# pmandros/node2vec2rank

Hardware: AMD Instinct MI355X
Metric: nodes ranked/sec + SpMM HBM GB/s, K-layer N-node graph at 1/2/4/8 GPUs (higher is better)
Workload: dtype fp32; 1 GPU; cfg4: 2-layer ER N=1M avg-deg 50, dims {8,16,32,64,128} x {cosine,euclidean}, sequential; nodes=1000000, layers=2, embed_dim=128, columns=10, comparisons=1, parallelism=single GPU

## Files before the change

### include/n2v2r.h

```cpp
#ifndef N2V2R_H
#define N2V2R_H

#include <stddef.h>
#include <stdint.h>

#ifdef __cplusplus
extern "C" {
#endif

typedef enum {
  N2V2R_OK = 0,
  N2V2R_ERR_BAD_ARG = 1,
  N2V2R_ERR_UNSUPPORTED_METRIC = 2,
  N2V2R_ERR_NO_CONVERGENCE = 3,
  N2V2R_ERR_HIP = 4,
  N2V2R_ERR_OUT_OF_MEMORY = 5,
  N2V2R_ERR_NOT_READY = 6,
  N2V2R_ERR_UNSUPPORTED_AGG = 7,
  N2V2R_ERR_INTERNAL = 8,
  N2V2R_ERR_RCCL = 9
} n2v2r_status;

enum { N2V2R_SEQUENTIAL = 0, N2V2R_ONE_VS_BEFORE = 1, N2V2R_ONE_VS_REST = 2 };
enum { N2V2R_COSINE = 0, N2V2R_EUCLIDEAN = 1, N2V2R_CORRELATION = 2 };
enum { N2V2R_SYM_DETECT = -1, N2V2R_SYM_NO = 0, N2V2R_SYM_YES = 1 };
enum { N2V2R_AGG_BORDA = 0, N2V2R_AGG_NONE = -1 };

enum { N2V2R_EIG_FULL_FIRST_PASS = 1, N2V2R_EIG_DENSE_RR = 2,
       N2V2R_EIG_TEST_REDO_CYCLE = 4 ,
       N2V2R_EIG_TEST_BAND_FAIL = 8 ,
       N2V2R_EIG_TEST_STURM_FAIL = 32 ,
       N2V2R_EIG_TIME_SPMM = 16 ,
       N2V2R_EIG_TEST_NO_STAGNATION = 64 ,
       N2V2R_EIG_TEST_FAIL_ALONE = 128 ,
       N2V2R_EIG_TEST_TRI_TIMEOUT = 1024  };

typedef struct n2v2r_handle n2v2r_handle;
typedef struct n2v2r_simgroup n2v2r_simgroup;

typedef struct {
  int block;
  int max_basis;
  int keep;
  int max_restarts;
  double tol;
  uint64_t seed;
  int solver_flags;
} n2v2r_eig_opts;

typedef struct {
  int restarts;
  int block_applications;
  int converged;
  int basis;
  double max_residual;
  double ms_total, ms_spmm, ms_ortho, ms_rr_host;
  int64_t spmm_launches;
  double spmm_algo_bytes;
  int stagnated;
  int rr_fallbacks;
  double gpu_ms_spmm[2];
  int64_t spmm_timed_launches[2];
  double spmm_stage_bytes[2];
  double est_scale;
  int lean_checks;
  int pool_blocks;
  int spmm_form;
  double stag_cap;
  int y_captured;
  int tri_fallbacks;
} n2v2r_eig_stats;

int n2v2r_create(int device, n2v2r_handle** out);
void n2v2r_destroy(n2v2r_handle* h);
int n2v2r_last_error(const n2v2r_handle* h, char* buf, size_t len);
const char* n2v2r_version(void);

#define N2V2R_UNIQUE_ID_BYTES 128
int n2v2r_comm_unique_id(char* out, size_t len);
int n2v2r_create_rccl(int device, int rank, int world, const char* unique_id, n2v2r_handle** out);
int n2v2r_simgroup_create(int world, n2v2r_simgroup** out);
void n2v2r_simgroup_destroy(n2v2r_simgroup* g);
int n2v2r_create_sim(int device, n2v2r_simgroup* g, int rank, n2v2r_handle** out);
int n2v2r_dist_info(const n2v2r_handle* h, int* rank, int* world, int64_t* row0, int64_t* n_local);

int n2v2r_create_multi(const int* devices, int n_gpus, n2v2r_handle** out);
int n2v2r_multi_devices(const n2v2r_handle* h, int* devices, int cap);

int n2v2r_set_num_layers(n2v2r_handle* h, int num_layers, int64_t n);
int n2v2r_set_layer_csr(n2v2r_handle* h, int k, int64_t n, int64_t nnz, const int64_t* indptr,
                        const int32_t* indices, const float* data, int symmetric);
int n2v2r_set_layer_dense(n2v2r_handle* h, int k, int64_t n, const float* A, int symmetric);
enum { N2V2R_CORR_UNSIGNED = 0, N2V2R_CORR_SIGNED = 1, N2V2R_CORR_SIGNED_HYBRID = 2,
       N2V2R_CORR_RAW = 3 };
int n2v2r_set_layer_corr(n2v2r_handle* h, int k, int64_t n, int64_t samples,
                         const double* E , int kind, double power);
int n2v2r_soft_connectivity(n2v2r_handle* h, int64_t n, int64_t samples, const double* E,
                            int kind, const double* powers, int n_powers, double* conn);
enum { N2V2R_COR_PEARSON = 0, N2V2R_COR_SPEARMAN = 1, N2V2R_COR_BICOR = 2 };
int n2v2r_set_layer_corr_method(n2v2r_handle* h, int k, int64_t n, int64_t samples,
                                const double* E , int kind,
                                double power, int method, int64_t* fallback );
int n2v2r_soft_connectivity_method(n2v2r_handle* h, int64_t n, int64_t samples, const double* E,
                                   int kind, const double* powers, int n_powers, int method,
                                   double* conn, int64_t* fallback );
enum { N2V2R_TF_ABSOLUTE = 1, N2V2R_TF_BINARIZE = 2, N2V2R_TF_THRESHOLD = 4 };
typedef struct { int64_t nonzero; int64_t kept; double cut; } n2v2r_transform_stats;
int n2v2r_transform_layer(n2v2r_handle* h, int k, int flags, double threshold,
                          double top_percent_keep, n2v2r_transform_stats* stats );
enum { N2V2R_TOM_UNSIGNED = 0, N2V2R_TOM_SIGNED = 1 };
int n2v2r_tom_layer(n2v2r_handle* h, int k, int type);
int n2v2r_layers_to_csr(n2v2r_handle* h, int64_t* nnz );
int n2v2r_count_layer_nonzeros(n2v2r_handle* h, int64_t* nnz );
int n2v2r_set_layer_csr_rows(n2v2r_handle* h, int k, int64_t n, int64_t row0, int64_t n_rows,
                             int64_t nnz, const int64_t* indptr, const int32_t* indices,
                             const float* data);

int n2v2r_uase(n2v2r_handle* h, int d, const n2v2r_eig_opts* opts, n2v2r_eig_stats* stats);
// ... 32 lines not shown
```

### include/n2v2r_diag.h

```cpp
#ifndef N2V2R_DIAG_H
#define N2V2R_DIAG_H

#include "n2v2r.h"

#ifdef __cplusplus
extern "C" {
#endif

int n2v2r_bench_spmm(n2v2r_handle* h, int k, int transpose, int b, int reps, const float* X,
                     float* Y, double* avg_ms, double* algo_bytes);
int n2v2r_bench_spmm_tiled(n2v2r_handle* h, int k, int transpose, int b, int nb, int reps,
                           const float* X, float* Y, double* avg_ms);

int n2v2r_spmm_col_blocks(const n2v2r_handle* h, int b);

int n2v2r_rr_top(n2v2r_handle* h, int c, const double* H, int p, double* w, float* S);

int n2v2r_pip_pass(n2v2r_handle* h, int64_t n, int nq, const float* Q, float* Za, float* Zb,
                   float tau, int first, int form, uint64_t seed, double* gram, double* R,
                   int* flags, int* any_flag, int* skipped);

typedef struct n2v2r_gram_info {
  int form;
  int rs_form;
  int rs_chunks;
  int split2;
  int tile_nb, tile_wb, tile_rows;
  int rpw1, rpw2;
} n2v2r_gram_info;

int n2v2r_gram_apply(n2v2r_handle* h, int b, const float* X, float* Z, float* W,
                     n2v2r_gram_info* info);

typedef struct n2v2r_ritz_info {
  int fused;
  int launches;
  int lds_bytes;
} n2v2r_ritz_info;

int n2v2r_ritz_step(n2v2r_handle* h, int b, int nq, int keep, int lean, const float* Q,
                    const float* W, const float* S, const double* theta, float* X, float* MX,
                    double* res, n2v2r_ritz_info* info);

typedef struct n2v2r_pass_info {
  int gram_form;
  int gram_flush;
  int64_t nchunks;
  int64_t rows_per_chunk;
  int stage;
  int nwg;
  int apply_kernel;
  int reserved;
  uint64_t fill_seed;
} n2v2r_pass_info;

int n2v2r_block_gram(n2v2r_handle* h, int b, int na, int nb, const float* A, const float* B,
                     double* G, n2v2r_pass_info* info);

int n2v2r_ortho_pass(n2v2r_handle* h, int b, int nq, const float* Q, float* Z, int in_place,
                     int first, int cond, uint64_t seed, double* gram, double* xinv, float* F,
                     int* flags, int* any_flag, n2v2r_pass_info* info);

int n2v2r_rr_band_top(n2v2r_handle* h, int c, int kp, const double* hband, int64_t hband_len,
                      const double* theta_prev, int p, double* w, float* S);

typedef struct n2v2r_rr_info {
  int form_ran;
  int sturm_err;
  int second_solves;
  int reduce_err;
  int tri_coop;
  int msect_points, msect_rounds;
  int reserved;
} n2v2r_rr_info;

int n2v2r_rr_stage(n2v2r_handle* h, int c, int kp, const double* hband, int64_t hband_len,
                   const double* theta_prev, int p, int form, double* w, float* S,
                   double* Y , n2v2r_rr_info* info);

typedef struct n2v2r_embed_info {
  int form;
  int launches;
  int ldu;
  int rpw;
  int64_t colmax_chunks;
  int64_t colmax_rows;
} n2v2r_embed_info;

int n2v2r_embed_step(n2v2r_handle* h, int b, int d, const float* U, const double* theta,
                     n2v2r_embed_info* info);

int n2v2r_h2d_layer_bytes(const n2v2r_handle* h, int64_t* per_rank, int cap);

int n2v2r_get_layer_dense(n2v2r_handle* h, int k, float* A );

int n2v2r_get_layer_csr_nnz(n2v2r_handle* h, int k, int transpose, int64_t* nnz);
int n2v2r_get_layer_csr(n2v2r_handle* h, int k, int transpose, int64_t* indptr, int32_t* indices,
                        float* data);

int n2v2r_bench_sparsify_pass(n2v2r_handle* h, int k, int which, int reps, double* avg_ms,
                              double* bytes);

int n2v2r_bench_transform_pass(n2v2r_handle* h, int k, int which, int flags, double threshold,
// ... 21 lines not shown
```

### node2vec2rank_amd/_lib.py

```python
from __future__ import annotations

import atexit
import ctypes
import os
import threading
import warnings
import weakref

import numpy as np

from .coexpression import KINDS, METHODS, Coexpression, method_name

_HERE = os.path.dirname(os.path.abspath(__file__))
LIB_PATH = os.environ.get("N2V2R_LIB", os.path.join(_HERE, "lib", "libn2v2r_hip.so"))

OK = 0
ERR_BAD_ARG = 1
ERR_UNSUPPORTED_METRIC = 2
ERR_NO_CONVERGENCE = 3
ERR_HIP = 4
ERR_OUT_OF_MEMORY = 5
ERR_NOT_READY = 6
ERR_UNSUPPORTED_AGG = 7
ERR_INTERNAL = 8
ERR_RCCL = 9
AGG_BORDA, AGG_NONE = 0, -1
EIG_TIME_SPMM = 16
EIG_TEST_NO_STAGNATION = 64
EIG_TEST_FAIL_ALONE = 128

STRATEGY = {"sequential": 0, "one_vs_before": 1, "one_vs_rest": 2}
METRIC = {"cosine": 0, "euclidean": 1, "correlation": 2}
SYM_DETECT, SYM_NO, SYM_YES = -1, 0, 1

EXPORTED = [
    "n2v2r_create", "n2v2r_destroy", "n2v2r_last_error", "n2v2r_version",
    "n2v2r_set_num_layers", "n2v2r_set_layer_csr", "n2v2r_uase", "n2v2r_get_embedding",
    "n2v2r_get_left_embedding", "n2v2r_get_singular_values", "n2v2r_set_embedding",
    "n2v2r_rank", "n2v2r_get_distances", "n2v2r_get_borda", "n2v2r_rank_timing",
    "n2v2r_pairwise_distances", "n2v2r_borda_columns", "n2v2r_borda_columns_ex",
    "n2v2r_column_sums",
    "n2v2r_synchronize", "n2v2r_bench_spmm", "n2v2r_bench_spmm_tiled", "n2v2r_spmm_col_blocks",
    "n2v2r_comm_unique_id", "n2v2r_create_rccl", "n2v2r_simgroup_create",
    "n2v2r_simgroup_destroy", "n2v2r_create_sim", "n2v2r_dist_info", "n2v2r_set_layer_csr_rows",
    "n2v2r_rr_top", "n2v2r_rr_band_top", "n2v2r_set_layer_dense", "n2v2r_project",
    "n2v2r_create_multi", "n2v2r_multi_devices", "n2v2r_h2d_layer_bytes",
    "n2v2r_set_layer_corr", "n2v2r_get_layer_dense", "n2v2r_transform_layer",
    "n2v2r_bench_transform_pass", "n2v2r_tom_layer", "n2v2r_bench_tom_tiles", "n2v2r_pip_pass",
    "n2v2r_gram_apply", "n2v2r_ritz_step", "n2v2r_layers_to_csr", "n2v2r_count_layer_nonzeros",
    "n2v2r_get_layer_csr_nnz", "n2v2r_get_layer_csr", "n2v2r_bench_sparsify_pass",
    "n2v2r_block_gram", "n2v2r_ortho_pass", "n2v2r_soft_connectivity",
    "n2v2r_soft_connectivity_chunks", "n2v2r_set_layer_corr_method",
    "n2v2r_soft_connectivity_method", "n2v2r_corr_ranks", "n2v2r_corr_standardise",
    "n2v2r_bench_corr_rows", "n2v2r_rr_stage", "n2v2r_embed_step",
]
UNIQUE_ID_BYTES = 128


class ArpackNoConvergence(RuntimeError):
    """UASE eigensolver did not reach the residual tolerance (scipy raises
    ``ArpackNoConvergence`` in the reference's svds path)."""


class EigOpts(ctypes.Structure):
    _fields_ = [("block", ctypes.c_int), ("max_basis", ctypes.c_int), ("keep", ctypes.c_int),
                ("max_restarts", ctypes.c_int), ("tol", ctypes.c_double),
                ("seed", ctypes.c_uint64), ("solver_flags", ctypes.c_int)]


class EigStats(ctypes.Structure):
    _fields_ = [("restarts", ctypes.c_int), ("block_applications", ctypes.c_int),
                ("converged", ctypes.c_int), ("basis", ctypes.c_int),
                ("max_residual", ctypes.c_double), ("ms_total", ctypes.c_double),
                ("ms_spmm", ctypes.c_double), ("ms_ortho", ctypes.c_double),
                ("ms_rr_host", ctypes.c_double), ("spmm_launches", ctypes.c_int64),
                ("spmm_algo_bytes", ctypes.c_double), ("stagnated", ctypes.c_int),
                ("rr_fallbacks", ctypes.c_int), ("gpu_ms_spmm", ctypes.c_double * 2),
                ("spmm_timed_launches", ctypes.c_int64 * 2),
                ("spmm_stage_bytes", ctypes.c_double * 2), ("est_scale", ctypes.c_double),
                ("lean_checks", ctypes.c_int), ("pool_blocks", ctypes.c_int),
                ("spmm_form", ctypes.c_int), ("stag_cap", ctypes.c_double),
                ("y_captured", ctypes.c_int), ("tri_fallbacks", ctypes.c_int)]

    def as_dict(self):
        out = {}
        for k, _ in self._fields_:
            v = getattr(self, k)
            out[k] = list(v) if isinstance(v, ctypes.Array) else v
        return out


class GramInfo(ctypes.Structure):
    _fields_ = [(k, ctypes.c_int) for k in ("form", "rs_form", "rs_chunks", "split2", "tile_nb",
                                            "tile_wb", "tile_rows", "rpw1", "rpw2")]


class EmbedInfo(ctypes.Structure):
    _fields_ = [("form", ctypes.c_int), ("launches", ctypes.c_int), ("ldu", ctypes.c_int),
                ("rpw", ctypes.c_int), ("colmax_chunks", ctypes.c_int64),
                ("colmax_rows", ctypes.c_int64)]


class RitzInfo(ctypes.Structure):
    _fields_ = [(k, ctypes.c_int) for k in ("fused", "launches", "lds_bytes")]


class PassInfo(ctypes.Structure):
    _fields_ = [("gram_form", ctypes.c_int), ("gram_flush", ctypes.c_int),
                ("nchunks", ctypes.c_int64), ("rows_per_chunk", ctypes.c_int64),
                ("stage", ctypes.c_int), ("nwg", ctypes.c_int), ("apply_kernel", ctypes.c_int),
                ("reserved", ctypes.c_int), ("fill_seed", ctypes.c_uint64)]


class RrInfo(ctypes.Structure):
    _fields_ = [(k, ctypes.c_int) for k in ("form_ran", "sturm_err", "second_solves",
                                            "reduce_err", "tri_coop", "msect_points",
                                            "msect_rounds", "reserved")]


RR_AS_FIT, RR_STURM, RR_BAND_REDUCE, RR_DENSE_FROM_BAND, RR_DENSE = -1, 0, 1, 2, 3

GRAM_STREAM, GRAM_LINES, GRAM_NARROW, GRAM_MFMA = 0, 1, 2, 3


class TransformStats(ctypes.Structure):
    _fields_ = [("nonzero", ctypes.c_int64), ("kept", ctypes.c_int64), ("cut", ctypes.c_double)]


TF_ABSOLUTE, TF_BINARIZE, TF_THRESHOLD = 1, 2, 4
TOM_KINDS = {"unsigned": 0, "signed": 1}


def _warn_zero_mad(what, fallback):
    if int(fallback[0]) > 0:
        warnings.warn(f"{what}: {int(fallback[0])} rows have zero MAD (first: row "
                      f"{int(fallback[1])}); Pearson standardisation used for them",
                      RuntimeWarning, stacklevel=3)


_lib = None
_lock = threading.RLock()

_vp = ctypes.c_void_p
_i = ctypes.c_int
_i64 = ctypes.c_int64


def _p(dtype):
    return np.ctypeslib.ndpointer(dtype=dtype, flags="C_CONTIGUOUS")


def load(path: str | None = None):
    global _lib
    with _lock:
        if _lib is not None:
            return _lib
        p = path or LIB_PATH
        if not os.path.exists(p):
            raise RuntimeError(
                f"n2v2r HIP library not found at {p}; build it with "
                "`python -m node2vec2rank_amd.build` (there is no CPU fallback)")
        lib = ctypes.CDLL(p)
        atexit.register(_teardown)
        sig = {
            "n2v2r_create": (_i, [_i, ctypes.POINTER(_vp)]),
            "n2v2r_destroy": (None, [_vp]),
            "n2v2r_last_error": (_i, [_vp, ctypes.c_char_p, ctypes.c_size_t]),
            "n2v2r_version": (ctypes.c_char_p, []),
            "n2v2r_set_num_layers": (_i, [_vp, _i, _i64]),
            "n2v2r_set_layer_csr": (_i, [_vp, _i, _i64, _i64, _p(np.int64), _p(np.int32),
                                         _p(np.float32), _i]),
            "n2v2r_uase": (_i, [_vp, _i, ctypes.POINTER(EigOpts), ctypes.POINTER(EigStats)]),
            "n2v2r_get_embedding": (_i, [_vp, _p(np.float32)]),
            "n2v2r_get_left_embedding": (_i, [_vp, _p(np.float32)]),
            "n2v2r_get_singular_values": (_i, [_vp, _p(np.float64)]),
            "n2v2r_set_embedding": (_i, [_vp, _i, _i64, _i, _p(np.float32)]),
            "n2v2r_rank": (_i, [_vp, _i, _p(np.int32), _i, _p(np.int32), _i, _i,
                                ctypes.POINTER(_i), ctypes.POINTER(_i)]),
            "n2v2r_get_distances": (_i, [_vp, _i, _p(np.float64)]),
            "n2v2r_get_borda": (_i, [_vp, _i, _p(np.int64)]),
            "n2v2r_rank_timing": (_i, [_vp, ctypes.POINTER(ctypes.c_double),
                                       ctypes.POINTER(ctypes.c_double)]),
            "n2v2r_pairwise_distances": (_i, [_vp, _p(np.float64), _p(np.float64), _i64, _i, _i,
                                              _p(np.float64)]),
            "n2v2r_borda_columns": (_i, [_vp, _p(np.float64), _i64, _i, _p(np.int64)]),
            "n2v2r_borda_columns_ex": (_i, [_vp, _p(np.float64), _i64, _i, _vp, _i, _vp,
                                            _p(np.int64), _p(np.int32)]),
            "n2v2r_column_sums": (_i, [_vp, _i, _p(np.float32)]),
            "n2v2r_synchronize": (_i, [_vp]),
            "n2v2r_bench_spmm": (_i, [_vp, _i, _i, _i, _i, _p(np.float32), _vp,
                                      ctypes.POINTER(ctypes.c_double),
                                      ctypes.POINTER(ctypes.c_double)]),
            "n2v2r_bench_spmm_tiled": (_i, [_vp, _i, _i, _i, _i, _i, _p(np.float32), _vp,
                                            ctypes.POINTER(ctypes.c_double)]),
            "n2v2r_spmm_col_blocks": (_i, [_vp, _i]),
            "n2v2r_rr_top": (_i, [_vp, _i, _p(np.float64), _i, _p(np.float64), _p(np.float32)]),
            "n2v2r_pip_pass": (_i, [_vp, _i64, _i, _p(np.float32), _p(np.float32), _vp,
                                    ctypes.c_float, _i, _i, ctypes.c_uint64, _p(np.float64), _vp,
                                    _p(np.int32), _p(np.int32), _p(np.int32)]),
            "n2v2r_gram_apply": (_i, [_vp, _i, _p(np.float32), _vp, _p(np.float32),
                                      ctypes.POINTER(GramInfo)]),
            "n2v2r_embed_step": (_i, [_vp, _i, _i, _vp, _vp, ctypes.POINTER(EmbedInfo)]),
            "n2v2r_ritz_step": (_i, [_vp, _i, _i, _i, _i, _vp, _vp, _vp, _vp, _vp, _vp, _vp,
                                     ctypes.POINTER(RitzInfo)]),
            "n2v2r_block_gram": (_i, [_vp, _i, _i, _i, _vp, _vp, _vp, ctypes.POINTER(PassInfo)]),
            "n2v2r_ortho_pass": (_i, [_vp, _i, _i, _vp, _vp, _i, _i, _i, ctypes.c_uint64, _vp,
                                      _vp, _vp, _vp, _vp, ctypes.POINTER(PassInfo)]),
            "n2v2r_rr_band_top": (_i, [_vp, _i, _i, _p(np.float64), ctypes.c_int64, _vp, _i,
                                       _p(np.float64), _p(np.float32)]),
            "n2v2r_rr_stage": (_i, [_vp, _i, _i, _vp, ctypes.c_int64, _vp, _i, _i, _vp, _vp, _vp,
                                    ctypes.POINTER(RrInfo)]),
            "n2v2r_set_layer_dense": (_i, [_vp, _i, _i64, _p(np.float32), _i]),
            "n2v2r_project": (_i, [_vp, _i64, _i64, _p(np.float64), _i, _p(np.float64)]),
            "n2v2r_comm_unique_id": (_i, [ctypes.c_char_p, ctypes.c_size_t]),
            "n2v2r_create_rccl": (_i, [_i, _i, _i, ctypes.c_char_p, ctypes.POINTER(_vp)]),
            "n2v2r_simgroup_create": (_i, [_i, ctypes.POINTER(_vp)]),
            "n2v2r_simgroup_destroy": (None, [_vp]),
            "n2v2r_create_sim": (_i, [_i, _vp, _i, ctypes.POINTER(_vp)]),
            "n2v2r_dist_info": (_i, [_vp, ctypes.POINTER(_i), ctypes.POINTER(_i),
                                     ctypes.POINTER(_i64), ctypes.POINTER(_i64)]),
            "n2v2r_set_layer_csr_rows": (_i, [_vp, _i, _i64, _i64, _i64, _i64, _p(np.int64),
                                              _p(np.int32), _p(np.float32)]),
            "n2v2r_create_multi": (_i, [_p(np.int32), _i, ctypes.POINTER(_vp)]),
            "n2v2r_multi_devices": (_i, [_vp, _vp, _i]),
            "n2v2r_h2d_layer_bytes": (_i, [_vp, _vp, _i]),
            "n2v2r_set_layer_corr": (_i, [_vp, _i, _i64, _i64, _p(np.float64), _i,
                                          ctypes.c_double]),
            "n2v2r_get_layer_dense": (_i, [_vp, _i, _p(np.float32)]),
            "n2v2r_transform_layer": (_i, [_vp, _i, _i, ctypes.c_double, ctypes.c_double,
                                           ctypes.POINTER(TransformStats)]),
            "n2v2r_bench_transform_pass": (_i, [_vp, _i, _i, _i, ctypes.c_double, _i,
                                                ctypes.POINTER(ctypes.c_double),
                                                ctypes.POINTER(ctypes.c_double)]),
            "n2v2r_tom_layer": (_i, [_vp, _i, _i]),
            "n2v2r_bench_tom_tiles": (_i, [_vp, _i, _i, _i, _p(np.float64),
                                           ctypes.POINTER(ctypes.c_double)]),
            "n2v2r_layers_to_csr": (_i, [_vp, _vp]),
            "n2v2r_count_layer_nonzeros": (_i, [_vp, _p(np.int64)]),
            "n2v2r_get_layer_csr_nnz": (_i, [_vp, _i, _i, ctypes.POINTER(_i64)]),
            "n2v2r_get_layer_csr": (_i, [_vp, _i, _i, _p(np.int64), _p(np.int32),
                                         _p(np.float32)]),
            "n2v2r_bench_sparsify_pass": (_i, [_vp, _i, _i, _i, ctypes.POINTER(ctypes.c_double),
                                               ctypes.POINTER(ctypes.c_double)]),
            "n2v2r_soft_connectivity": (_i, [_vp, _i64, _i64, _p(np.float64), _i, _p(np.float64),
                                             _i, _p(np.float64)]),
            "n2v2r_soft_connectivity_chunks": (_i, [_vp, _i64, _i64, _p(np.float64), _i,
                                                    _p(np.float64), _i, _i, _p(np.float64),
                                                    ctypes.POINTER(_i),
                                                    ctypes.POINTER(ctypes.c_double)]),
            "n2v2r_set_layer_corr_method": (_i, [_vp, _i, _i64, _i64, _p(np.float64), _i,
                                                 ctypes.c_double, _i, _vp]),
            "n2v2r_soft_connectivity_method": (_i, [_vp, _i64, _i64, _p(np.float64), _i,
                                                    _p(np.float64), _i, _i, _p(np.float64),
                                                    _vp]),
            "n2v2r_corr_ranks": (_i, [_vp, _i64, _i64, _p(np.float64), _p(np.float64)]),
            "n2v2r_corr_standardise": (_i, [_vp, _i64, _i64, _p(np.float64), _i, _p(np.float64),
                                            ctypes.POINTER(_i64)]),
            "n2v2r_bench_corr_rows": (_i, [_vp, _i64, _i64, _p(np.float64), _i, _i,
                                           _p(np.float64)]),
        }
        for name, (res, args) in sig.items():
            f = getattr(lib, name)
            f.restype = res
            f.argtypes = args
        _lib = lib
        return lib


def comm_unique_id() -> bytes:
    lib = load()
    buf = ctypes.create_string_buffer(UNIQUE_ID_BYTES)
    st = lib.n2v2r_comm_unique_id(buf, UNIQUE_ID_BYTES)
    if st != OK:
        raise RuntimeError(f"n2v2r_comm_unique_id failed with status {st}")
    return buf.raw


class SimGroup:

    def __init__(self, world: int):
        self.lib = load()
        g = _vp()
        st = self.lib.n2v2r_simgroup_create(int(world), ctypes.byref(g))
        if st != OK:
            raise RuntimeError(f"n2v2r_simgroup_create failed with status {st}")
# ... 499 lines not shown
            e = np.ascontiguousarray(np.asarray(values), dtype=np.float64)
        except (TypeError, ValueError) as err:
            raise ValueError(f"expression must be a real n x samples array: {err}") from None
        if e.ndim != 2:
            raise ValueError(f"expression must be 2-D (n x samples), got {e.ndim}-D")
        return e

    def corr_ranks(self, E):
        e = self._rows_arg(E)
        out = np.empty_like(e)
        self._check(self.lib.n2v2r_corr_ranks(self.h, e.shape[0], e.shape[1], e, out),
                    "corr_ranks")
        return out

    def corr_standardise(self, E, method: str = "pearson", return_bad_row: bool = False):
        e = self._rows_arg(E)
        out = np.empty_like(e)
        bad = _i64()
        self._check(self.lib.n2v2r_corr_standardise(self.h, e.shape[0], e.shape[1], e,
                                                    METHODS[method_name(method)], out,
                                                    ctypes.byref(bad)), "corr_standardise")
        return (out, int(bad.value)) if return_bad_row else out

    def bench_corr_rows(self, E, method: str = "pearson", reps: int = 10):
        e = self._rows_arg(E)
        ms = np.empty(int(reps), dtype=np.float64)
        self._check(self.lib.n2v2r_bench_corr_rows(self.h, e.shape[0], e.shape[1], e,
                                                   METHODS[method_name(method)], int(reps), ms),
                    "bench_corr_rows")
        return ms

    def soft_connectivity_chunks(self, E, kind: str = "unsigned", powers=(6.0,), chunks: int = 0):
        e, kid, pw = self._soft_args(E, kind, powers)
        out = np.empty((pw.size, e.shape[0]), dtype=np.float64)
        used, ms = _i(), ctypes.c_double()
        self._check(self.lib.n2v2r_soft_connectivity_chunks(
            self.h, e.shape[0], e.shape[1], e, kid, pw, int(pw.size), int(chunks), out,
            ctypes.byref(used), ctypes.byref(ms)), "soft_connectivity_chunks")
        return out, used.value, ms.value

    def rr_top(self, H, p: int):
        H = np.ascontiguousarray(H, dtype=np.float64)
        c = H.shape[0]
        w = np.empty(p, dtype=np.float64)
        S = np.empty((c, p), dtype=np.float32)
        self._check(self.lib.n2v2r_rr_top(self.h, c, H, int(p), w, S), "rr_top")
        return w, S

    def pip_pass(self, Q, Za, Zb=None, tau: float = 0.0, first: int = 0, form: int = 0,
                 seed: int = 1):
        Q = np.ascontiguousarray(Q, dtype=np.float32)
        nq, n = Q.shape[0], Q.shape[1]
        za = np.array(Za, dtype=np.float32, order="C")
        zb = None if Zb is None else np.array(Zb, dtype=np.float32, order="C")
        if Q.shape != (nq, n, 8) or za.shape != (n, 8) or (zb is not None and zb.shape != (n, 8)):
            raise ValueError("pip_pass: Q is (nq, n, 8), Za and Zb are (n, 8)")
        nz = 1 if zb is None else 2
        gram = np.empty((nq + 1, 8, 8) if zb is None else (2, nq + 2, 8, 8), dtype=np.float64)
        R = np.empty((8, 8), dtype=np.float64) if zb is None else None
        flags = np.empty(8, dtype=np.int32)
        any_flag = np.empty(1, dtype=np.int32)
        skipped = np.empty(nq + nz, dtype=np.int32)
        self._check(self.lib.n2v2r_pip_pass(
            self.h, n, nq, Q, za, None if zb is None else zb.ctypes.data_as(ctypes.c_void_p),
            float(tau), int(first), int(form), int(seed), gram,
            None if R is None else R.ctypes.data_as(ctypes.c_void_p), flags, any_flag, skipped),
            "pip_pass")
        return {"Za": za, "Zb": zb, "gram": gram, "R": R, "flags": flags,
                "any_flag": int(any_flag[0]), "skipped": skipped}

    def gram_apply(self, X, want_z: bool = True):
        X = np.ascontiguousarray(X, dtype=np.float32)
        if X.ndim != 2 or X.shape[0] != self.n:
            raise ValueError(f"gram_apply: X must be ({self.n}, b), got {X.shape}")
        b, nl = X.shape[1], self._n_local()
        W = np.empty((nl, b), dtype=np.float32)
        Z = np.empty((self.num_layers, nl, b), dtype=np.float32) if want_z else None
        info = GramInfo()
        self._check(self.lib.n2v2r_gram_apply(
            self.h, int(b), X, Z.ctypes.data_as(ctypes.c_void_p) if want_z else None, W,
            ctypes.byref(info)), "gram_apply")
        return W, Z, {k: getattr(info, k) for k, _ in GramInfo._fields_}

    def embed_step(self, U, theta, b: int = 8):
        if U is None or theta is None:
            raise ValueError("embed_step: U and theta are required")
        U = np.ascontiguousarray(U, dtype=np.float32)
        theta = np.ascontiguousarray(theta, dtype=np.float64)
        if U.ndim != 2 or U.shape[0] != self.n or theta.shape != (U.shape[1],):
            raise ValueError(f"embed_step: U must be ({self.n}, d) and theta (d,), got "
                             f"{U.shape} and {theta.shape}")
        info = EmbedInfo()
        self._check(self.lib.n2v2r_embed_step(
            self.h, int(b), int(U.shape[1]), U.ctypes.data_as(ctypes.c_void_p),
            theta.ctypes.data_as(ctypes.c_void_p), ctypes.byref(info)), "embed_step")
        self.d = int(U.shape[1])
        return {k: getattr(info, k) for k, _ in EmbedInfo._fields_}

    def ritz_step(self, Q, W, S, theta, lean: bool = False):
        Q = np.ascontiguousarray(Q, dtype=np.float32)
        S = np.ascontiguousarray(S, dtype=np.float32)
        theta = np.ascontiguousarray(theta, dtype=np.float64)
        W = None if W is None else np.ascontiguousarray(W, dtype=np.float32)
        nl = self._n_local()
        if Q.ndim != 3 or Q.shape[1] != nl or (W is not None and W.shape != Q.shape):
            raise ValueError(f"ritz_step: Q and W must be (nq, {nl}, b), got {Q.shape}")
        nq, b = Q.shape[0], Q.shape[2]
        if S.ndim != 2 or S.shape[0] != nq * b or theta.shape != (S.shape[1],):
            raise ValueError("ritz_step: S must be (nq b, keep) and theta (keep,)")
        keep = S.shape[1]
        pb = max(1, keep // max(b, 1))
        X = np.empty((pb, nl, b), dtype=np.float32)
        MX = None if lean else np.empty((pb, nl, b), dtype=np.float32)
        res = None if lean else np.empty(keep, dtype=np.float64)
        info = RitzInfo()

        def ptr(a):
            return None if a is None else a.ctypes.data_as(ctypes.c_void_p)

        self._check(self.lib.n2v2r_ritz_step(
            self.h, int(b), int(nq), int(keep), int(bool(lean)), ptr(Q), ptr(W), ptr(S),
            ptr(theta), ptr(X), ptr(MX), ptr(res), ctypes.byref(info)), "ritz_step")
        return X, MX, res, {k: getattr(info, k) for k, _ in RitzInfo._fields_}

    def block_gram(self, A, B):
        A = np.ascontiguousarray(A, dtype=np.float32)
        B = np.ascontiguousarray(B, dtype=np.float32)
        nl = self._n_local()
        if A.ndim != 3 or B.ndim != 3 or A.shape[1:] != B.shape[1:] or A.shape[1] != nl:
            raise ValueError(f"block_gram: A and B must be (blocks, {nl}, b), got {A.shape}, "
                             f"{B.shape}")
        na, nb, b = A.shape[0], B.shape[0], A.shape[2]
        G = np.empty((na * b, nb * b), dtype=np.float64)
        info = PassInfo()
        vp = lambda a: a.ctypes.data_as(ctypes.c_void_p)
        self._check(self.lib.n2v2r_block_gram(self.h, int(b), int(na), int(nb), vp(A), vp(B),
                                              vp(G), ctypes.byref(info)), "block_gram")
        return G, {k: getattr(info, k) for k, _ in PassInfo._fields_}

    def ortho_pass(self, Q, Z, in_place: bool = True, first: int = 0, cond: int = -1,
                   seed: int = 1):
        z = np.array(Z, dtype=np.float32, order="C")
        nl = self._n_local()
        if z.ndim != 2 or z.shape[0] != nl:
            raise ValueError(f"ortho_pass: Z must be ({nl}, b), got {z.shape}")
        b = z.shape[1]
        Q = np.ascontiguousarray(Q, dtype=np.float32).reshape(-1, nl, b)
        nq = Q.shape[0]
        gram = np.empty(((nq + 1) * b, b), dtype=np.float64)
        xinv = None if b == 8 else np.empty((b, b), dtype=np.float64)
        F = None if b == 8 else np.empty(((nq + 1) * b, b), dtype=np.float32)
        flags = np.empty(b, dtype=np.int32)
        any_flag = np.empty(1, dtype=np.int32)
        info = PassInfo()
        vp = lambda a: None if a is None or a.size == 0 else a.ctypes.data_as(ctypes.c_void_p)
        self._check(self.lib.n2v2r_ortho_pass(
            self.h, int(b), int(nq), vp(Q), vp(z), int(bool(in_place)), int(first), int(cond),
            int(seed), vp(gram), vp(xinv), vp(F), vp(flags), vp(any_flag), ctypes.byref(info)),
            "ortho_pass")
        return {"Z": z, "gram": gram, "xinv": xinv, "F": F, "flags": flags,
                "any_flag": int(any_flag[0]),
                "info": {k: getattr(info, k) for k, _ in PassInfo._fields_}}

    def rr_band_top(self, hband, c: int, kp: int, theta_prev, p: int):
        hband = np.ascontiguousarray(hband, dtype=np.float64).ravel()
        tp = None
# ... 106 lines not shown
```

### node2vec2rank_amd/build.py

```python
from __future__ import annotations

import os
import subprocess
import sys

HERE = os.path.dirname(os.path.abspath(__file__))
CSRC = os.path.join(HERE, "csrc")
OUT_DIR = os.path.join(HERE, "lib")
_TAG = os.environ.get("N2V2R_BUILD_TAG", "")
LIB = os.path.join(OUT_DIR, f"libn2v2r_hip_{_TAG}.so" if _TAG else "libn2v2r_hip.so")
OBJ_DIR = os.path.join(OUT_DIR, f"obj_{_TAG}" if _TAG else "obj")

HIP_SOURCES = ["spmm.hip", "dense.hip", "gemm.hip", "corr.hip", "soft_threshold.hip", "tom.hip", "transform.hip", "sparsify.hip", "rank.hip",
               "rr.hip", "rr_band.hip", "rr_sturm.hip", "ingest.hip", "engine.cpp", "layers.cpp",
               "comm.cpp", "gram_op.cpp", "solver.cpp", "ranking.cpp", "multi.cpp"]
HOST_SOURCES: list = []
HEADERS = ["common.h", "corr_tile.h", "pip_pass.h", "spmm_args.h", "engine.h", "gram_op.h", os.path.join("..", "..", "include", "n2v2r.h"),
           os.path.join("..", "..", "include", "n2v2r_diag.h")]
ARCH = os.environ.get("N2V2R_OFFLOAD_ARCH", "gfx950")
_EXTRA = os.environ.get("N2V2R_EXTRA_HIP_FLAGS", "").split() if _TAG else []


def _hipcc():
    for c in (os.environ.get("HIPCC"), "/opt/rocm/bin/hipcc", "hipcc"):
        if c and (os.path.isabs(c) and os.path.exists(c) or not os.path.isabs(c)):
            return c
    raise RuntimeError("hipcc not found")


def _newer(target, deps):
    if not os.path.exists(target):
        return True
    t = os.path.getmtime(target)
    return any(os.path.getmtime(d) > t for d in deps if os.path.exists(d))


def build(force: bool = False, verbose: bool = False) -> str:
    os.makedirs(OBJ_DIR, exist_ok=True)
    hipcc = _hipcc()
    headers = [os.path.join(CSRC, h) for h in HEADERS]
    objs, cmds = [], []
    for src in HIP_SOURCES + HOST_SOURCES:
        path = os.path.join(CSRC, src)
        obj = os.path.join(OBJ_DIR, src + ".o")
        objs.append(obj)
        if not force and not _newer(obj, [path, __file__] + headers):
            continue
        if src in HIP_SOURCES:
            lang = ["-x", "hip"]
            cmd = [hipcc, *lang, f"--offload-arch={ARCH}", "-O3", "-std=c++17", "-fPIC",
                   "-munsafe-fp-atomics", *_EXTRA, "-c", path, "-o", obj]
        else:
            cmd = ["g++", "-O3", "-march=x86-64-v3", "-std=c++17", "-fPIC", "-c", path, "-o", obj]
        cmds.append(cmd)
    from concurrent.futures import ThreadPoolExecutor
    jobs = max(1, min(8, len(cmds), os.cpu_count() or 1))

    def _run(cmd):
        if verbose:
            print(" ".join(cmd), flush=True)
        subprocess.run(cmd, check=True)

    with ThreadPoolExecutor(jobs) as ex:
        list(ex.map(_run, cmds))
    if force or _newer(LIB, objs):
        tmp = LIB + ".tmp"
        cmd = [hipcc, f"--offload-arch={ARCH}", "-shared", "-fPIC", *objs, "-o", tmp,
               "-L/opt/rocm/lib", "-lrccl", "-Wl,-rpath,/opt/rocm/lib"]
        if verbose:
            print(" ".join(cmd), flush=True)
        subprocess.run(cmd, check=True)
        os.replace(tmp, LIB)
    return LIB


if __name__ == "__main__":
    print(build(force="--force" in sys.argv, verbose=True))
```

### node2vec2rank_amd/csrc/engine.h

```cpp
#pragma once

#include <hip/hip_runtime.h>
#include <rccl/rccl.h>

#include <algorithm>
#include <chrono>
#include <cmath>
#include <condition_variable>
#include <cstdarg>
#include <cstdlib>
#include <cstdio>
#include <cstring>
#include <memory>
#include <mutex>
#include <numeric>
#include <string>
#include <thread>
#include <exception>
#include <system_error>
#include <vector>

#include "../../include/n2v2r.h"
#include "../../include/n2v2r_diag.h"
#include "common.h"

#include "pip_pass.h"
#include "spmm_args.h"
#define DIST_MAX_COLS 256
struct DistPlan {
  int n_cols;
  int col_dim[DIST_MAX_COLS];
  int col_metric[DIST_MAX_COLS];
  int col_out[DIST_MAX_COLS];
  int dmax;
};
extern "C" {
hipError_t n2v2r_launch_spmm(const SpmmArgs& args, int B, hipStream_t stream);
int n2v2r_spmm_rpw(const SpmmArgs& args, int B);
hipError_t n2v2r_launch_row_sums(const CsrDev& A, float* out, hipStream_t stream);
hipError_t n2v2r_launch_spmm_tile(const SpmmTileArgs& a, hipStream_t stream);
hipError_t n2v2r_launch_chunk_major_keys(uint64_t* keys, int64_t nnz, int64_t npad, int W,
                                         int64_t rc, hipStream_t stream);
int n2v2r_spmm_tile_rows(int64_t n, int ncu, int wpc, int wbits);
hipError_t n2v2r_launch_cb_count(const CsrDev& A, int64_t cw, int nb, int32_t* cnt,
                                 hipStream_t stream);
hipError_t n2v2r_launch_cb_rowptrs(const int32_t* cnt, int64_t n, int nb, int64_t nnz,
                                   int64_t* tsum, size_t tsum_elems, int64_t* rp, int32_t* wo,
                                   int wbits, hipStream_t stream);
int64_t n2v2r_cb_scan_tiles(int64_t n, int nb);
hipError_t n2v2r_launch_cb_fill(const CsrDev& A, int64_t cw, int nb, const int64_t* rp,
                                int32_t* idx, float* dat, int cbits, int wbits,
                                hipStream_t stream);
hipError_t n2v2r_launch_ritz_nn(const BlockList& A0, const BlockList& A1, const float* G, int ldg,
                                int cb, const OutBlockList& O0, const OutBlockList& O1, int64_t n,
                                int grid, hipStream_t stream);
size_t n2v2r_ritz_nn_lds_bytes(int a_blocks, int cb);
hipError_t n2v2r_launch_ts_nn(const BlockList& A, const float* G, int ldg, int cb,
                              const OutBlockList& O, const BlockList& C, float alpha, float beta,
                              int64_t n, hipStream_t stream);
hipError_t n2v2r_launch_rr_band(const double* hband, int c, int kp, double* theta, double* AB,
                                double* Varr, double* taua, double* d, double* e, double* refl,
                                double* Y, float* S, int ldS, int p, int* err,
                                hipStream_t stream);
int n2v2r_rr_band_jm(int c);
hipError_t n2v2r_launch_ts_tn2(const BlockList& A, const float* Za, const float* Zb, int64_t n,
                               double* partial, size_t partial_elems, double* out,
                               hipStream_t stream);
hipError_t n2v2r_launch_rmul8(const double* r2, double* r1, hipStream_t stream);
hipError_t n2v2r_launch_pair_fixup(double* g2, int nblk_all, int nq_old, double* ra,
                                   hipStream_t stream);
constexpr size_t N2V2R_PAIR_PLAN_WORDS = 208 + (size_t)(N2V2R_BAND_MAXC / 8) * 129;
hipError_t n2v2r_launch_pip_pair(const BlockList& Q, float* Za, float* Zb, double* g2, int64_t n,
                                 int* flags, int* any_flag, int* sticky, uint64_t seed_a,
                                 uint64_t seed_b, int64_t row0, float skip_tol, int* skipped,
                                 int* plan, size_t plan_bytes, hipStream_t stream);
hipError_t n2v2r_launch_fill_normal(float* blk, int w, int64_t n, uint64_t seed, const int* flags,
                                    const int* cond, uint64_t ctr0, hipStream_t stream);
hipError_t n2v2r_launch_resid(const BlockList& X, const BlockList& MX, const double* theta,
                              int64_t n, double* partial, size_t partial_elems, double* out,
                              hipStream_t stream);
hipError_t n2v2r_launch_scale_cols(float* blk, int w, int64_t n, const float* s,
                                   hipStream_t stream);
hipError_t n2v2r_colmax_plan(int64_t n, int d, size_t key_elems, int64_t* nchunks,
                             int64_t* rows_per_chunk);
hipError_t n2v2r_launch_colmax_keys(const float* U, int64_t ldu, int64_t n, int d, int64_t row0,
                                    unsigned long long* keys, size_t key_elems,
                                    unsigned long long* best, hipStream_t stream);
hipError_t n2v2r_launch_colmax_sign(const unsigned long long* best, int ncols_padded,
                                    const float* U, int64_t ldu, int d, int64_t row0, int64_t n,
                                    float* sign, hipStream_t stream);
hipError_t n2v2r_launch_distances(const float* Y, int K, int64_t n, int64_t ldy, int64_t lrows,
                                  int strategy, int layer_i, const DistPlan& plan, double* out,
                                  int64_t ldo, hipStream_t stream);
hipError_t n2v2r_launch_pairwise(const double* a, const double* b, int64_t n, int dim, int metric,
                                 double* out, hipStream_t stream);
hipError_t n2v2r_launch_borda_init(const double* vals, int64_t n, int nseg, uint64_t* keys,
                                   int32_t* idx, unsigned long long* seg_or,
                                   unsigned long long* seg_and, hipStream_t stream);
int n2v2r_radix_tiles(int64_t n);
size_t n2v2r_radix_hist_elems(int64_t n, int nseg);
hipError_t n2v2r_launch_radix_pass(const uint64_t* kin, const int32_t* pin, uint64_t* kout,
                                   int32_t* pout, int64_t n, int nseg, int shift, uint32_t* hist,
                                   hipStream_t stream);
hipError_t n2v2r_launch_borda_finish(const int32_t* sorted_idx, int64_t n, int nseg, int ncols,
                                     int32_t* pos, int64_t* borda, hipStream_t stream);
hipError_t n2v2r_launch_tie_flags(const uint64_t* sorted_keys, int64_t n, int nseg, int32_t* tied,
// ... 70 lines not shown
                                 hipStream_t stream);
size_t n2v2r_rr_sturm_scratch(int c, int p);
void n2v2r_rr_sturm_msect(int p, int* points, int* rounds);
hipError_t n2v2r_launch_rr_band_expand(const double* hband, int c, int kp, const double* theta,
                                       double* H, hipStream_t stream);
hipError_t n2v2r_launch_csr_scan(const int64_t* ip, const int32_t* ix, const float* dv,
                                 int64_t n_rows, int64_t n_cols, uint64_t* keys, int32_t* idx,
                                 unsigned* flags, hipStream_t stream);
hipError_t n2v2r_launch_csr_from_sorted(const uint64_t* keys, const int32_t* idx, const float* dv,
                                        int64_t nnz, int64_t n_cols, int64_t* tp, int32_t* tx,
                                        float* td, hipStream_t stream);
hipError_t n2v2r_launch_csr_compare(const int64_t* ap, const int32_t* ax, const float* av,
                                    const int64_t* bp, const int32_t* bx, const float* bv,
                                    int64_t n_rows, int64_t nnz, unsigned* flag,
                                    hipStream_t stream);
hipError_t n2v2r_launch_csr_rebase(const int64_t* ip, int64_t r0, int64_t nr, int64_t* out,
                                   hipStream_t stream);
}

inline bool rr_sturm_enabled() {
  const char* e = std::getenv("N2V2R_RR");
  return !(e && e[0] == 'b');
}

enum class RrForm {
  Sturm = 0,
  BandReduce = 1,
  DenseFromBand = 2,
  Dense = 3
};
inline bool banded(RrForm f) { return f == RrForm::Sturm || f == RrForm::BandReduce; }

constexpr int kReduceMaxc = 640;
inline bool rr_reduce_fits(int kp, int c) { return kp + 8 <= 192 && c <= kReduceMaxc; }
inline RrForm rr_after_sturm(int kp, int c) {
  return rr_reduce_fits(kp, c) ? RrForm::BandReduce : RrForm::DenseFromBand;
}

inline bool lean_enabled() {
  const char* e = std::getenv("N2V2R_LEAN_W");
  return !(e && e[0] == '0');
}


namespace n2v2r_int {

struct HipFail {
  hipError_t e;
  std::string where;
};
struct StatusFail {
  int code;
  std::string msg;
};

#define HIPCHK(expr)                                                  \
  do {                                                                \
    hipError_t _e = (expr);                                           \
    if (_e != hipSuccess) throw HipFail{_e, #expr};                   \
  } while (0)

inline double now_ms() {
  using namespace std::chrono;
  return duration<double, std::milli>(steady_clock::now().time_since_epoch()).count();
}

inline bool env_flag(const char* name) {
  const char* e = std::getenv(name);
  return e && *e && *e != '0';
}
inline bool debug_poison() {
  static const bool v = env_flag("N2V2R_POISON");
  return v;
}
inline bool debug_finite() {
  static const bool v = env_flag("N2V2R_DEBUG_FINITE");
  return v;
}
inline bool debug_ortho() {
  static const bool v = env_flag("N2V2R_DEBUG_ORTHO");
  return v;
}

struct DevBuf {
  void* p = nullptr;
  size_t bytes = 0;
  DevBuf() = default;
  DevBuf(const DevBuf&) = delete;
  DevBuf& operator=(const DevBuf&) = delete;
  ~DevBuf() { release(); }
  void release() {
    if (p) (void)hipFree(p);
    p = nullptr;
    bytes = 0;
  }
  void ensure(size_t b, hipStream_t st = nullptr) {
    if (bytes >= b && p) return;
    release();
    if (b == 0) b = 16;
    hipError_t e = hipMalloc(&p, b);
    if (e != hipSuccess) {
      p = nullptr;
      throw StatusFail{N2V2R_ERR_OUT_OF_MEMORY,
                       "hipMalloc of " + std::to_string(b) + " bytes failed"};
    }
    const int fill = debug_poison() ? 0xFF : 0;
    if (st) {
      e = hipMemsetAsync(p, fill, b, st);
    } else {
      e = hipMemset(p, fill, b);
      if (e == hipSuccess) e = hipDeviceSynchronize();
    }
    if (e != hipSuccess) throw HipFail{e, "hipMemset"};
    bytes = b;
  }
  void ensure_raw(size_t b) {
    if (bytes >= b && p) return;
    if (b == 0) b = 16;
    if (debug_poison()) return ensure(b);
    release();
    if (hipMalloc(&p, b) != hipSuccess) {
      p = nullptr;
      throw StatusFail{N2V2R_ERR_OUT_OF_MEMORY,
                       "hipMalloc of " + std::to_string(b) + " bytes failed"};
    }
    bytes = b;
  }
  void swap(DevBuf& o) {
    std::swap(p, o.p);
    std::swap(bytes, o.bytes);
  }
  template <class T>
  T* as() const {
    return static_cast<T*>(p);
  }
};

struct LayerDev {
  DevBuf indptr, indices, data;
  DevBuf t_indptr, t_indices, t_data;
  int64_t nnz = 0, t_nnz = 0;
  int64_t n_rows = 0;
  bool unit = false, t_unit = false;
  bool symmetric = true;
  bool loaded = false;
  bool dense = false;
  DevBuf dA, dAT;
  int64_t lda = 0;
  const float* dense_a() const { return dA.as<float>(); }
  const float* dense_at() const { return symmetric ? dA.as<float>() : dAT.as<float>(); }
  CsrDev csr() const {
    return CsrDev{indptr.as<int64_t>(), indices.as<int32_t>(), data.as<float>(), n_rows, nnz,
                  unit ? 1 : 0};
  }
  CsrDev csr_t() const {
    if (symmetric) return csr();
    return CsrDev{t_indptr.as<int64_t>(), t_indices.as<int32_t>(), t_data.as<float>(), n_rows,
                  t_nnz, t_unit ? 1 : 0};
  }
  struct ColBlocks {
    DevBuf wo, idx, dat;
    CsrBlk blk[CB_MAX];
    int nb = 0;
    int wbits = 0;
    int cbits = 0;
    int64_t ncols = 0;
    bool built = false;
    bool usable = false;
  };
  ColBlocks cb, cb_t;
  DevBuf c_indptr, c_indices, c_data;
  int64_t c_nnz = 0, c_rows = 0;
  int64_t c_rc = 0;
  bool c_built = false;
  CsrDev csr_c() const {
    return CsrDev{c_indptr.as<int64_t>(), c_indices.as<int32_t>(), c_data.as<float>(), c_rows,
                  c_nnz, (symmetric ? unit : t_unit) ? 1 : 0};
  }
  void drop_col_blocks() {
    for (ColBlocks* c : {&cb, &cb_t}) {
      c->wo.release();
      c->idx.release();
      c->dat.release();
      c->built = false;
    }
    c_indptr.release();
    c_indices.release();
    c_data.release();
    c_built = false;
  }
};

void build_col_blocks(const CsrDev& A, int64_t ncols, LayerDev::ColBlocks& out, hipStream_t st,
                      int nb, int wbits);
bool ensure_col_blocks(LayerDev& L, int64_t ncols, hipStream_t st, int nb, int wbits);
int tile_wbits(const std::vector<std::unique_ptr<LayerDev>>& layers, int nb);
void ensure_colcsr(LayerDev& L, int64_t ncols, int64_t rows_out, hipStream_t st, int64_t npad = 0,
                   int W = 1, int64_t rc = 0);

struct Comm {
  int rank = 0, world = 1;
  virtual ~Comm() = default;
  virtual void allgather(const void* send, void* recv, size_t bytes, hipStream_t st) = 0;
  virtual void allreduce_sum_f64(double* buf, size_t count, hipStream_t st) = 0;
  virtual void allreduce_max_u64(unsigned long long* buf, size_t count, hipStream_t st) = 0;
  virtual void allreduce_sum_u64(unsigned long long* buf, size_t count, hipStream_t st) = 0;
  virtual void allreduce_sum_f32(float* buf, size_t count, hipStream_t st) = 0;
  virtual void reduce_scatter_sum_f32(const float* send, float* recv, size_t count,
                                      hipStream_t st) = 0;
  virtual const char* kind() const = 0;
  virtual bool shares_device() const { return false; }
  virtual void abort() {}
};

struct NcclFail {
  ncclResult_t r;
  std::string where;
};
#define NCCLCHK(expr)                                   \
  do {                                                  \
    ncclResult_t _r = (expr);                           \
    if (_r != ncclSuccess) throw NcclFail{_r, #expr};   \
  } while (0)

std::unique_ptr<Comm> make_rccl_comm(ncclComm_t c, int rank, int world);
}

struct n2v2r_simgroup {
  int world = 1;
  std::mutex m;
  std::condition_variable cv;
  int arrived = 0;
  uint64_t generation = 0;
  bool aborted = false;
  std::vector<const void*> ptrs;
  std::vector<std::vector<unsigned char>> host;
  std::vector<int> dev;
  void barrier() {
    std::unique_lock<std::mutex> lk(m);
    const uint64_t gen = generation;
    if (aborted) throw n2v2r_int::StatusFail{N2V2R_ERR_INTERNAL, "thread group aborted"};
    if (++arrived == world) {
      arrived = 0;
      ++generation;
      cv.notify_all();
    } else {
      cv.wait(lk, [&] { return generation != gen || aborted; });
      if (generation == gen)
        throw n2v2r_int::StatusFail{N2V2R_ERR_INTERNAL, "thread group aborted"};
    }
  }
  void abort() {
    std::lock_guard<std::mutex> lk(m);
    aborted = true;
    cv.notify_all();
  }
};

namespace n2v2r_int {
std::unique_ptr<Comm> make_thread_comm(n2v2r_simgroup* g, int rank, int device);

struct EigWorkspace {
  std::vector<std::unique_ptr<DevBuf>> pool;
  size_t block_bytes = 0;
  std::vector<std::unique_ptr<DevBuf>> zk;
  DevBuf zg;
  DevBuf rinv, flg, anyflag, gsmall, csmall;
  DevBuf rback;
  DevBuf tri, refl, ytri, tscr;
  DevBuf trcoop;
  DevBuf btf;
  DevBuf hband, band, varr, taua, rrerr;
  DevBuf fcoef;
  DevBuf dbgflag;
  DevBuf tflag;
  DevBuf s2part;
  DevBuf g2, pair_ra;
  DevBuf pair_plan;
  DevBuf sturm;
  DevBuf rres;
  DevBuf skipc;
  DevBuf tblk;
};
}

using n2v2r_int::Comm;
using n2v2r_int::DevBuf;
using n2v2r_int::LayerDev;
using n2v2r_int::EigWorkspace;
using n2v2r_int::HipFail;
using n2v2r_int::StatusFail;

struct n2v2r_handle {
  int device = 0;
  hipStream_t stream = nullptr;
  hipStream_t side = nullptr;
  hipEvent_t cb_ev[2 * SPMM_MAX_LAYERS] = {};
  void* pin = nullptr;
  size_t pin_bytes = 0;
  void ensure_pin(size_t bytes) {
    if (pin_bytes >= bytes) return;
    if (pin) (void)hipHostFree(pin);
    pin = nullptr;
    pin_bytes = 0;
    if (hipHostMalloc(&pin, bytes, hipHostMallocDefault) != hipSuccess) {
      (void)hipGetLastError();
      throw std::bad_alloc();
    }
    pin_bytes = bytes;
  }
  std::string err;
  int K = 0;
  int64_t n = 0;
  std::unique_ptr<Comm> comm;
  int rank = 0, world = 1;
  int64_t row0 = 0, nloc = 0, npad = 0;
  int64_t h2d_layer_bytes = 0;
  std::vector<std::unique_ptr<LayerDev>> layers;

  int d = 0;
  int ldy = 0;
  DevBuf Y;
  DevBuf U;
  std::vector<double> sigma;
  bool have_embedding = false;

  int ncmp = 0, ncols = 0;
  DevBuf D;
  DevBuf Dloc;
  DevBuf Dgat;
  DevBuf borda;
  bool have_borda = false;
  std::vector<hipEvent_t> tev;
  double ms_dist = 0, ms_borda = 0;

  DevBuf partial;
  size_t partial_elems = 0;
  DevBuf theta;
  DevBuf resid;
  DevBuf colscale;
  DevBuf keys, best;
  DevBuf gath;
  EigWorkspace ews;
  DevBuf dense_work;
  size_t dense_work_elems = 0;
  bool dense_layers() const { return !layers.empty() && layers[0]->dense; }
  void dense_apply(const float* Aloc, int64_t lda, const float* X, int ldx, int b, float* Y,
                   int64_t ldy, float beta, const float* colscale, const float* Bt = nullptr) {
    const size_t need = (size_t)std::max<int64_t>(nloc, 1) * b * 16;
    if (dense_work_elems < need) {
      dense_work.ensure(sizeof(float) * need);
      dense_work_elems = need;
    }
    const char* tn = std::getenv("N2V2R_DENSE_TN");
    if (Bt && nloc == n && !(tn && tn[0] == '0')) {
      const hipError_t e = n2v2r_launch_dense_tn(Bt, lda, nloc, n, X, ldx, b, Y, ldy, beta,
                                                 colscale, dense_work.as<float>(),
                                                 dense_work_elems, stream);
      if (e == hipSuccess) return;
      if (e != hipErrorNotSupported) throw HipFail{e, "n2v2r_launch_dense_tn"};
    }
    HIPCHK(n2v2r_launch_dense_gemm(Aloc, lda, nloc, n, X, ldx, b, Y, ldy, beta, colscale,
                                   dense_work.as<float>(), dense_work_elems, stream));
  }
  DevBuf rs_keys[2], rs_idx[2], rs_pos, rs_hist, rs_or, rs_and;
  DevBuf ing_keys[2], ing_pay[2], ing_hist, ing_flag;
  DevBuf tf_scr;
  DevBuf tom_out;
  DevBuf ypanel;


  void set_err(const char* fmt, ...) {
    char buf[1024];
    va_list ap;
    va_start(ap, fmt);
    vsnprintf(buf, sizeof(buf), fmt, ap);
    va_end(ap);
    err = buf;
  }

  void set_partition(int64_t n_global) {
    n = n_global;
    if (world <= 1) {
      row0 = 0;
      nloc = npad = n;
      return;
    }
    npad = (n + world - 1) / world;
    row0 = std::min<int64_t>(n, (int64_t)rank * npad);
    nloc = std::max<int64_t>(0, std::min<int64_t>(n, row0 + npad) - row0);
  }

  void gather_panel(const float* local, float* global, int w) {
    if (!comm) {
      if (local != global)
        HIPCHK(hipMemcpyAsync(global, local, sizeof(float) * npad * w, hipMemcpyDeviceToDevice,
                              stream));
      return;
    }
    comm->allgather(local, global, sizeof(float) * npad * w, stream);
  }
  hipStream_t cstream = nullptr;
  hipEvent_t cev[2 * SPMM_MAX_LAYERS] = {};
  void gather_panel_async(const float* local, float* global, int w, int slot) {
    if (!cstream) {
      HIPCHK(hipStreamCreateWithFlags(&cstream, hipStreamNonBlocking));
      for (hipEvent_t& e : cev) HIPCHK(hipEventCreateWithFlags(&e, hipEventDisableTiming));
    }
    HIPCHK(hipEventRecord(cev[2 * slot], stream));
    HIPCHK(hipStreamWaitEvent(cstream, cev[2 * slot], 0));
    comm->allgather(local, global, sizeof(float) * npad * w, cstream);
    HIPCHK(hipEventRecord(cev[2 * slot + 1], cstream));
  }
  void gather_wait(int slot) { HIPCHK(hipStreamWaitEvent(stream, cev[2 * slot + 1], 0)); }
  hipEvent_t rev[SPMM_MAX_LAYERS + 1] = {};
  int rs_pending = 0;
  void reduce_scatter_async(const float* send, float* recv, size_t count) {
    if (!cstream) {
      HIPCHK(hipStreamCreateWithFlags(&cstream, hipStreamNonBlocking));
      for (hipEvent_t& e : cev) HIPCHK(hipEventCreateWithFlags(&e, hipEventDisableTiming));
    }
    if (!rev[0])
      for (hipEvent_t& e : rev) HIPCHK(hipEventCreateWithFlags(&e, hipEventDisableTiming));
    HIPCHK(hipEventRecord(rev[rs_pending], stream));
    HIPCHK(hipStreamWaitEvent(cstream, rev[rs_pending], 0));
    comm->reduce_scatter_sum_f32(send, recv, count, cstream);
    ++rs_pending;
  }
  void rs_wait_all() {
    if (!rs_pending) return;
    HIPCHK(hipEventRecord(rev[SPMM_MAX_LAYERS], cstream));
    HIPCHK(hipStreamWaitEvent(stream, rev[SPMM_MAX_LAYERS], 0));
    rs_pending = 0;
  }
  void allreduce_f64(double* buf, size_t count) {
    if (comm) comm->allreduce_sum_f64(buf, count, stream);
  }

  std::vector<n2v2r_handle*> ranks;
  std::unique_ptr<n2v2r_simgroup> own_group;
  struct n2v2r_int_rank_pool* pool = nullptr;
  bool broken = false;
  bool multi() const { return !ranks.empty(); }
};

namespace n2v2r_int {

template <class F>
int guarded(n2v2r_handle* h, F&& f) {
// ... 92 lines not shown
```

### node2vec2rank_amd/csrc/gram_op.cpp

```cpp
#include "gram_op.h"

using namespace n2v2r_int;

namespace n2v2r_int {

bool layers_ready(n2v2r_handle* h) {
  if (h->K < 1) {
    h->err = "no layers set";
    return false;
  }
  for (auto& L : h->layers)
    if (!L->loaded) {
      h->err = "a layer was not loaded";
      return false;
    }
  return true;
}

bool col_blocks_wanted(const n2v2r_handle* h, int b) {
  if (b != 8 || h->dense_layers() || h->layers.empty()) return false;
  const char* e = std::getenv("N2V2R_SPMM_CB");
  if (e && e[0] == '1') return true;
  if (e && e[0] == '0') return false;
  const double panel = 4.0 * b * (double)h->n;
  return panel > 8.0e6;
}

bool gather_overlap() {
  const char* e = std::getenv("N2V2R_GATHER_OVERLAP");
  return !(e && e[0] == '0');
}

bool split2_wanted(const n2v2r_handle* h, int b) {
  const char* e = std::getenv("N2V2R_SPMM_SPLIT");
  const int force = e ? (e[0] == '0' ? 0 : 1) : -1;
  if (b != 8 || h->comm || h->dense_layers() || h->K < 2 || h->K > 8) return false;
  if (force >= 0) return force == 1;
  return (double)h->K * (double)h->n * 32.0 > 4.0 * 1024 * 1024;
}

int tile_nb_auto(int64_t nglob) {
  int nb = 4;
  while (nb < 64 && (double)nglob * 32.0 / nb > 2.0 * 1024 * 1024) nb *= 2;
  return nb;
}

int tile_rows_for(const n2v2r_handle* h, int wbits) {
  int ncu = 0;
  HIPCHK(hipDeviceGetAttribute(&ncu, hipDeviceAttributeMultiprocessorCount, h->device));
  return n2v2r_spmm_tile_rows(h->nloc, ncu, 2, wbits);
}

SpmmTileArgs spmm_tile_args(const CsrBlk* table, int nb, int wbits, int tile_rows, int64_t n,
                            int k0, int nk, int sum, int64_t ldy) {
  SpmmTileArgs a{};
  a.blk = table + (size_t)k0 * nb;
  a.ldx = 8;
  a.ldy = ldy;
  a.n = n;
  a.K = nk;
  a.nb = nb;
  a.sum = sum;
  a.tile_rows = tile_rows;
  a.wbits = wbits;
  return a;
}


void GramOp::setup(int b_, bool time_stages) {
  b = b_;
  time_spmm = time_stages;
  tkind.clear();
  tbytes.clear();
  const size_t bb = sizeof(float) * npad * b;
  while ((int)h->ews.zk.size() < K) h->ews.zk.emplace_back(new DevBuf());
  for (int k = 0; k < K; ++k) h->ews.zk[k]->ensure(bb);
  if (h->comm) {
    h->gath.ensure(sizeof(float) * h->world * npad * b);
    h->ews.zg.ensure(sizeof(float) * (size_t)K * h->world * npad * b);
  }
  setup_tiled();
  setup_stage2_form();
}

void GramOp::setup_tiled() {
  const int64_t nglob = h->n;
  col_blocks = col_blocks_wanted(h, b);
  if (!col_blocks) return;
  const int nb_auto = tile_nb_auto(nglob);
  const char* tn_ = std::getenv("N2V2R_SPMM_TILE_NB");
  tile_nb = tn_ ? std::atoi(tn_) : nb_auto;
  if (tile_nb != 4 && tile_nb != 8 && tile_nb != 16 && tile_nb != 32 && tile_nb != 64 &&
      tile_nb != 128)
    tile_nb = nb_auto;
  tile_wb = tile_wbits(h->layers, tile_nb);
  for (auto& Lp : h->layers)
    col_blocks = ensure_col_blocks(*Lp, nglob, st, tile_nb, tile_wb) && col_blocks;
  if (!col_blocks) return;
  tile_rows = tile_rows_for(h, tile_wb);
  const int nb = tile_nb;
  std::vector<CsrBlk> hb((size_t)2 * K * nb);
  for (int k = 0; k < K; ++k) {
    const LayerDev& L = *h->layers[k];
    for (int j = 0; j < nb; ++j) {
      hb[(size_t)k * nb + j] = (L.symmetric ? L.cb : L.cb_t).blk[j];
      hb[(size_t)(K + k) * nb + j] = L.cb.blk[j];
    }
  }
  h->ews.tblk.ensure(sizeof(CsrBlk) * hb.size());
  HIPCHK(hipMemcpyAsync(h->ews.tblk.p, hb.data(), sizeof(CsrBlk) * hb.size(),
                        hipMemcpyHostToDevice, st));
  HIPCHK(hipStreamSynchronize(st));
}

void GramOp::setup_stage2_form() {
  rs_form = false;
  if (h->comm && !h->dense_layers()) {
    const char* e = std::getenv("N2V2R_DIST_STAGE2");
    rs_form = e && std::strcmp(e, "rs") == 0 ? true
              : e && std::strcmp(e, "gather") == 0 ? false
              : h->world > 1;
    if (rs_form) {
      const char* ce = std::getenv("N2V2R_RS_CHUNKS");
      rs_chunks = std::max(1, std::min(SPMM_MAX_LAYERS, ce ? std::atoi(ce) : 4));
      rs_rc = (npad + rs_chunks - 1) / rs_chunks;
      rs_chunks = (int)((npad + rs_rc - 1) / rs_rc);
      if (rs_chunks <= 1) rs_rc = 0;
      for (auto& Lp : h->layers)
        ensure_colcsr(*Lp, h->n, (int64_t)h->world * npad, st, npad, h->world, rs_rc);
    }
  }
  split2 = split2_wanted(h, b) && !col_blocks;
  pending = nullptr;
  if (split2) h->ews.s2part.ensure(sizeof(float) * (size_t)K * npad * 8);
}

void GramOp::poison_scratch() {
  for (auto& d : h->ews.zk) HIPCHK(hipMemsetAsync(d->p, 0xFF, d->bytes, st));
}


int GramOp::tbeg() {
  if (!time_spmm) return -1;
  const size_t i = tkind.size();
  while (h->tev.size() < 2 * (i + 1)) {
    hipEvent_t e;
    HIPCHK(hipEventCreate(&e));
    h->tev.push_back(e);
  }
  HIPCHK(hipEventRecord(h->tev[2 * i], st));
  tkind.push_back(-1);
  tbytes.push_back(0.0);
  return (int)i;
}
void GramOp::tend(int i, int kind, double bytes) {
  if (i < 0) return;
  HIPCHK(hipEventRecord(h->tev[2 * (size_t)i + 1], st));
  tkind[i] = kind;
  tbytes[i] = bytes;
}
void GramOp::tsum(n2v2r_eig_stats* out) {
  if (!time_spmm || !out) return;
  HIPCHK(hipStreamSynchronize(st));
  for (size_t i = 0; i < tkind.size(); ++i) {
    if (tkind[i] < 0) continue;
    float ms = 0.f;
    HIPCHK(hipEventElapsedTime(&ms, h->tev[2 * i], h->tev[2 * i + 1]));
    out->gpu_ms_spmm[tkind[i]] += ms;
    out->spmm_timed_launches[tkind[i]] += 1;
    out->spmm_stage_bytes[tkind[i]] += tbytes[i];
  }
}
double GramOp::layer_bytes(int k, bool transposed) const {
  const LayerDev& L = *h->layers[k];
  const bool t = transposed && !L.symmetric;
  return spmm_algo_bytes(t ? L.t_nnz : L.nnz, t ? L.t_unit : L.unit, n,
                         (int64_t)h->world * npad, b);
}
double GramOp::stage_bytes(bool transposed) const {
  double s = 0.0;
  for (int k = 0; k < K; ++k) s += layer_bytes(k, transposed);
  return s;
}


void GramOp::materialize() {
  if (!pending) return;
  const float* parts[SPMM_MAX_LAYERS];
  const int np = pending_parts(parts);
  HIPCHK(n2v2r_launch_zsum(parts, np, pending, n, st));
  pending = nullptr;
}

void GramOp::stage1(const float* xg, int layer) {
  const int k0 = layer < 0 ? 0 : layer, nk = layer < 0 ? K : 1;
  const double bytes = layer < 0 ? stage_bytes(true) : layer_bytes(layer, true);
  int te;
  if (col_blocks) {
    SpmmTileArgs a = tile_args(false, k0, nk, 0, 8);
    for (int i = 0; i < nk; ++i) {
      a.X[i] = xg;
      a.Y[i] = zk(k0 + i);
    }
    te = tbeg();
    HIPCHK(n2v2r_launch_spmm_tile(a, st));
  } else {
    SpmmArgs a{};
    a.K = nk;
    a.ldx = a.ldy = b;
    a.split = split2 ? 1 : 0;
    for (int i = 0; i < nk; ++i) {
      a.A[i] = h->layers[k0 + i]->csr_t();
      a.X[i] = xg;
      a.Y[i] = zk(k0 + i);
    }
    a.rpw = rpw1 = n2v2r_spmm_rpw(a, b);
    te = tbeg();
    HIPCHK(n2v2r_launch_spmm(a, b, st));
  }
  tend(te, 0, bytes);
}

void GramOp::stage1_gathered(const float* xg) {
  if (h->comm && K > 1 && gather_overlap() && st == h->stream) {
    for (int k = 0; k < K; ++k) {
      stage1(xg, k);
      h->gather_panel_async(zk(k), gathered_z(k), b, k);
    }
    for (int k = 0; k < K; ++k) h->gather_wait(k);
    return;
  }
  stage1(xg);
  if (h->comm)
    for (int k = 0; k < K; ++k) h->gather_panel(zk(k), gathered_z(k), b);
}

void GramOp::stage2_flat(float* Wout) {
  SpmmArgs s{};
  s.K = K;
  s.sum = 1;
  s.ldx = s.ldy = b;
  for (int k = 0; k < K; ++k) {
    s.A[k] = h->layers[k]->csr();
    s.X[k] = stage2_in(k);
  }
  s.Y[0] = Wout;
  if (split2) {
    materialize();
    s.sum = 0;
    s.split = 1;
    for (int k = 0; k < K; ++k) s.Y[k] = s2part(k);
    pending = Wout;
  }
  s.rpw = rpw2 = n2v2r_spmm_rpw(s, b);
  const double bytes = stage_bytes(false);
  const int te = tbeg();
  HIPCHK(n2v2r_launch_spmm(s, b, st));
  tend(te, 1, bytes);
  for (int k = 0; k < K; ++k) {
    const LayerDev& L = *h->layers[k];
    algo_bytes += spmm_algo_bytes(L.nnz, L.unit, n, n, b) +
                  spmm_algo_bytes(L.symmetric ? L.nnz : L.t_nnz,
                                  L.symmetric ? L.unit : L.t_unit, n, n, b);
  }
  launches += 2;
}

void GramOp::stage2_tiled(float* Wout) {
  SpmmTileArgs s = tile_args(true, 0, K, 1, 8);
  for (int k = 0; k < K; ++k) s.X[k] = stage2_in(k);
  s.Y[0] = Wout;
  const double b0 = stage_bytes(true), b1 = stage_bytes(false);
  const int te = tbeg();
  HIPCHK(n2v2r_launch_spmm_tile(s, st));
  tend(te, 1, b1);
  algo_bytes += b0 + b1;
  launches += 2;
}

void GramOp::stage2_rs(float* Wout) {
  const int64_t ng = (int64_t)h->world * npad;
  float* P = h->ews.zg.as<float>();
  const double b0 = stage_bytes(true);
  double b1 = 0.0;
  SpmmArgs s2{};
  s2.K = K;
  s2.sum = 1;
  s2.ldx = s2.ldy = b;
  for (int k = 0; k < K; ++k) {
    const LayerDev& L = *h->layers[k];
    s2.A[k] = L.csr_c();
    s2.X[k] = zk(k);
    b1 += spmm_algo_bytes(L.c_nnz, s2.A[k].unit != 0, ng, npad, b);
  }
  s2.Y[0] = P;
  s2.rpw = rpw2 = n2v2r_spmm_rpw(s2, b);
  const int te = tbeg();
  if (rs_chunks <= 1) {
    HIPCHK(n2v2r_launch_spmm(s2, b, st));
    tend(te, 1, b1);
    h->comm->reduce_scatter_sum_f32(P, Wout, (size_t)npad * b, st);
  } else {
    const int W = h->world;
    for (int c = 0; c < rs_chunks; ++c) {
      const int64_t r0 = (int64_t)c * rs_rc;
      const int64_t rows_c = std::min<int64_t>(rs_rc, npad - r0);
      if (rows_c <= 0) break;
      SpmmArgs sc = s2;
      for (int k = 0; k < K; ++k) {
        sc.A[k].indptr = s2.A[k].indptr + (size_t)r0 * W;
        sc.A[k].n_rows = (int64_t)W * rows_c;
      }
      float* pc = P + (size_t)r0 * W * b;
      sc.Y[0] = pc;
      HIPCHK(n2v2r_launch_spmm(sc, b, st));
      h->reduce_scatter_async(pc, Wout + (size_t)r0 * b, (size_t)rows_c * b);
    }
    tend(te, 1, b1);
    h->rs_wait_all();
  }
  algo_bytes += b0 + b1;
  launches += 2;
}

void GramOp::apply_M_dense(const float* xg, float* Wout) {
  const int64_t ng = (int64_t)h->world * npad;
  const double gb = 4.0 * (double)n * (double)h->n + 4.0 * (double)(ng + n) * b;
  for (int k = 0; k < K; ++k) {
    const LayerDev& L = *h->layers[k];
    const int te = tbeg();
    h->dense_apply(L.dense_at(), L.lda, xg, b, b, zk(k), b, 0.f, nullptr,
                   h->comm ? nullptr : L.dense_a());
    tend(te, 0, gb);
  }
  for (int k = 0; k < K; ++k) {
    const LayerDev& L = *h->layers[k];
    if (h->comm) h->gather_panel(zk(k), gathered_z(k), b);
    const int te = tbeg();
    h->dense_apply(L.dense_a(), L.lda, stage2_in(k), b, b, Wout, b, k == 0 ? 0.f : 1.f, nullptr,
                   h->comm ? nullptr : L.dense_at());
    tend(te, 1, gb);
    algo_bytes += 2.0 * gb;
  }
  launches += 2 * K;
}

void GramOp::apply(const float* X, float* Wout) {
  const double t0 = now_ms();
  lds_poison(st);
  const float* xg = X;
  if (h->comm) {
    float* xgb = h->gath.as<float>();
    h->gather_panel(X, xgb, b);
    xg = xgb;
  }
  if (h->dense_layers()) {
    apply_M_dense(xg, Wout);
  } else if (rs_form) {
    stage1(xg);
    stage2_rs(Wout);
  } else {
    stage1_gathered(xg);
    if (col_blocks)
      stage2_tiled(Wout);
    else
      stage2_flat(Wout);
  }
  t_spmm += now_ms() - t0;
}

}

extern "C" {

int n2v2r_gram_apply(n2v2r_handle* h, int b, const float* X, float* Z, float* W,
                     n2v2r_gram_info* info) {
  return guarded(h, [&]() -> int {
    if (h->multi() || (b != 8 && b != 16 && b != 32 && b != 64) || !X || !W) return N2V2R_ERR_BAD_ARG;
    if (!layers_ready(h)) return N2V2R_ERR_BAD_ARG;
    GramOp op(h);
    op.setup(b);
    hipStream_t st = op.st;
    DevBuf xb, wb;
    xb.ensure(sizeof(float) * op.npad * b, st);
    wb.ensure(sizeof(float) * op.npad * b, st);
    float* x = xb.as<float>();
    float* w = wb.as<float>();
    const size_t rows = sizeof(float) * (size_t)op.n * b;
    HIPCHK(hipMemsetAsync(w, 0xFF, rows, st));
    for (int k = 0; k < op.K; ++k) HIPCHK(hipMemsetAsync(op.zk(k), 0xFF, rows, st));
    if (op.split2)
      for (int k = 0; k < op.K; ++k) HIPCHK(hipMemsetAsync(op.s2part(k), 0xFF, rows, st));
    if (h->comm) {
      HIPCHK(hipMemsetAsync(h->gath.p, 0xFF, h->gath.bytes, st));
      HIPCHK(hipMemsetAsync(h->ews.zg.p, 0xFF, h->ews.zg.bytes, st));
    }
    HIPCHK(hipMemcpyAsync(x, X + (size_t)h->row0 * b, rows, hipMemcpyHostToDevice, st));
    HIPCHK(hipStreamSynchronize(st));
    op.apply(x, w);
    op.materialize();
    HIPCHK(hipMemcpyAsync(W, w, rows, hipMemcpyDeviceToHost, st));
    if (Z)
      for (int k = 0; k < op.K; ++k)
        HIPCHK(hipMemcpyAsync(Z + (size_t)k * op.n * b, op.zk(k), rows, hipMemcpyDeviceToHost,
                              st));
    HIPCHK(hipStreamSynchronize(st));
    if (info) {
      info->form = op.spmm_form();
      info->rs_form = op.rs_form ? 1 : 0;
      info->rs_chunks = op.rs_form ? op.rs_chunks : 0;
      info->split2 = op.split2 ? 1 : 0;
      info->tile_nb = op.col_blocks ? op.tile_nb : 0;
      info->tile_wb = op.col_blocks ? op.tile_wb : 0;
      info->tile_rows = op.col_blocks ? op.tile_rows : 0;
      info->rpw1 = op.rpw1;
      info->rpw2 = op.rpw2;
    }
    return N2V2R_OK;
  });
}

}
```

### node2vec2rank_amd/csrc/gram_op.h

```cpp
#pragma once

#include "engine.h"

namespace n2v2r_int {

bool layers_ready(n2v2r_handle* h);

inline void lds_poison(hipStream_t st) {
  if (debug_poison()) HIPCHK(n2v2r_launch_lds_poison(st));
}

bool col_blocks_wanted(const n2v2r_handle* h, int b);
bool gather_overlap();
bool split2_wanted(const n2v2r_handle* h, int b);

int tile_nb_auto(int64_t nglob);
int tile_rows_for(const n2v2r_handle* h, int wbits);
SpmmTileArgs spmm_tile_args(const CsrBlk* table, int nb, int wbits, int tile_rows, int64_t n,
                            int k0, int nk, int sum, int64_t ldy);

struct GramOp {
  n2v2r_handle* h;
  hipStream_t st;
  int64_t n;
  int64_t npad;
  int K;
  int b = 0;
  bool col_blocks = false;
  int tile_rows = 0, tile_nb = CB_NB, tile_wb = CB_WIN_BITS_MIN;
  bool rs_form = false;
  int rs_chunks = 1;
  int64_t rs_rc = 0;
  bool split2 = false;
  float* pending = nullptr;
  int rpw1 = 0, rpw2 = 0;
  double t_spmm = 0;
  int64_t launches = 0;
  double algo_bytes = 0;
  bool time_spmm = false;
  std::vector<int> tkind;
  std::vector<double> tbytes;

  explicit GramOp(n2v2r_handle* h_)
      : h(h_), st(h_->stream), n(h_->nloc), npad(h_->npad), K(h_->K) {}

  void setup(int b_, bool time_stages = false);
  void apply(const float* X, float* Wout);

  float* zk(int k) const { return h->ews.zk[k]->as<float>(); }
  float* s2part(int k) const { return h->ews.s2part.as<float>() + (size_t)k * npad * 8; }
  void materialize();
  int pending_parts(const float* parts[SPMM_MAX_LAYERS]) const {
    for (int k = 0; k < K; ++k) parts[k] = s2part(k);
    return K;
  }
  void stored() { pending = nullptr; }
  SpmmTileArgs tile_args(bool stage2, int k0, int nk, int sum, int64_t ldy) const {
    return spmm_tile_args(h->ews.tblk.as<CsrBlk>() + (size_t)(stage2 ? K : 0) * tile_nb, tile_nb,
                          tile_wb, tile_rows, n, k0, nk, sum, ldy);
  }
  int spmm_form() const { return h->dense_layers() ? 4 : col_blocks ? 5 : split2 ? 1 : 0; }
  void tsum(n2v2r_eig_stats* out);
  void poison_scratch();

 private:
  int tbeg();
  void tend(int i, int kind, double bytes);
  double layer_bytes(int k, bool transposed) const;
  double stage_bytes(bool transposed) const;
  float* gathered_z(int k) const {
    return h->ews.zg.as<float>() + (size_t)k * h->world * npad * b;
  }
  const float* stage2_in(int k) const { return h->comm ? gathered_z(k) : zk(k); }
  void setup_tiled();
  void setup_stage2_form();
  void stage1(const float* xg, int layer = -1);
  void stage1_gathered(const float* xg);
  void stage2_flat(float* Wout);
  void stage2_tiled(float* Wout);
  void stage2_rs(float* Wout);
  void apply_M_dense(const float* xg, float* Wout);
};

}
```

### node2vec2rank_amd/csrc/layers.cpp

```cpp
#include "engine.h"

using namespace n2v2r_int;

namespace n2v2r_int {
void build_col_blocks(const CsrDev& A, int64_t ncols, LayerDev::ColBlocks& out, hipStream_t st,
                      int nb, int wbits) {
  const int64_t n = A.n_rows;
  const int64_t cw = (ncols + nb - 1) / nb;
  int cbits = 1;
  while (((int64_t)1 << cbits) < cw) ++cbits;
  out.ncols = ncols;
  out.nb = nb;
  out.wbits = wbits;
  out.cbits = cbits + wbits <= 31 ? cbits : 0;
  out.built = true;
  out.usable = false;
  if (n <= 0 || out.cbits == 0) return;
  DevBuf cnt, rp64, tsum;
  cnt.ensure(sizeof(int32_t) * nb * n, st);
  HIPCHK(n2v2r_launch_cb_count(A, cw, nb, cnt.as<int32_t>(), st));
  const int64_t ntiles = n2v2r_cb_scan_tiles(n, nb);
  tsum.ensure(sizeof(int64_t) * ntiles, st);
  rp64.ensure(sizeof(int64_t) * nb * (n + 1), st);
  const int64_t nw1 = ((n + ((int64_t)1 << wbits) - 1) >> wbits) + 1;
  out.wo.ensure(sizeof(int32_t) * nb * nw1, st);
  HIPCHK(n2v2r_launch_cb_rowptrs(cnt.as<int32_t>(), n, nb, A.nnz, tsum.as<int64_t>(),
                                 (size_t)ntiles, rp64.as<int64_t>(), out.wo.as<int32_t>(), wbits,
                                 st));
  std::vector<int64_t> ends(2 * (size_t)nb);
  for (int j = 0; j < nb; ++j) {
    HIPCHK(hipMemcpyAsync(&ends[2 * j], rp64.as<int64_t>() + (size_t)j * (n + 1),
                          sizeof(int64_t), hipMemcpyDeviceToHost, st));
    HIPCHK(hipMemcpyAsync(&ends[2 * j + 1], rp64.as<int64_t>() + (size_t)j * (n + 1) + n,
                          sizeof(int64_t), hipMemcpyDeviceToHost, st));
  }
  HIPCHK(hipStreamSynchronize(st));
  if (ends[2 * (nb - 1) + 1] != A.nnz || ends[0] != 0)
    throw StatusFail{N2V2R_ERR_INTERNAL, "column-block split lost entries"};
  for (int j = 0; j < nb; ++j)
    if (ends[2 * j + 1] - ends[2 * j] > (int64_t)INT32_MAX) return;
  out.idx.ensure(sizeof(int32_t) * std::max<int64_t>(A.nnz, 1), st);
  if (!A.unit) out.dat.ensure(sizeof(float) * std::max<int64_t>(A.nnz, 1), st);
  HIPCHK(n2v2r_launch_cb_fill(A, cw, nb, rp64.as<int64_t>(), out.idx.as<int32_t>(),
                              A.unit ? nullptr : out.dat.as<float>(), out.cbits, wbits, st));
  HIPCHK(hipStreamSynchronize(st));
  for (int j = 0; j < nb; ++j)
    out.blk[j] = CsrBlk{out.wo.as<int32_t>() + (size_t)j * nw1, out.idx.as<int32_t>(),
                        A.unit ? nullptr : out.dat.as<float>(), ends[2 * j], n,
                        ends[2 * j + 1] - ends[2 * j], A.unit, out.cbits, (int64_t)j * cw};
  out.usable = true;
}

bool ensure_col_blocks(LayerDev& L, int64_t ncols, hipStream_t st, int nb, int wbits) {
  auto stale = [&](const LayerDev::ColBlocks& c) {
    return !c.built || c.ncols != ncols || c.nb != nb || c.wbits != wbits;
  };
  if (stale(L.cb)) build_col_blocks(L.csr(), ncols, L.cb, st, nb, wbits);
  if (!L.symmetric && stale(L.cb_t)) build_col_blocks(L.csr_t(), ncols, L.cb_t, st, nb, wbits);
  return L.cb.usable && L.cb.cbits && (L.symmetric || (L.cb_t.usable && L.cb_t.cbits));
}

int tile_wbits(const std::vector<std::unique_ptr<LayerDev>>& layers, int nb) {
  (void)layers;
  (void)nb;
  if (const char* e = std::getenv("N2V2R_SPMM_WBITS")) {
    const int v = std::atoi(e);
    if (v >= CB_WIN_BITS_MIN && v <= CB_WIN_BITS_MAX) return v;
  }
  return 6;
}

void ensure_colcsr(LayerDev& L, int64_t ncols, int64_t rows_out, hipStream_t st, int64_t npad,
                   int W, int64_t rc) {
  if (rc <= 0 || rc >= npad) rc = 0;
  if (L.c_built && L.c_rows == rows_out && L.c_rc == rc) return;
  const CsrDev s = L.csr_t();
  const int64_t nnz = s.nnz;
  if (nnz > (int64_t)INT32_MAX)
    throw StatusFail{N2V2R_ERR_BAD_ARG, "a rank's layer block over 2^31 - 1 entries"};
  L.c_indptr.ensure(sizeof(int64_t) * (rows_out + 1));
  L.c_indices.ensure(sizeof(int32_t) * std::max<int64_t>(nnz, 1));
  if (!s.unit) L.c_data.ensure(sizeof(float) * std::max<int64_t>(nnz, 1));
  if (nnz == 0) {
    HIPCHK(n2v2r_launch_csr_from_sorted(nullptr, nullptr, nullptr, 0, rows_out,
                                        L.c_indptr.as<int64_t>(), nullptr, nullptr, st));
  } else {
    DevBuf keys[2], pay[2], hist, flag;
    for (int i = 0; i < 2; ++i) {
      keys[i].ensure(sizeof(uint64_t) * nnz);
      pay[i].ensure(sizeof(int32_t) * nnz);
    }
    flag.ensure(sizeof(unsigned) * 4, st);
    HIPCHK(hipMemsetAsync(flag.p, 0, sizeof(unsigned) * 4, st));
    HIPCHK(n2v2r_launch_csr_scan(s.indptr, s.indices, s.unit ? nullptr : s.data, s.n_rows,
                                 ncols, keys[0].as<uint64_t>(), pay[0].as<int32_t>(),
                                 flag.as<unsigned>(), st));
    if (rc > 0)
      HIPCHK(n2v2r_launch_chunk_major_keys(keys[0].as<uint64_t>(), nnz, npad, W, rc, st));
    hist.ensure(sizeof(uint32_t) * n2v2r_radix_hist_elems(nnz, 1));
    int bits = 1;
    const int64_t span = rc > 0 ? rows_out : ncols;
    while (bits < 31 && ((int64_t)1 << bits) < span) ++bits;
    int cur = 0;
    for (int sh = 32; sh < 32 + bits; sh += 8) {
      HIPCHK(n2v2r_launch_radix_pass(keys[cur].as<uint64_t>(), pay[cur].as<int32_t>(),
                                     keys[cur ^ 1].as<uint64_t>(), pay[cur ^ 1].as<int32_t>(),
                                     nnz, 1, sh, hist.as<uint32_t>(), st));
      cur ^= 1;
    }
    HIPCHK(n2v2r_launch_csr_from_sorted(keys[cur].as<uint64_t>(), pay[cur].as<int32_t>(), s.data,
                                        nnz, rows_out, L.c_indptr.as<int64_t>(),
                                        L.c_indices.as<int32_t>(),
                                        s.unit ? nullptr : L.c_data.as<float>(), st));
    HIPCHK(hipStreamSynchronize(st));
  }
  L.c_nnz = nnz;
  L.c_rows = rows_out;
  L.c_rc = rc;
  L.c_built = true;
}

int host_threads() {
  return (int)std::min<unsigned>(16u, std::max(1u, std::thread::hardware_concurrency()));
}

// ... 181 lines not shown
    HIPCHK(hipMemsetAsync(flag + 2, 0xFF, sizeof(unsigned), st));
    HIPCHK(n2v2r_launch_corr_bicor(e, n, s, z, flag, st));
  } else if (method == N2V2R_COR_SPEARMAN) {
    ranks.ensure_raw(sizeof(double) * n * s);
    HIPCHK(n2v2r_launch_corr_ranks(e, n, s, ranks.as<double>(), st));
    HIPCHK(n2v2r_launch_corr_standardise(ranks.as<double>(), n, s, z, flag, st));
  } else {
    HIPCHK(n2v2r_launch_corr_standardise(e, n, s, z, flag, st));
  }
  unsigned w[3] = {0, 0, 0};
  HIPCHK(hipMemcpyAsync(w, flag, sizeof(unsigned) * (method == N2V2R_COR_BICOR ? 3 : 1),
                        hipMemcpyDeviceToHost, st));
  HIPCHK(hipStreamSynchronize(st));
  out.bad = w[0];
  if (method == N2V2R_COR_BICOR && w[1] > 0) {
    out.fallback[0] = (int64_t)w[1];
    out.fallback[1] = (int64_t)w[2];
  }
  return out;
}
}

extern "C" {

int n2v2r_set_num_layers(n2v2r_handle* h, int num_layers, int64_t n) {
  if (h && h->multi()) return multi_set_num_layers(h, num_layers, n);
  return guarded(h, [&]() -> int {
    if (num_layers < 1 || n < 1 || n > (int64_t)INT32_MAX) {
      h->set_err("bad layer count %d or node count %lld", num_layers, (long long)n);
      return N2V2R_ERR_BAD_ARG;
    }
    if (num_layers > SPMM_MAX_LAYERS) {
      h->set_err("at most %d layers are supported", SPMM_MAX_LAYERS);
      return N2V2R_ERR_BAD_ARG;
    }
    h->K = num_layers;
    h->set_partition(n);
    h->layers.clear();
    for (int k = 0; k < num_layers; ++k) h->layers.emplace_back(new LayerDev());
    h->have_embedding = false;
    h->ncmp = h->ncols = 0;
    return N2V2R_OK;
  });
}

int n2v2r_set_layer_csr(n2v2r_handle* h, int k, int64_t n, int64_t nnz, const int64_t* indptr,
                        const int32_t* indices, const float* data, int symmetric) {
  if (h && h->multi()) return multi_set_layer_csr(h, k, n, nnz, indptr, indices, data, symmetric);
  return guarded(h, [&]() -> int {
    if (k < 0 || k >= h->K || n != h->n || nnz < 0 || !indptr || (nnz > 0 && (!indices || !data))) {
      h->set_err("bad CSR arguments for layer %d", k);
      return N2V2R_ERR_BAD_ARG;
    }
    if (indptr[0] != 0 || indptr[n] != nnz) {
      h->set_err("layer %d: indptr must start at 0 and end at nnz", k);
      return N2V2R_ERR_BAD_ARG;
    }
    if (symmetric != N2V2R_SYM_YES && nnz > (int64_t)INT32_MAX) {
      h->set_err("layer %d: more than 2^31 - 1 entries need symmetric = N2V2R_SYM_YES (the GPU "
                 "transpose / symmetry test sorts int32 entry indices)", k);
      return N2V2R_ERR_BAD_ARG;
    }
    for (int64_t r = 0; r < n; ++r)
      if (indptr[r + 1] < indptr[r]) {
        h->set_err("layer %d: indptr not monotone", k);
        return N2V2R_ERR_BAD_ARG;
      }
    for (int j = 0; j < h->K; ++j)
      if (j != k && h->layers[j]->loaded && h->layers[j]->dense) {
        h->err = "layers must be all CSR or all dense";
        return N2V2R_ERR_BAD_ARG;
      }
    LayerDev& L = *h->layers[k];
    L.dense = false;
    L.loaded = false;
    L.drop_col_blocks();
    L.n_rows = h->nloc;
    const hipStream_t st = h->stream;
    const bool whole = !h->comm;
    DevBuf gip, gix, gdv;
    DevBuf& dip = whole ? L.indptr : gip;
    DevBuf& dix = whole ? L.indices : gix;
    DevBuf& ddv = whole ? L.data : gdv;
    dip.ensure(sizeof(int64_t) * (n + 1));
    dix.ensure(sizeof(int32_t) * std::max<int64_t>(nnz, 1));
    ddv.ensure(sizeof(float) * std::max<int64_t>(nnz, 1));
    HIPCHK(hipMemcpyAsync(dip.p, indptr, sizeof(int64_t) * (n + 1), hipMemcpyHostToDevice, st));
    const bool ones = nnz > 0 && host_all_ones(nnz, data);
    if (nnz) {
      HIPCHK(hipMemcpyAsync(dix.p, indices, sizeof(int32_t) * nnz, hipMemcpyHostToDevice, st));
      if (ones)
        HIPCHK(hipMemsetD32Async((hipDeviceptr_t)ddv.p, 0x3F800000, (size_t)nnz, st));
      else
        HIPCHK(hipMemcpyAsync(ddv.p, data, sizeof(float) * nnz, hipMemcpyHostToDevice, st));
    }
    h->h2d_layer_bytes += 8 * (n + 1) + (ones ? 4 : 8) * nnz;
    const bool need_t = symmetric != N2V2R_SYM_YES;
    DevBuf* keys = h->ing_keys;
    DevBuf* pay = h->ing_pay;
    DevBuf& hist = h->ing_hist;
    DevBuf& flag = h->ing_flag;
    flag.ensure_raw(sizeof(unsigned) * 4);
    HIPCHK(hipMemsetAsync(flag.p, 0, sizeof(unsigned) * 4, st));
    if (need_t && nnz) {
      keys[0].ensure_raw(sizeof(uint64_t) * nnz);
      pay[0].ensure_raw(sizeof(int32_t) * nnz);
    }
    HIPCHK(n2v2r_launch_csr_scan(dip.as<int64_t>(), dix.as<int32_t>(), ddv.as<float>(), n, n,
                                 need_t && nnz ? keys[0].as<uint64_t>() : nullptr,
                                 need_t && nnz ? pay[0].as<int32_t>() : nullptr,
                                 flag.as<unsigned>(), st));
    unsigned fl = 0;
    HIPCHK(hipMemcpyAsync(&fl, flag.p, sizeof(unsigned), hipMemcpyDeviceToHost, st));
    HIPCHK(hipStreamSynchronize(st));
    if (fl & 1u) {
      h->set_err("layer %d: column index out of range", k);
      return N2V2R_ERR_BAD_ARG;
    }
    const bool unit = !(fl & 2u);
    const bool sorted = !(fl & 4u);
    auto transpose = [&](const int64_t* ip_, const int32_t* ix_, const float* dv_, bool have_keys,
                         DevBuf& tp, DevBuf& tx, DevBuf& td) {
      tp.ensure(sizeof(int64_t) * (n + 1));
      tx.ensure(sizeof(int32_t) * std::max<int64_t>(nnz, 1));
      if (!unit) td.ensure(sizeof(float) * std::max<int64_t>(nnz, 1));
      if (nnz == 0) {
        HIPCHK(n2v2r_launch_csr_from_sorted(nullptr, nullptr, nullptr, 0, n, tp.as<int64_t>(),
                                            nullptr, nullptr, st));
        return;
      }
      keys[0].ensure_raw(sizeof(uint64_t) * nnz);
      pay[0].ensure_raw(sizeof(int32_t) * nnz);
      keys[1].ensure_raw(sizeof(uint64_t) * nnz);
      pay[1].ensure_raw(sizeof(int32_t) * nnz);
      if (!have_keys)
        HIPCHK(n2v2r_launch_csr_scan(ip_, ix_, dv_, n, n, keys[0].as<uint64_t>(),
                                     pay[0].as<int32_t>(), flag.as<unsigned>() + 1, st));
      hist.ensure_raw(sizeof(uint32_t) * n2v2r_radix_hist_elems(nnz, 1));
      int bits = 1;
      while (bits < 31 && ((int64_t)1 << bits) < n) ++bits;
      int cur = 0;
      for (int sh = 32; sh < 32 + bits; sh += 8) {
        HIPCHK(n2v2r_launch_radix_pass(keys[cur].as<uint64_t>(), pay[cur].as<int32_t>(),
                                       keys[cur ^ 1].as<uint64_t>(), pay[cur ^ 1].as<int32_t>(),
                                       nnz, 1, sh, hist.as<uint32_t>(), st));
        cur ^= 1;
      }
      HIPCHK(n2v2r_launch_csr_from_sorted(keys[cur].as<uint64_t>(), pay[cur].as<int32_t>(), dv_,
                                          nnz, n, tp.as<int64_t>(), tx.as<int32_t>(),
                                          unit ? nullptr : td.as<float>(), st));
    };
    bool sym = symmetric == N2V2R_SYM_YES;
    DevBuf gtp, gtx, gtd;
    DevBuf& tp = whole ? L.t_indptr : gtp;
    DevBuf& tx = whole ? L.t_indices : gtx;
    DevBuf& td = whole ? L.t_data : gtd;
    if (need_t) {
      transpose(dip.as<int64_t>(), dix.as<int32_t>(), ddv.as<float>(), true, tp, tx, td);
      if (symmetric == N2V2R_SYM_DETECT) {
        const float* tv = unit ? ddv.as<float>() : td.as<float>();
        HIPCHK(hipMemsetAsync(flag.as<unsigned>() + 2, 0, sizeof(unsigned), st));
        if (sorted) {
          HIPCHK(n2v2r_launch_csr_compare(dip.as<int64_t>(), dix.as<int32_t>(), ddv.as<float>(),
                                          tp.as<int64_t>(), tx.as<int32_t>(), tv, n, nnz,
                                          flag.as<unsigned>() + 2, st));
        } else {
          DevBuf sp_, sx, sv;
          transpose(tp.as<int64_t>(), tx.as<int32_t>(), tv, false, sp_, sx, sv);
          HIPCHK(n2v2r_launch_csr_compare(sp_.as<int64_t>(), sx.as<int32_t>(),
                                          unit ? ddv.as<float>() : sv.as<float>(),
                                          tp.as<int64_t>(), tx.as<int32_t>(), tv, n, nnz,
                                          flag.as<unsigned>() + 2, st));
          HIPCHK(hipStreamSynchronize(st));
        }
        unsigned mism = 0;
        HIPCHK(hipMemcpyAsync(&mism, flag.as<unsigned>() + 2, sizeof(unsigned),
                              hipMemcpyDeviceToHost, st));
        HIPCHK(hipStreamSynchronize(st));
        sym = mism == 0;
      }
    }
    HIPCHK(hipStreamSynchronize(st));
    keys[0].release();
    keys[1].release();
    pay[0].release();
    pay[1].release();
    auto slice = [&](DevBuf& sip, DevBuf& six, DevBuf& sdv, bool copy_values, DevBuf& oip,
                     DevBuf& oix, DevBuf& odv, int64_t& onnz) {
      int64_t p0 = 0, p1 = 0;
      HIPCHK(hipMemcpyAsync(&p0, sip.as<int64_t>() + h->row0, sizeof(int64_t),
                            hipMemcpyDeviceToHost, st));
      HIPCHK(hipMemcpyAsync(&p1, sip.as<int64_t>() + h->row0 + h->nloc, sizeof(int64_t),
                            hipMemcpyDeviceToHost, st));
      HIPCHK(hipStreamSynchronize(st));
      onnz = p1 - p0;
      oip.ensure(sizeof(int64_t) * (h->nloc + 1));
      oix.ensure(sizeof(int32_t) * std::max<int64_t>(onnz, 1));
      odv.ensure(sizeof(float) * std::max<int64_t>(onnz, 1));
      HIPCHK(n2v2r_launch_csr_rebase(sip.as<int64_t>(), h->row0, h->nloc, oip.as<int64_t>(), st));
      if (onnz) {
        HIPCHK(hipMemcpyAsync(oix.p, six.as<int32_t>() + p0, sizeof(int32_t) * onnz,
                              hipMemcpyDeviceToDevice, st));
        if (copy_values)
          HIPCHK(hipMemcpyAsync(odv.p, sdv.as<float>() + p0, sizeof(float) * onnz,
                                hipMemcpyDeviceToDevice, st));
      }
      HIPCHK(hipStreamSynchronize(st));
    };
    if (whole) {
      L.nnz = nnz;
      L.t_nnz = nnz;
      if (sym) {
        L.t_indptr.release();
        L.t_indices.release();
        L.t_data.release();
      }
    } else {
      slice(gip, gix, gdv, true, L.indptr, L.indices, L.data, L.nnz);
      if (!sym) slice(gtp, gtx, gtd, !unit, L.t_indptr, L.t_indices, L.t_data, L.t_nnz);
    }
    L.unit = unit;
    L.t_unit = unit;
    L.symmetric = sym;
    L.loaded = true;
    h->have_embedding = false;
    return N2V2R_OK;
  });
}

int n2v2r_set_layer_dense(n2v2r_handle* h, int k, int64_t n, const float* A, int symmetric) {
  if (h && h->multi()) return multi_set_layer_dense(h, k, n, A, symmetric);
  return guarded(h, [&]() -> int {
    if (k < 0 || k >= h->K || n != h->n || !A) {
      h->set_err("bad dense arguments for layer %d", k);
      return N2V2R_ERR_BAD_ARG;
    }
    for (int j = 0; j < h->K; ++j)
      if (j != k && h->layers[j]->loaded && !h->layers[j]->dense) {
        h->err = "layers must be all CSR or all dense";
        return N2V2R_ERR_BAD_ARG;
      }
    LayerDev& L = *h->layers[k];
    L.dense = true;
    L.n_rows = h->nloc;
    L.lda = (n + 63) / 64 * 64;
    const int64_t nl = std::max<int64_t>(h->nloc, 1);
    L.dA.ensure(sizeof(float) * nl * L.lda);
    HIPCHK(hipMemcpy2D(L.dA.p, sizeof(float) * L.lda, A + h->row0 * n, sizeof(float) * n,
                       sizeof(float) * n, h->nloc, hipMemcpyHostToDevice));
    bool sym = symmetric == N2V2R_SYM_YES;
    if (!sym) {
      DevBuf full;
      const float* src = L.dA.as<float>();
      if (h->comm) {
        full.ensure(sizeof(float) * n * L.lda);
        HIPCHK(hipMemcpy2D(full.p, sizeof(float) * L.lda, A, sizeof(float) * n,
                           sizeof(float) * n, n, hipMemcpyHostToDevice));
        src = full.as<float>();
      }
      L.dAT.ensure(sizeof(float) * nl * L.lda);
      HIPCHK(n2v2r_launch_transpose(src + h->row0, L.lda, n, h->nloc, L.dAT.as<float>(), L.lda,
                                    h->stream));
      if (symmetric == N2V2R_SYM_DETECT) {
        DevBuf cnt;
        cnt.ensure(sizeof(unsigned long long));
        HIPCHK(n2v2r_launch_mismatch(L.dA.as<float>(), L.dAT.as<float>(), L.lda, h->nloc, n,
                                     cnt.as<unsigned long long>(), h->stream));
        unsigned long long mism = 0;
        HIPCHK(hipMemcpyAsync(&mism, cnt.p, sizeof(mism), hipMemcpyDeviceToHost, h->stream));
        HIPCHK(hipStreamSynchronize(h->stream));
        sym = mism == 0;
      }
      HIPCHK(hipStreamSynchronize(h->stream));
      if (sym) L.dAT.release();
    }
    L.symmetric = sym;
    L.loaded = true;
    h->have_embedding = false;
    return N2V2R_OK;
  });
}

int n2v2r_set_layer_corr(n2v2r_handle* h, int k, int64_t n, int64_t samples, const double* E,
                         int kind, double power) {
  return n2v2r_set_layer_corr_method(h, k, n, samples, E, kind, power, N2V2R_COR_PEARSON, nullptr);
}

int n2v2r_set_layer_corr_method(n2v2r_handle* h, int k, int64_t n, int64_t samples,
                                const double* E, int kind, double power, int method,
                                int64_t* fallback) {
  if (h && h->multi())
    return multi_set_layer_corr(h, k, n, samples, E, kind, power, method, fallback);
  return guarded(h, [&]() -> int {
    if (k < 0 || k >= h->K || n != h->n || n < 1 || !E) {
      h->set_err("bad co-expression arguments for layer %d", k);
      return N2V2R_ERR_BAD_ARG;
    }
    LayerDev& L = *h->layers[k];
    L.loaded = false;
// ... 317 lines not shown
    return nullptr;
  }
  return h->layers[k].get();
}
}

extern "C" {

int n2v2r_layers_to_csr(n2v2r_handle* h, int64_t* nnz) {
  if (h && h->multi()) return multi_layers_to_csr(h, nnz);
  return guarded(h, [&]() -> int {
    if (const int st = sparsify_refusal(h, "layers_to_csr")) return st;
    const int K = h->K;
    hipStream_t st = h->stream;
    DevBuf red;
    if (h->comm) red.ensure_raw(sizeof(unsigned long long) * (K + 1));
    std::vector<CsrBuild> a(K), t(K);
    int fail = N2V2R_OK;
    std::string why;
    try {
      DevBuf cnt;
      for (int k = 0; k < K; ++k) {
        const LayerDev& L = *h->layers[k];
        sparsify_count(h, L.dA.as<float>(), L.lda, cnt, a[k]);
        if (!L.symmetric) sparsify_count(h, L.dAT.as<float>(), L.lda, cnt, t[k]);
      }
      for (int k = 0; k < K; ++k)
        for (CsrBuild* b : {&a[k], &t[k]}) {
          if (b == &t[k] && h->layers[k]->symmetric) continue;
          b->ix.ensure_raw(sizeof(int32_t) * std::max<int64_t>(b->nnz, 1));
          b->dv.ensure_raw(sizeof(float) * std::max<int64_t>(b->nnz, 1));
        }
      for (int k = 0; k < K; ++k) {
        const LayerDev& L = *h->layers[k];
        for (CsrBuild* b : {&a[k], &t[k]}) {
          const bool tr = b == &t[k];
          if (tr && L.symmetric) continue;
          if (b->unit && b->nnz)
            HIPCHK(hipMemsetD32Async((hipDeviceptr_t)b->dv.p, 0x3F800000, (size_t)b->nnz, st));
          HIPCHK(n2v2r_launch_dense_row_compact((tr ? L.dAT : L.dA).as<float>(), h->nloc, L.lda,
                                                h->n, b->ip.as<int64_t>(), b->ix.as<int32_t>(),
                                                b->unit ? nullptr : b->dv.as<float>(), st));
        }
      }
      HIPCHK(hipStreamSynchronize(st));
    } catch (const StatusFail& sf) {
      fail = sf.code;
      why = sf.msg;
      (void)hipGetLastError();
    } catch (const HipFail& hf) {
      fail = N2V2R_ERR_HIP;
      why = std::string("HIP error (") + hipGetErrorString(hf.e) + ") at " + hf.where;
      (void)hipGetLastError();
    }
    std::vector<unsigned long long> tot(K + 1);
    for (int k = 0; k < K; ++k) tot[k] = fail ? 0ull : (unsigned long long)a[k].nnz;
    tot[K] = (unsigned long long)fail;
    if (h->comm) {
      unsigned long long* r = red.as<unsigned long long>();
      HIPCHK(hipMemcpyAsync(r, tot.data(), sizeof(unsigned long long) * (K + 1),
                            hipMemcpyHostToDevice, st));
      h->comm->allreduce_sum_u64(r, K, st);
      h->comm->allreduce_max_u64(r + K, 1, st);
      HIPCHK(hipMemcpyAsync(tot.data(), r, sizeof(unsigned long long) * (K + 1),
                            hipMemcpyDeviceToHost, st));
      HIPCHK(hipStreamSynchronize(st));
    }
    if (tot[K] != N2V2R_OK) {
      if (fail)
        h->err = "layers_to_csr: " + why;
      else
        h->set_err("layers_to_csr: another rank failed (status %d); nothing was converted",
                   (int)tot[K]);
      return fail ? fail : (int)tot[K];
    }
    for (int k = 0; k < K; ++k) {
      LayerDev& L = *h->layers[k];
      L.drop_col_blocks();
      L.indptr.swap(a[k].ip);
      L.indices.swap(a[k].ix);
      L.data.swap(a[k].dv);
      L.nnz = a[k].nnz;
      L.unit = a[k].unit;
      if (L.symmetric) {
        L.t_indptr.release();
        L.t_indices.release();
        L.t_data.release();
        L.t_nnz = L.nnz;
        L.t_unit = L.unit;
      } else {
        L.t_indptr.swap(t[k].ip);
        L.t_indices.swap(t[k].ix);
        L.t_data.swap(t[k].dv);
        L.t_nnz = t[k].nnz;
        L.t_unit = t[k].unit;
      }
      L.n_rows = h->nloc;
      L.dense = false;
      L.dA.release();
      L.dAT.release();
      if (nnz) nnz[k] = (int64_t)tot[k];
    }
    h->tom_out.release();
    h->dense_work.release();
    h->dense_work_elems = 0;
    h->have_embedding = false;
    return N2V2R_OK;
  });
}

int n2v2r_count_layer_nonzeros(n2v2r_handle* h, int64_t* nnz) {
  if (h && h->multi()) return multi_count_layer_nonzeros(h, nnz);
  return guarded(h, [&]() -> int {
    if (!nnz) {
      h->err = "count_layer_nonzeros: null output buffer";
      return N2V2R_ERR_BAD_ARG;
    }
    if (const int st = sparsify_refusal(h, "count_layer_nonzeros")) return st;
    const int K = h->K;
    hipStream_t st = h->stream;
    std::vector<unsigned long long> tot(K);
    DevBuf cnt;
    for (int k = 0; k < K; ++k) {
      CsrBuild b;
      sparsify_count(h, h->layers[k]->dA.as<float>(), h->layers[k]->lda, cnt, b);
      tot[k] = (unsigned long long)b.nnz;
    }
    if (h->comm) {
      DevBuf red;
      red.ensure_raw(sizeof(unsigned long long) * K);
      unsigned long long* r = red.as<unsigned long long>();
      HIPCHK(hipMemcpyAsync(r, tot.data(), sizeof(unsigned long long) * K, hipMemcpyHostToDevice,
                            st));
      h->comm->allreduce_sum_u64(r, K, st);
      HIPCHK(hipMemcpyAsync(tot.data(), r, sizeof(unsigned long long) * K, hipMemcpyDeviceToHost,
                            st));
      HIPCHK(hipStreamSynchronize(st));
    }
    for (int k = 0; k < K; ++k) nnz[k] = (int64_t)tot[k];
    return N2V2R_OK;
  });
}

int n2v2r_get_layer_csr_nnz(n2v2r_handle* h, int k, int transpose, int64_t* nnz) {
  if (h && h->multi()) return multi_get_layer_csr_nnz(h, k, transpose, nnz);
  return guarded(h, [&]() -> int {
    const LayerDev* L = nnz ? csr_layer_for_read(h, k, transpose) : nullptr;
    if (!L) {
      if (!nnz) h->err = "get_layer_csr_nnz: null output";
      return N2V2R_ERR_BAD_ARG;
    }
    *nnz = transpose ? L->t_nnz : L->nnz;
    return N2V2R_OK;
  });
}

int n2v2r_get_layer_csr(n2v2r_handle* h, int k, int transpose, int64_t* indptr, int32_t* indices,
                        float* data) {
  if (h && h->multi()) return multi_get_layer_csr(h, k, transpose, indptr, indices, data);
  return guarded(h, [&]() -> int {
    const LayerDev* L = indptr ? csr_layer_for_read(h, k, transpose) : nullptr;
    if (!L) {
      if (!indptr) h->err = "get_layer_csr: null output buffer";
      return N2V2R_ERR_BAD_ARG;
    }
    const CsrDev c = transpose ? L->csr_t() : L->csr();
    if (c.nnz > 0 && (!indices || !data)) {
      h->err = "get_layer_csr: null output buffer";
      return N2V2R_ERR_BAD_ARG;
    }
    HIPCHK(hipStreamSynchronize(h->stream));
    HIPCHK(hipMemcpy(indptr, c.indptr, sizeof(int64_t) * (c.n_rows + 1), hipMemcpyDeviceToHost));
    if (c.nnz > 0) {
      HIPCHK(hipMemcpy(indices, c.indices, sizeof(int32_t) * c.nnz, hipMemcpyDeviceToHost));
      if (c.unit)
        std::fill(data, data + c.nnz, 1.0f);
// ... 476 lines not shown
```

### node2vec2rank_amd/csrc/solver.cpp

```cpp
#include "gram_op.h"

#include <optional>

using namespace n2v2r_int;

namespace n2v2r_int {
constexpr int kAutoMaxc = 640;

struct BasisPlan {
  int b, keep, maxc;
};
BasisPlan plan_basis(int d, int64_t nglob, int block_opt, int keep_opt, int max_basis_opt,
                     bool dense_rr, bool dense_layers) {
  int b = block_opt ? block_opt : (dense_layers ? 32 : 8);
  if (b != 8 && b != 16 && b != 32 && b != 64)
    throw StatusFail{N2V2R_ERR_BAD_ARG, "block must be 8, 16, 32 or 64"};
  int keep = 0, maxc = 0;
  const bool dense_rule = dense_layers && !block_opt;
  const bool big_graph = !dense_rule && nglob >= ((int64_t)1 << 22) && d <= 160;
  for (;; b /= 2) {
    keep = keep_opt ? keep_opt : (dense_rule ? d + b : std::max(d + 16, (d * 21) / 16));
    keep = ((keep + b - 1) / b) * b;
    if (!keep_opt && !dense_rule && b == 8 && keep > 184 && std::max(d + 16, (d * 5) / 4) <= 184)
      keep = 184;
// ... 26 lines not shown
}

struct ReadBack {
  enum Flag { kRefilled = 1, kRrErr = 2, kSecondSolves = 3, kTriErr = 4 };
  static constexpr int nrr = 64, nsl = 8;
  int wres = 0, wth = 0, wflag = 0, wrr = 0, wsl = 0, words = 0;
  void lay_out(int keep) {
    wth = wres + 2 * keep;
    wflag = wth + 2 * keep;
    wrr = wflag + 8;
    wsl = wrr + 2 * nrr;
    words = wsl + nsl * keep;
  }
  size_t bytes(int upto_word) const { return sizeof(int32_t) * (size_t)upto_word; }
  template <class T>
  T* at(void* pin, int word) const {
    return reinterpret_cast<T*>(static_cast<int32_t*>(pin) + word);
  }
};

bool pair_apply_launches(const BlockList& all, double* g2, int64_t n, const PipPass& pa,
                         const PipPass& pz, int* plan, size_t plan_bytes, hipStream_t st) {
  const int nq_old = all.count - 2;
  float* za = const_cast<float*>(all.blk[nq_old]);
  float* zb = const_cast<float*>(all.blk[nq_old + 1]);
  BlockList q = all;
  q.count = nq_old;
  if (plan) {
    const hipError_t pe = n2v2r_launch_pip_pair(q, za, zb, g2, n, pa.flags, pa.any_flag, pa.sticky,
                                                pa.seed, pz.seed, pa.row0, pa.skip_tol, pa.skipped,
                                                plan, plan_bytes, st);
    if (pe == hipSuccess) return true;
    if (pe != hipErrorNotSupported) throw HipFail{pe, "n2v2r_launch_pip_pair"};
  }
  HIPCHK(n2v2r_launch_pip_fused(q, za, za, g2, nq_old * 8, n, pa, st));
  HIPCHK(n2v2r_launch_pair_fixup(g2, nq_old + 2, nq_old, pa.rsave, st));
  q.count = nq_old + 1;
  HIPCHK(n2v2r_launch_pip_fused(q, zb, zb, g2 + (size_t)(nq_old + 2) * 64, (nq_old + 1) * 8, n, pz,
                                st));
  return false;
}

struct Eig {
  n2v2r_handle* h;
  hipStream_t st;
  int64_t n;
  int64_t npad;
  int64_t row0;
  int K;
  GramOp op;
  int b = 0;
  int nb_max = 0;
  int pb = 0;
  int d = 0;
  uint64_t seed = 0;
  std::vector<float*> freelist;
  std::vector<float*> Q, W;
  n2v2r_eig_stats* stats = nullptr;
  double t_ortho = 0;
  uint64_t fill_counter = 0;
  int kry0 = 0;
  bool full_first = false;
  bool band_rr = false;
  bool band_reduce = false;
  bool y_captured = false;
  bool ritz_done = false;
  int ritz_launches = 0;
  int stats_rr_fallbacks = 0;
  int* tri_err = nullptr;
  bool tri_single = false;
  int tri_fallbacks = 0;
  bool lean_off = false;
  float reorth_tol = 0.f;
  bool defer = false;
  bool pair_apply = false;
  float* deferred = nullptr;
  struct LeanRetry {};
  explicit Eig(n2v2r_handle* h_)
      : h(h_), st(h_->stream), n(h_->nloc), npad(h_->npad), row0(h_->row0), K(h_->K), op(h_) {}

  int flags = 0;
  bool flag(int f) const { return (flags & f) != 0; }
  int keep = 0, c_max = 0;
  double tol = 0, stag_cap = 0;
  int max_restarts = 0;
  bool sturm = false;
  bool lean = false;
  bool lazy = true;
  ReadBack rb;
  int cycle = 0, apps = 0, conv = 0, stagnated = 0, lean_checks = 0;
  double maxres = 0, t_start = 0, t_rr = 0;
  double est_scale = 1.0;
  double last_true = 1e300;
  bool rr_armed = false;
  bool tri_test_armed = false;
  std::vector<float*> X, MX;
  float* E_lean = nullptr;
  std::vector<double> wh, res2, hist_res;

  double* part_p = nullptr;
  size_t part_n = 0;
  double* gsm_p = nullptr;
  int* flg_p = nullptr;
  int* any_p = nullptr;

  int dbg_cycle = 0, dbg_apps = 0;
  void dbg(const void* p, int64_t count, bool f64, const char* what) {
    if (!debug_finite() || !p || count <= 0) return;
    int* flag = h->ews.dbgflag.as<int>();
    HIPCHK(hipMemsetAsync(flag, 0, sizeof(int), st));
    HIPCHK(n2v2r_launch_nonfinite(p, count, f64 ? 1 : 0, flag, st));
    int bad = 0;
    HIPCHK(hipMemcpyAsync(&bad, flag, sizeof(int), hipMemcpyDeviceToHost, st));
    HIPCHK(hipStreamSynchronize(st));
    if (bad) {
      const std::string msg = std::string("non-finite values first seen in ") + what +
                              " (cycle " + std::to_string(dbg_cycle) + ", block application " +
                              std::to_string(dbg_apps) + ", b " + std::to_string(b) + ")";
      fprintf(stderr, "[n2v2r] %s\n", msg.c_str());
      throw StatusFail{N2V2R_ERR_INTERNAL, msg};
    }
  }
  void dbg_ortho(float* z, const std::vector<float*>& basis, const char* what,
                 const int* flags = nullptr) {
    if (!debug_ortho()) return;
    std::vector<float*> all(basis);
    all.push_back(z);
    const int nq = (int)all.size();
    DevBuf g;
    g.ensure(sizeof(double) * (size_t)nq * b * b);
    tn(blocks(all, 0, nq), one(z), g.as<double>(), nullptr);
    std::vector<double> hg((size_t)nq * b * b);
    HIPCHK(hipMemcpyAsync(hg.data(), g.p, sizeof(double) * hg.size(), hipMemcpyDeviceToHost, st));
    HIPCHK(hipStreamSynchronize(st));
    double off = 0.0, self = 0.0, nrm = 0.0;
    for (int r = 0; r < nq * b; ++r)
      for (int j = 0; j < b; ++j) {
        const double v = hg[(size_t)r * b + j];
        if (r >= (nq - 1) * b) {
          const int i = r - (nq - 1) * b;
          self = std::max(self, std::fabs(v - (i == j ? 1.0 : 0.0)));
          if (i == j) nrm = std::max(nrm, v);
        } else {
          off = std::max(off, std::fabs(v));
        }
      }
    int fl[8] = {};
    if (flags) {
      HIPCHK(hipMemcpyAsync(fl, flags, sizeof(fl), hipMemcpyDeviceToHost, st));
      HIPCHK(hipStreamSynchronize(st));
    }
    if (off > 1e-3 || self > 1e-3)
      fprintf(stderr, "[n2v2r] %s: cycle %d, application %d, basis %d blocks: |Q^T z| %.3e, "
              "|z^T z - I| %.3e, max z_j^T z_j %.3e%s flags %d%d%d%d%d%d%d%d\n", what,
              dbg_cycle, dbg_apps, nq - 1, off, self, nrm, deferred == z ? " (deferred)" : "",
              fl[0], fl[1], fl[2], fl[3], fl[4], fl[5], fl[6], fl[7]);
  }

  void poison_scratch() {
    if (!debug_poison()) return;
    EigWorkspace& w = h->ews;
    for (DevBuf* d : {&w.rinv, &w.flg, &w.anyflag, &w.gsmall, &w.csmall, &w.tri, &w.refl,
                      &w.ytri, &w.tscr, &w.hband, &w.band, &w.varr, &w.taua, &w.rrerr, &w.fcoef,
                      &h->partial, &h->theta, &h->resid})
      if (d->p) HIPCHK(hipMemsetAsync(d->p, 0xFF, d->bytes, st));
    for (auto& d : w.pool) HIPCHK(hipMemsetAsync(d->p, 0xFF, d->bytes, st));
    op.poison_scratch();
  }

  float* take() {
    if (freelist.empty()) {
      h->ews.pool.emplace_back(new DevBuf());
      h->ews.pool.back()->ensure(sizeof(float) * npad * b, st);
      return h->ews.pool.back()->as<float>();
    }
    float* p = freelist.back();
    freelist.pop_back();
    return p;
  }
  void give(float* p) {
    if (p) freelist.push_back(p);
  }

  BlockList blocks(const std::vector<float*>& v, int from, int count) const {
    BlockList L{};
    L.count = count;
    L.width = b;
    for (int i = 0; i < count; ++i) L.blk[i] = v[from + i];
    return L;
  }
  BlockList one(const float* p) const {
    BlockList L{};
    L.count = 1;
    L.width = b;
    L.blk[0] = p;
    return L;
  }
  OutBlockList out_one(float* p) const {
    OutBlockList L{};
    L.count = 1;
    L.width = b;
    L.blk[0] = p;
    return L;
  }

  void tn(const BlockList& A, const BlockList& B, double* out, const int* cond) {
    HIPCHK(n2v2r_launch_ts_tn(A, B, n, part_p, part_n, out, cond, st));
    if (h->comm)
      h->allreduce_f64(out, (size_t)A.count * A.width * B.count * B.width);
  }


  uint64_t last_fill_seed = 0;
  uint64_t next_fill_seed() { return last_fill_seed = seed ^ (0xABCDull + ++fill_counter); }

  PipPass pass_in_slot(int s) const {
    PipPass p;
    p.flags = flg_p + 64 * s;
    p.any_flag = any_p + s;
    p.row0 = row0;
    return p;
  }
  const std::vector<float*>& first_blocks(const std::vector<float*>& basis,
                                          const std::vector<float*>* local) const {
    return local && !full_first && local->size() < basis.size() ? *local : basis;
  }
  PipPass first_pass(const std::vector<float*>& first, const std::vector<float*>* local,
                     double* save, int* sticky, double* rsave) const {
    const int nsave = (save && local) ? (int)local->size() : 0;
    PipPass p = pass_in_slot(0);
    p.first = 1;
    p.save = nsave ? save : nullptr;
    p.save_row0 = ((int)first.size() - nsave) * b;
    p.save_rows = nsave * b;
    p.sticky = sticky;
    p.rsave = rsave;
    return p;
  }
  PipPass selective_pass(int* sticky, double* rsave = nullptr) const {
    PipPass p = pass_in_slot(1);
    p.skip_tol = reorth_tol;
    p.skipped = reorth_tol != 0.f ? h->ews.skipc.as<int>() : nullptr;
    p.sticky = sticky;
    p.rsave = rsave;
    return p;
  }
  PipPass third_pass() const {
    PipPass p = pass_in_slot(2);
    p.cond = any_p + 1;
    return p;
  }

  void pip_pass(float* Z, const std::vector<float*>& basis, PipPass p,
                const float* Zin = nullptr) {
    p.seed = next_fill_seed();
    const float* zin = Zin ? Zin : Z;
    const int nq = (int)basis.size();
    std::vector<float*> qz(basis);
    qz.push_back(const_cast<float*>(zin));
    const BlockList L = blocks(qz, 0, nq + 1);
    bool done = false;
    if (op.pending && zin == op.pending && !p.cond && !h->comm) {
      const float* parts[SPMM_MAX_LAYERS];
      const int np = op.pending_parts(parts);
// ... 58 lines not shown
    const auto it = std::find(basis.begin(), basis.end(), deferred);
    if (it == basis.end()) throw StatusFail{N2V2R_ERR_INTERNAL, "deferred block left the basis"};
    const std::vector<float*> pre(basis.begin(), it);
    const double t0 = now_ms();
    if (!pre.empty()) pip_pass(deferred, pre, selective_pass(any_p + 3));
    t_ortho += now_ms() - t0;
    deferred = nullptr;
  }

  bool pair_pass(float* zb, const std::vector<float*>& basis) {
    if (!deferred || basis.empty() || basis.back() != deferred) return false;
    const int nq_old = (int)basis.size() - 1;
    if (nq_old + 2 > N2V2R_MAX_BLOCKS || (nq_old + 1) * 8 > N2V2R_BAND_MAXC) return false;
    std::vector<float*> all(basis);
    all.push_back(zb);
    if (h->ews.g2.bytes < sizeof(double) * 2 * (size_t)(nq_old + 2) * 64) return false;
    double* g2 = h->ews.g2.as<double>();
    const double t0 = now_ms();
    lds_poison(st);
    const BlockList L = blocks(all, 0, nq_old + 2);
    const hipError_t e = n2v2r_launch_ts_tn2(L, deferred, zb, n, part_p, part_n, g2, st);
    if (e == hipErrorNotSupported) return false;
    if (e != hipSuccess) throw HipFail{e, "n2v2r_launch_ts_tn2"};
    if (h->comm) h->allreduce_f64(g2, 2 * (size_t)(nq_old + 2) * 64);
    PipPass pa = selective_pass(any_p + 3, h->ews.pair_ra.as<double>()),
            pz = selective_pass(any_p + 3);
    pa.seed = next_fill_seed();
    pz.seed = next_fill_seed();
    pair_apply_launches(L, g2, n, pa, pz, pair_apply ? h->ews.pair_plan.as<int>() : nullptr,
                        h->ews.pair_plan.bytes, st);
    t_ortho += now_ms() - t0;
    deferred = nullptr;
    return true;
  }

  std::vector<float*> local_of(const std::vector<float*>& basis) const {
    const int last = (int)basis.size() - 1;
    const int lo = last <= kry0 ? 0 : last - 1;
    return std::vector<float*>(basis.begin() + lo, basis.end());
  }

  size_t band_off(int j) const {
    if (j == kry0) return 0;
    return (size_t)(kry0 * b + b) * b + (size_t)(j - kry0 - 1) * 2 * b * b;
  }

  void expand_one(const float* w_from, const std::vector<float*>& basis, std::vector<float*>& qs,
                  std::vector<float*>& ws, bool save_band = false, bool lazy = false) {
    float* z = take();
    const std::vector<float*> loc = local_of(basis);
    double* save = (save_band && band_rr)
                       ? h->ews.hband.as<double>() + band_off((int)basis.size() - 1)
                       : nullptr;
    if (defer && lazy && !full_first) {
      const double t0 = now_ms();
      lds_poison(st);
      const std::vector<float*>& first = first_blocks(basis, &loc);
      pip_pass(z, first, first_pass(first, &loc, save, any_p + 3, nullptr), w_from);
      t_ortho += now_ms() - t0;
      if (deferred && pair_pass(z, basis)) {
      } else if (deferred) {
        flush_deferred(basis);
        const double t1 = now_ms();
        pip_pass(z, basis, selective_pass(any_p + 3));
        t_ortho += now_ms() - t1;
      } else {
        deferred = z;
      }
    } else {
      orthonormalize(z, basis, w_from, &loc, save, lazy);
    }
    dbg(z, n * b, false, "orthonormalised Krylov block");
    dbg_ortho(z, basis, "Krylov block before its SpMM");
    float* w = take();
    op.apply(z, w);
    if (debug_finite()) op.materialize();
    dbg(w, n * b, false, "SpMM image M q");
    ++dbg_apps;
    qs.push_back(z);
    ws.push_back(w);
  }


  void reuse_pool() {
    const size_t bb = sizeof(float) * npad * b;
    if (h->ews.block_bytes != bb) {
      h->ews.pool.clear();
      h->ews.block_bytes = bb;
    }
    freelist.clear();
    for (auto& blk : h->ews.pool) freelist.push_back(blk->as<float>());
  }

  void size_scratch() {
    h->partial_elems = std::max<size_t>(4096ull * 1024ull, (size_t)c_max * c_max * 8);
    h->partial_elems = std::max<size_t>(h->partial_elems,
                                        (size_t)((n + 8191) / 8192 + 24) * 2 * (c_max + 2 * b) * b);
    h->partial.ensure(sizeof(double) * h->partial_elems);
    h->ews.gsmall.ensure(sizeof(double) * (size_t)c_max * c_max);
    h->ews.csmall.ensure(sizeof(float) * (size_t)c_max * c_max);
    h->ews.tri.ensure(sizeof(double) * 3 * (size_t)c_max);
    h->ews.refl.ensure(sizeof(double) * std::max<size_t>((size_t)c_max * c_max,
                                                        (size_t)c_max * (c_max / 8 + 2) * 9));
    h->ews.ytri.ensure(sizeof(double) * (size_t)c_max * keep);
    h->ews.tscr.ensure(sizeof(double) * 6 * (size_t)((keep + 63) / 64 * 64) * c_max);
    h->ews.trcoop.ensure(n2v2r_rr_tridiag_scratch_bytes(c_max));
    h->ews.btf.ensure(n2v2r_rr_bt_scratch_bytes(c_max));
    h->ews.rinv.ensure(sizeof(double) * 64 * 64);
    h->ews.fcoef.ensure(sizeof(float) * (size_t)(c_max + 64) * 64);
    h->ews.flg.ensure(sizeof(int) * 256);
    h->ews.anyflag.ensure(sizeof(int) * 4);
    h->theta.ensure(sizeof(double) * c_max);
    h->resid.ensure(sizeof(double) * c_max);
    band_reduce = rr_reduce_fits(keep, c_max);
    band_rr = b == 8 && !flag(N2V2R_EIG_DENSE_RR) && c_max <= N2V2R_BAND_MAXC &&
              (band_reduce || rr_sturm_enabled());
    if (band_rr) {
      h->ews.hband.ensure(sizeof(double) * ((size_t)(keep + b) * b + (size_t)nb_max * 2 * b * b));
      h->ews.band.ensure(sizeof(double) * (size_t)c_max * (b + 1));
      h->ews.varr.ensure(sizeof(double) * (size_t)(keep + b) * (keep + b));
      h->ews.taua.ensure(sizeof(double) * (size_t)(keep + b));
      h->ews.rrerr.ensure(sizeof(int) * 4);
      h->ews.sturm.ensure(sizeof(double) * n2v2r_rr_sturm_scratch(c_max, keep));
    }
    sturm = band_rr && rr_sturm_enabled();
    part_p = h->partial.as<double>();
    part_n = h->partial_elems;
    gsm_p = h->ews.gsmall.as<double>();
    flg_p = h->ews.flg.as<int>();
    any_p = h->ews.anyflag.as<int>();
    lean = b == 8 && band_rr && sturm && !lean_off && lean_enabled();
    h->ews.skipc.ensure(sizeof(int) * (4 + N2V2R_BAND_MAXC / 8));
    HIPCHK(hipMemsetAsync(h->ews.skipc.p, 0, sizeof(int) * (4 + N2V2R_BAND_MAXC / 8), st));
    if (lean) h->ews.rres.ensure(sizeof(double) * 128);
    rb.lay_out(keep);
    h->ews.dbgflag.ensure(sizeof(int) * 4);
    h->ews.tflag.ensure(sizeof(double) * 2);
    wh.assign(keep, 0.0);
    res2.assign(keep, 0.0);
  }

  void set_plan(int b_, int keep_, int nblk) {
    b = b_;
    keep = keep_;
    pb = keep / b;
    nb_max = nblk;
    c_max = nblk * b;
    reuse_pool();
    size_scratch();
  }

  void read_reorth_switches() {
    const char* rt = std::getenv("N2V2R_REORTH_TOL");
    reorth_tol = rt ? (float)std::atof(rt) : (float)std::min(0.1 * tol, 1e-6);
    const char* e = std::getenv("N2V2R_REORTH_DEFER");
    defer = !(e && e[0] == '0') && lean;
    deferred = nullptr;
    const char* pa = std::getenv("N2V2R_PAIR_APPLY");
    pair_apply = pa && std::strcmp(pa, "fused") == 0   ? true
                 : pa && std::strcmp(pa, "split") == 0 ? false
                                                       : n >= (int64_t)1 << 19;
    if (defer) {
      h->ews.g2.ensure(sizeof(double) * 2 * (size_t)(nb_max + 2) * 64, st);
      static const double eye[64] = {1, 0, 0, 0, 0, 0, 0, 0, 0, 1, 0, 0, 0, 0, 0, 0,
                                     0, 0, 1, 0, 0, 0, 0, 0, 0, 0, 0, 1, 0, 0, 0, 0,
                                     0, 0, 0, 0, 1, 0, 0, 0, 0, 0, 0, 0, 0, 1, 0, 0,
                                     0, 0, 0, 0, 0, 0, 1, 0, 0, 0, 0, 0, 0, 0, 0, 1};
      h->ews.pair_ra.ensure(sizeof(double) * 64, st);
      h->ews.pair_plan.ensure(sizeof(int) * N2V2R_PAIR_PLAN_WORDS, st);
      HIPCHK(hipMemcpyAsync(h->ews.pair_ra.p, eye, sizeof(eye), hipMemcpyHostToDevice, st));
      HIPCHK(hipStreamSynchronize(st));
    }
  }


  static bool trace() {
    static const bool v = [] {
      const char* e = std::getenv("N2V2R_TRACE");
      return e && *e && *e != '0';
    }();
    return v;
  }

  double launch_rr(RrForm form, int nq) {
    const int c = nq * b;
    double* trid = h->ews.tri.as<double>();
    op.materialize();
    const double tr0 = now_ms();
    lds_poison(st);
    if (banded(form)) {
      const std::vector<float*> loc = local_of(Q);
      tn(blocks(loc, 0, (int)loc.size()), one(W.back()),
         h->ews.hband.as<double>() + band_off(nq - 1), nullptr);
      if (!rr_armed) HIPCHK(hipMemsetAsync(h->ews.rrerr.as<int>(), 0, 4 * sizeof(int), st));
      rr_armed = true;
      lds_poison(st);
      if (form == RrForm::Sturm) {
        HIPCHK(n2v2r_launch_rr_sturm(h->ews.hband.as<double>(), c, kry0 * b,
                                     h->theta.as<double>(), h->ews.sturm.as<double>(),
                                     h->ews.sturm.bytes / sizeof(double),
                                     h->ews.ytri.as<double>(), h->ews.csmall.as<float>(), keep,
                                     keep, h->ews.rrerr.as<int>(), st));
      } else {
        HIPCHK(n2v2r_launch_rr_band(h->ews.hband.as<double>(), c, kry0 * b, h->theta.as<double>(),
                                    h->ews.band.as<double>(), h->ews.varr.as<double>(),
                                    h->ews.taua.as<double>(), trid, trid + c_max,
                                    h->ews.refl.as<double>(), h->ews.ytri.as<double>(),
                                    h->ews.csmall.as<float>(), keep, keep,
                                    h->ews.rrerr.as<int>(), st));
      }
    } else {
      if (form == RrForm::DenseFromBand) {
        HIPCHK(n2v2r_launch_rr_band_expand(h->ews.hband.as<double>(), c, kry0 * b,
                                           h->ews.sturm.as<double>() + 4,
                                           h->ews.gsmall.as<double>(), st));
      } else {
        tn(blocks(Q, 0, nq), blocks(W, 0, nq), h->ews.gsmall.as<double>(), nullptr);
      }
      dbg(h->ews.gsmall.p, (int64_t)c * c, true, "projected matrix H = Q^T W");
      lds_poison(st);
// ... 141 lines not shown
    if (!banded(form)) {
      bool timed_out = pflag[ReadBack::kTriErr] != 0;
      if (tri_test_armed && tri_err && !tri_single) {
        timed_out = true;
        tri_test_armed = false;
      }
      if (h->comm) {
        double* fl = h->ews.tflag.as<double>();
        const double mine = timed_out ? 1.0 : 0.0;
        HIPCHK(hipMemcpyAsync(fl, &mine, sizeof(double), hipMemcpyHostToDevice, st));
        h->allreduce_f64(fl, 1);
        double any_to = 0.0;
        HIPCHK(hipMemcpyAsync(&any_to, fl, sizeof(double), hipMemcpyDeviceToHost, st));
        HIPCHK(hipStreamSynchronize(st));
        timed_out = any_to > 0.0;
      }
      if (!timed_out) return std::nullopt;
      fprintf(stderr, "[n2v2r] multi-workgroup tridiagonalisation timed out at cycle %d (c %d); "
                      "one-workgroup kernel from here on\n", cycle, c);
      tri_single = true;
      ++tri_fallbacks;
      return form;
    }
    const bool failed = pflag[ReadBack::kRrErr] != 0 || flag(N2V2R_EIG_TEST_BAND_FAIL) ||
                        (flag(N2V2R_EIG_TEST_STURM_FAIL) && form == RrForm::Sturm);
    if (form == RrForm::Sturm) {
      if (trace())
        fprintf(stderr, "[n2v2r] cycle %d: %d of %d Ritz vectors took a second solve\n", cycle,
                pflag[ReadBack::kSecondSolves], keep);
      if (!failed) return std::nullopt;
      if (trace()) fprintf(stderr, "[n2v2r] Sturm Rayleigh-Ritz failed, reducing fallback\n");
      ++stats_rr_fallbacks;
      const RrForm next = rr_after_sturm(keep, c_max);
      if (next == RrForm::DenseFromBand) return next;
      if (kry0 > 0)
        HIPCHK(hipMemcpyAsync(h->theta.as<double>(), h->ews.sturm.as<double>() + 4,
                              sizeof(double) * kry0 * b, hipMemcpyDeviceToDevice, st));
      return RrForm::BandReduce;
    }
    if (!failed) return std::nullopt;
    if (lean) throw LeanRetry{};
    if (trace()) fprintf(stderr, "[n2v2r] banded Rayleigh-Ritz failed, dense fallback\n");
    return RrForm::Dense;
  }

  int nonfinite_pair() const {
    for (int j = 0; j < keep; ++j)
      if (!std::isfinite(wh[j]) || (j < d && !std::isfinite(res2[j]))) return j;
    return -1;
  }

  void drop_cycle(int q_start) {
    const int nq = (int)Q.size();
    give(E_lean);
    for (int q = 0; q < pb; ++q) {
      give(X[q]);
      give(MX[q]);
    }
    for (int q = q_start; q < nq; ++q) {
      give(Q[q]);
      give(W[q]);
    }
    apps -= nq - q_start;
    Q.resize(q_start);
    W.resize(q_start);
  }

  bool residuals_flat() {
    hist_res.push_back(maxres);
    const size_t W8 = 8;
    if (hist_res.size() < 2 * W8) return false;
    const double recent = *std::min_element(hist_res.end() - W8, hist_res.end());
    const double before = *std::min_element(hist_res.begin(), hist_res.end() - W8);
    return !flag(N2V2R_EIG_TEST_NO_STAGNATION) && recent > 0.9 * before && recent <= 100.0 * tol;
  }

  bool lean_final_check(double th1, int ldu) {
    ++lean_checks;
    const int qd = (d + b - 1) / b;
    std::vector<float*> MV(qd);
    const char* ycv = std::getenv("N2V2R_YCAP");
    const bool cap = op.col_blocks && !h->comm && b == 8 && qd * b == ldu &&
                     !(ycv && ycv[0] == '0');
    if (cap) h->Y.ensure(sizeof(float) * (size_t)K * npad * ldu, st);
    for (int q = 0; q < qd; ++q) {
      MV[q] = take();
      op.apply(X[q], MV[q]);
      op.materialize();
      if (cap)
        for (int k = 0; k < K; ++k)
          HIPCHK(hipMemcpy2DAsync(h->Y.as<float>() + (size_t)k * npad * ldu + (size_t)q * b,
                                  sizeof(float) * ldu, op.zk(k),
                                  sizeof(float) * b, sizeof(float) * b, n,
                                  hipMemcpyDeviceToDevice, st));
    }
    y_captured = cap;
    double* pres = rb.at<double>(h->pin, rb.wres);
    HIPCHK(n2v2r_launch_resid(blocks(X, 0, qd), blocks(MV, 0, qd), h->theta.as<double>(), n,
                              h->partial.as<double>(), h->partial_elems,
                              h->resid.as<double>(), st));
    h->allreduce_f64(h->resid.as<double>(), (size_t)qd * b);
    HIPCHK(hipMemcpyAsync(pres, h->resid.as<double>(), sizeof(double) * qd * b,
                          hipMemcpyDeviceToHost, st));
    HIPCHK(hipStreamSynchronize(st));
    for (float* p : MV) give(p);
    double worst = 0.0, est_max = 0.0;
    int tconv = 0;
    for (int j = 0; j < d; ++j) {
      const double r = std::sqrt(std::max(pres[j], 0.0)) / th1;
      const double e = std::sqrt(std::max(res2[j], 0.0)) / th1;
      worst = std::max(worst, r);
      est_max = std::max(est_max, e);
      if (r <= tol) ++tconv;
    }
    const double ratio = est_max > 0.0 ? worst / est_max : 0.0;
    if (trace())
      fprintf(stderr, "[n2v2r] cycle %d: true max_res %.3e converged %d/%d (estimate %.3e)\n",
              cycle, worst, tconv, d, maxres);
    maxres = worst;
    conv = tconv;
    stagnated = 0;
    bool done = true;
    if (conv < d && cycle + 1 < max_restarts) {
      const bool flat = lean_checks >= 2 && worst > 0.9 * last_true;
      if (!flag(N2V2R_EIG_TEST_NO_STAGNATION) && (flat || lean_checks >= 4) &&
          worst <= 100.0 * tol) {
        stagnated = 1;
      } else {
        done = false;
        if (ratio > 0.0) est_scale = std::min(1e3, std::max(1.0, est_scale * 1.25 * ratio));
        hist_res.clear();
      }
    }
    last_true = worst;
    return done;
  }

  void restart() {
    std::vector<float*> E, EW;
    if (lean) {
      E.push_back(E_lean);
      EW.push_back(take());
      op.apply(E_lean, EW[0]);
    } else {
      expand_one(W.back(), Q, E, EW);
    }
    ++apps;
    for (float* p : Q) give(p);
    for (float* p : W) give(p);
    Q.assign(X.begin(), X.end());
    W.assign(MX.begin(), MX.end());
    Q.insert(Q.end(), E.begin(), E.end());
    W.insert(W.end(), EW.begin(), EW.end());
    kry0 = pb;
  }

  void fill_stats() {
    if (!stats) return;
    stats->restarts = cycle + 1;
    stats->block_applications = apps;
    stats->converged = conv;
    stats->basis = c_max;
    stats->max_residual = maxres;
    stats->ms_total = now_ms() - t_start;
    stats->ms_spmm = op.t_spmm;
    stats->ms_ortho = t_ortho;
    stats->ms_rr_host = t_rr;
    stats->spmm_launches = op.launches;
    stats->spmm_algo_bytes = op.algo_bytes;
    stats->stagnated = stagnated;
    stats->rr_fallbacks = stats_rr_fallbacks;
    stats->est_scale = est_scale;
    stats->lean_checks = lean_checks;
    stats->pool_blocks = (int)h->ews.pool.size();
    stats->spmm_form = op.spmm_form();
    stats->stag_cap = stag_cap;
    stats->y_captured = y_captured ? 1 : 0;
    stats->tri_fallbacks = tri_fallbacks;
    op.tsum(stats);
  }

  int run(int d_, const n2v2r_eig_opts& o, std::vector<double>& theta_out, float* Uout,
          int ldu) {
    d = d_;
    seed = o.seed ? o.seed : 0x5EEDull;
    flags = o.solver_flags;
    full_first = flag(N2V2R_EIG_FULL_FIRST_PASS);
    tri_test_armed = flag(N2V2R_EIG_TEST_TRI_TIMEOUT);
    kry0 = 0;
    tol = o.tol > 0 ? o.tol : 1e-6;
    max_restarts = o.max_restarts > 0 ? o.max_restarts : 2000;
    const BasisPlan plan = plan_basis(d, h->n, o.block, o.keep, o.max_basis,
                                      flag(N2V2R_EIG_DENSE_RR), h->dense_layers());
    b = plan.b;
    keep = plan.keep;
    c_max = plan.maxc;
    pb = keep / b;
    nb_max = c_max / b;
    stag_cap = 2.0 * std::max(tol, std::sqrt((double)c_max) * 0x1p-24);
    reuse_pool();
    op.setup(b, flag(N2V2R_EIG_TIME_SPMM));
    size_scratch();
    read_reorth_switches();
    poison_scratch();

    float* q0 = take();
    HIPCHK(n2v2r_launch_fill_normal(q0, b, n, seed, nullptr, nullptr, (uint64_t)row0 * b, st));
    Q.assign(1, q0);
    orthonormalize(q0, {});
    dbg(q0, n * b, false, "orthonormalised start block");
    W.assign(1, take());
    op.apply(Q[0], W[0]);
    if (debug_finite()) op.materialize();
    dbg(W[0], n * b, false, "SpMM image of the start block");
    if (flag(N2V2R_EIG_TEST_FAIL_ALONE) && h->comm && h->rank == 1)
      throw StatusFail{N2V2R_ERR_INTERNAL, "test: rank 1 fails alone"};
    apps = 1;
    X.assign(pb, nullptr);
    MX.assign(pb, nullptr);
    t_start = now_ms();
    for (cycle = 0;; ++cycle) {
      dbg_cycle = cycle;
      y_captured = false;
      const int q_start = (int)Q.size();
      if (lazy && cycle == 0) HIPCHK(hipMemsetAsync(h->ews.anyflag.as<int>() + 3, 0, sizeof(int), st));
      while ((int)Q.size() < nb_max) {
        expand_one(W.back(), Q, Q, W, true, lazy);
        ++apps;
        if (lean && (int)W.size() - 2 > q_start - 1) {
          give(W[W.size() - 2]);
          W[W.size() - 2] = nullptr;
        }
      }
      flush_deferred(Q);
      const int nq = (int)Q.size();
      const int c = nq * b;
      for (int q = 0; q < pb; ++q) {
        X[q] = take();
        MX[q] = lean ? nullptr : take();
      }
      E_lean = nullptr;
      RrForm form = !band_rr ? RrForm::Dense : sturm ? RrForm::Sturm : RrForm::BandReduce;
      for (;;) {
        const double tr0 = launch_rr(form, nq);
        const double to0 = now_ms();
        ritz_vectors(nq);
        launch_residuals();
        read_back(form, c, tr0);
        read_estimates();
        t_ortho += now_ms() - to0;
        const std::optional<RrForm> next = rr_next(form, c);
        if (!next) break;
        form = *next;
      }
      int refilled = lazy ? rb.at<int>(h->pin, rb.wflag)[ReadBack::kRefilled] : 0;
      if (flag(N2V2R_EIG_TEST_REDO_CYCLE) && cycle == 0 && lazy) refilled = 1;
      const int bad = nonfinite_pair();
      if (lazy && !refilled && bad >= 0) {
        fprintf(stderr,
                "[n2v2r] WARNING: non-finite Ritz pair %d at cycle %d (c %d, b %d, %s "
                "Rayleigh-Ritz); cycle expanded again with three passes.  Rerun with "
                "N2V2R_DEBUG_FINITE=1 to locate the stage.\n",
                bad, cycle, c, b, banded(form) ? "banded" : "dense");
        refilled = 1;
      }
      if (refilled) {
        if (trace()) fprintf(stderr, "[n2v2r] rank-deficient block, cycle %d expanded again\n", cycle);
        drop_cycle(q_start);
        lazy = false;
        --cycle;
        continue;
      }
      if (bad >= 0)
        throw StatusFail{N2V2R_ERR_NO_CONVERGENCE,
                         "non-finite Ritz pair " + std::to_string(bad) + " at cycle " +
                             std::to_string(cycle) + " (c " + std::to_string(c) + ", b " +
                             std::to_string(b) + (banded(form) ? ", banded" : ", dense") +
                             " Rayleigh-Ritz, theta " + std::to_string(wh[bad]) + ")"};
      maxres = 0;
      conv = 0;
      const double th1 = std::max(wh[0], 1e-300);
      for (int j = 0; j < d; ++j) {
        const double r = std::sqrt(std::max(res2[j], 0.0)) / th1;
        maxres = std::max(maxres, r);
        if (r <= tol) ++conv;
// ... 84 lines not shown
                          h->stream));
    HIPCHK(hipStreamSynchronize(h->stream));
    for (int j = 0; j < d; ++j) sc[j] *= sgn[j];
  }
  HIPCHK(hipMemcpyAsync(h->colscale.p, sc.data(), sizeof(float) * ldu, hipMemcpyHostToDevice,
                        h->stream));
  const float* ug = h->U.as<float>();
  DevBuf ugath;
  if (h->comm) {
    ugath.ensure(sizeof(float) * h->world * h->npad * ldu);
    h->gather_panel(h->U.as<float>(), ugath.as<float>(), ldu);
    ug = ugath.as<float>();
  }
  h->Y.ensure(sizeof(float) * (size_t)h->K * h->npad * ldu);
  if (h->dense_layers()) {
    for (int k = 0; k < h->K; ++k) {
      const LayerDev& L = *h->layers[k];
      for (int q = 0; q * 64 < ldu; ++q)
        h->dense_apply(L.dense_at(), L.lda, ug + q * 64, ldu, std::min(64, ldu - q * 64),
                       h->Y.as<float>() + (size_t)k * h->npad * ldu + q * 64, ldu, 0.f,
                       h->colscale.as<float>() + q * 64);
      if (info) info->launches += (ldu + 63) / 64;
    }
  }
  if (!h->dense_layers() && tiled) {
    const int64_t ng = h->comm ? (int64_t)h->world * h->npad : h->npad;
    DevBuf& panel = h->ypanel;
    panel.ensure_raw(sizeof(float) * ng * 8);
    SpmmTileArgs a = op.tile_args(false, 0, h->K, 0, ldu);
    for (int q = 0; !captured && q * 8 < ldu; ++q) {
      HIPCHK(hipMemcpy2DAsync(panel.p, sizeof(float) * 8, ug + q * 8, sizeof(float) * ldu,
                              sizeof(float) * 8, ng, hipMemcpyDeviceToDevice, h->stream));
      for (int k = 0; k < h->K; ++k) {
        a.X[k] = panel.as<float>();
        a.Y[k] = h->Y.as<float>() + (size_t)k * h->npad * ldu + q * 8;
      }
      HIPCHK(n2v2r_launch_spmm_tile(a, h->stream));
      if (info) ++info->launches;
    }
    for (int k = 0; k < h->K; ++k)
      HIPCHK(n2v2r_launch_scale_cols(h->Y.as<float>() + (size_t)k * h->npad * ldu, ldu,
                                     h->npad, h->colscale.as<float>(), h->stream));
    HIPCHK(hipStreamSynchronize(h->stream));
  }
  for (int q = 0; !h->dense_layers() && !tiled && q * b < ldu; ++q) {
    SpmmArgs a{};
    a.K = h->K;
    a.sum = 0;
    a.ldx = ldu;
    a.ldy = ldu;
    a.colscale = h->colscale.as<float>() + q * b;
    for (int k = 0; k < h->K; ++k) {
      a.A[k] = h->layers[k]->csr_t();
      a.X[k] = ug + q * b;
      a.Y[k] = h->Y.as<float>() + (size_t)k * h->npad * ldu + q * b;
    }
    HIPCHK(n2v2r_launch_spmm(a, b, h->stream));
    if (info) {
      ++info->launches;
      info->rpw = n2v2r_spmm_rpw(a, b);
    }
  }
  HIPCHK(hipStreamSynchronize(h->stream));
}
}

extern "C" {

int n2v2r_uase(n2v2r_handle* h, int d, const n2v2r_eig_opts* opts, n2v2r_eig_stats* stats) {
  if (h && h->multi()) return multi_uase(h, d, opts, stats);
  return guarded(h, [&]() -> int {
    if (!layers_ready(h)) return N2V2R_ERR_BAD_ARG;
    if (d < 1 || d > 600 || d >= h->n) {
      h->set_err("embedding dimension %d out of range [1, min(600, n-1)]", d);
      return N2V2R_ERR_BAD_ARG;
    }
    n2v2r_eig_opts o{};
    if (opts) o = *opts;
    if (stats) memset(stats, 0, sizeof(*stats));
    h->have_embedding = false;
    h->ncmp = h->ncols = 0;
    h->have_borda = false;
    for (DevBuf* b : {&h->ing_keys[0], &h->ing_keys[1], &h->ing_pay[0], &h->ing_pay[1],
                      &h->ing_hist})
      b->release();
    const int ldu = ((d + 63) / 64) * 64;
    h->U.ensure(sizeof(float) * h->npad * ldu);
    HIPCHK(hipMemsetAsync(h->U.p, 0, sizeof(float) * h->npad * ldu, h->stream));
    std::vector<double> theta;
    int st = 0;
    std::optional<Eig> eig;
    for (int attempt = 0;; ++attempt) {
      eig.emplace(h);
      eig->stats = stats;
      eig->lean_off = attempt > 0;
      try {
        st = eig->run(d, o, theta, h->U.as<float>(), ldu);
      } catch (const Eig::LeanRetry&) {
        fprintf(stderr, "[n2v2r] banded Rayleigh-Ritz failed under lean images; fit rerun\n");
        HIPCHK(hipStreamSynchronize(h->stream));
        continue;
      }
      break;
    }
    build_embedding(h, eig->op, theta, ldu, eig->y_captured);
    h->have_embedding = true;
    h->ncmp = h->ncols = 0;
    if (st != N2V2R_OK)
      h->set_err("UASE did not converge: max residual %.3e (tol %.1e%s)",
                 stats ? stats->max_residual : -1.0, o.tol > 0 ? o.tol : 1e-6,
                 stats && stats->stagnated ? "; stopped flat above the fp32-floor cap" : "");
    return st;
  });
}

int n2v2r_embed_step(n2v2r_handle* h, int b, int d, const float* U, const double* theta,
                     n2v2r_embed_info* info) {
  if (info) {
    *info = n2v2r_embed_info{};
    info->form = -1;
  }
  return guarded(h, [&]() -> int {
    if (h->multi() || (b != 8 && b != 16 && b != 32 && b != 64) || !U || !theta)
      return N2V2R_ERR_BAD_ARG;
    if (!layers_ready(h)) return N2V2R_ERR_BAD_ARG;
    if (d < 1 || d > 600 || d >= h->n) {
      h->set_err("embedding dimension %d out of range [1, min(600, n-1)]", d);
      return N2V2R_ERR_BAD_ARG;
    }
    GramOp op(h);
    op.setup(b);
    hipStream_t st = h->stream;
    h->have_embedding = false;
    h->ncmp = h->ncols = 0;
    h->have_borda = false;
    const int ldu = ((d + 63) / 64) * 64;
    h->U.ensure(sizeof(float) * h->npad * ldu);
    HIPCHK(hipMemsetAsync(h->U.p, 0, sizeof(float) * h->npad * ldu, st));
    if (h->nloc > 0)
      HIPCHK(hipMemcpy2DAsync(h->U.p, sizeof(float) * ldu, U + (size_t)h->row0 * d,
                              sizeof(float) * d, sizeof(float) * d, h->nloc,
                              hipMemcpyHostToDevice, st));
    h->keys.ensure(sizeof(unsigned long long) * 1024 * (size_t)ldu);
    h->best.ensure(sizeof(unsigned long long) * ldu);
    h->colscale.ensure(sizeof(float) * ldu);
    h->Y.ensure(sizeof(float) * (size_t)h->K * h->npad * ldu);
    HIPCHK(hipMemsetAsync(h->keys.p, 0xFF, sizeof(unsigned long long) * 1024 * (size_t)ldu, st));
    HIPCHK(hipMemsetAsync(h->best.p, 0xFF, sizeof(unsigned long long) * ldu, st));
    HIPCHK(hipMemsetAsync(h->colscale.p, 0xFF, sizeof(float) * ldu, st));
    for (int k = 0; k < h->K && h->nloc > 0; ++k)
      HIPCHK(hipMemsetAsync(h->Y.as<float>() + (size_t)k * h->npad * ldu, 0xFF,
                            sizeof(float) * h->nloc * ldu, st));
    HIPCHK(hipStreamSynchronize(st));
    build_embedding(h, op, std::vector<double>(theta, theta + d), ldu, false, info);
    h->have_embedding = true;
    h->ncmp = h->ncols = 0;
    return N2V2R_OK;
  });
}

int n2v2r_ritz_step(n2v2r_handle* h, int b, int nq, int keep, int lean, const float* Q,
                    const float* W, const float* S, const double* theta, float* X, float* MX,
                    double* res, n2v2r_ritz_info* info) {
  return guarded(h, [&]() -> int {
    if (h->multi() || (b != 8 && b != 16 && b != 32 && b != 64) || nq < 1 || keep < b ||
        keep % b != 0 || (int64_t)keep + b > (int64_t)nq * b || (int64_t)nq * b > N2V2R_BAND_MAXC ||
        (lean && b != 8) || !Q || !S || !theta || !X || (!lean && (!W || !MX || !res)))
// ... 72 lines not shown
    if (na < 1 || nb < 1 || !A || !B || !G) return N2V2R_ERR_BAD_ARG;
    Eig eig(h);
    if (const int s = diag_eig(h, b, std::max(na, nb), eig)) return s;
    if (const int s = diag_gram_info(eig, na, nb, info)) return s;
    hipStream_t st = eig.st;
    const size_t rows = sizeof(float) * (size_t)eig.n * b;
    std::vector<float*> a, bb;
    for (int q = 0; q < na; ++q) {
      a.push_back(eig.take());
      HIPCHK(hipMemcpyAsync(a[q], A + (size_t)q * eig.n * b, rows, hipMemcpyHostToDevice, st));
    }
    for (int q = 0; q < nb; ++q) {
      bb.push_back(eig.take());
      HIPCHK(hipMemcpyAsync(bb[q], B + (size_t)q * eig.n * b, rows, hipMemcpyHostToDevice, st));
    }
    const size_t gbytes = sizeof(double) * (size_t)na * b * nb * b;
    HIPCHK(hipMemsetAsync(eig.gsm_p, 0xFF, gbytes, st));
    HIPCHK(hipMemsetAsync(eig.part_p, 0xFF, h->partial.bytes, st));
    HIPCHK(hipStreamSynchronize(st));
    eig.tn(eig.blocks(a, 0, na), eig.blocks(bb, 0, nb), eig.gsm_p, nullptr);
    HIPCHK(hipMemcpyAsync(G, eig.gsm_p, gbytes, hipMemcpyDeviceToHost, st));
    HIPCHK(hipStreamSynchronize(st));
    return N2V2R_OK;
  });
}

int n2v2r_ortho_pass(n2v2r_handle* h, int b, int nq, const float* Q, float* Z, int in_place,
                     int first, int cond, uint64_t seed, double* gram, double* xinv, float* F,
                     int* flags, int* any_flag, n2v2r_pass_info* info) {
  return guarded(h, [&]() -> int {
    if (nq < 0 || (nq > 0 && !Q) || !Z || !gram || !flags || !any_flag || cond < -1 || cond > 1 ||
        (b != 8 && (!xinv || !F)))
      return N2V2R_ERR_BAD_ARG;
    Eig eig(h);
    if (const int s = diag_eig(h, b, nq + 1, eig)) return s;
    if (const int s = diag_gram_info(eig, nq + 1, 1, info)) return s;
    const int c = nq * b;
    const int kern = b == 8 ? 0 : n2v2r_nn_kernel(nq + 1, b, b);
    if (kern < 0) return N2V2R_ERR_BAD_ARG;
    eig.seed = seed;
    hipStream_t st = eig.st;
    const size_t rows = sizeof(float) * (size_t)eig.n * b;
    std::vector<float*> basis;
    for (int q = 0; q < nq; ++q) {
      basis.push_back(eig.take());
      HIPCHK(hipMemcpyAsync(basis[q], Q + (size_t)q * eig.n * b, rows, hipMemcpyHostToDevice, st));
    }
    float* zin = eig.take();
    float* z = in_place ? zin : eig.take();
    HIPCHK(hipMemcpyAsync(zin, Z, rows, hipMemcpyHostToDevice, st));
    if (!in_place) HIPCHK(hipMemsetAsync(z, 0xFF, rows, st));
    const size_t gbytes = sizeof(double) * (size_t)(c + b) * b;
    HIPCHK(hipMemsetAsync(eig.gsm_p, 0xFF, gbytes, st));
    HIPCHK(hipMemsetAsync(eig.part_p, 0xFF, h->partial.bytes, st));
    HIPCHK(hipMemsetAsync(h->ews.rinv.p, 0xFF, h->ews.rinv.bytes, st));
    HIPCHK(hipMemsetAsync(h->ews.fcoef.p, 0xFF, h->ews.fcoef.bytes, st));
    HIPCHK(hipMemsetAsync(eig.flg_p, 0x5A, sizeof(int) * 256, st));
    HIPCHK(hipMemsetAsync(eig.any_p, 0x5A, sizeof(int) * 4, st));
    PipPass p = cond >= 0 ? eig.third_pass() : eig.pass_in_slot(first ? 0 : 1);
    p.first = first;
    if (cond >= 0)
      HIPCHK(hipMemcpyAsync(const_cast<int*>(p.cond), &cond, sizeof(int), hipMemcpyHostToDevice, st));
    HIPCHK(hipStreamSynchronize(st));
    eig.pip_pass(z, basis, p, in_place ? nullptr : zin);
    HIPCHK(hipMemcpyAsync(Z, z, rows, hipMemcpyDeviceToHost, st));
    HIPCHK(hipMemcpyAsync(gram, eig.gsm_p, gbytes, hipMemcpyDeviceToHost, st));
    if (b != 8) {
      HIPCHK(hipMemcpyAsync(xinv, h->ews.rinv.p, sizeof(double) * b * b, hipMemcpyDeviceToHost, st));
      HIPCHK(hipMemcpyAsync(F, h->ews.fcoef.p, sizeof(float) * (size_t)(c + b) * b,
                            hipMemcpyDeviceToHost, st));
    }
    HIPCHK(hipMemcpyAsync(flags, p.flags, sizeof(int) * b, hipMemcpyDeviceToHost, st));
    HIPCHK(hipMemcpyAsync(any_flag, p.any_flag, sizeof(int), hipMemcpyDeviceToHost, st));
    HIPCHK(hipStreamSynchronize(st));
    if (info) {
      if (b != 8) n2v2r_pip_chol_plan(c, b, 1, &info->stage, &info->nwg);
      info->apply_kernel = kern;
      info->fill_seed = eig.last_fill_seed;
    }
    return N2V2R_OK;
  });
}

int n2v2r_get_embedding(n2v2r_handle* h, float* Y) {
  if (h && h->multi()) return multi_get_embedding(h, Y);
  return guarded(h, [&]() -> int {
    if (!h->have_embedding) {
      h->err = "No n2v2r embeddings found";
      return N2V2R_ERR_NOT_READY;
    }
    copy_embedding(h, Y, (int64_t)h->nloc * h->d);
    return N2V2R_OK;
  });
}

int n2v2r_get_left_embedding(n2v2r_handle* h, float* X) {
  if (h && h->multi()) return multi_get_left_embedding(h, X);
  return guarded(h, [&]() -> int {
    if (!h->have_embedding || h->U.p == nullptr) {
      h->err = "No n2v2r embeddings found";
      return N2V2R_ERR_NOT_READY;
    }
    HIPCHK(hipMemcpy2DAsync(X, sizeof(float) * h->d, h->U.as<float>(), sizeof(float) * h->ldy,
                            sizeof(float) * h->d, h->nloc, hipMemcpyDeviceToHost, h->stream));
    HIPCHK(hipStreamSynchronize(h->stream));
    for (int64_t i = 0; i < h->nloc; ++i)
      for (int j = 0; j < h->d; ++j) X[i * h->d + j] *= (float)std::sqrt(h->sigma[j]);
    return N2V2R_OK;
  });
}

int n2v2r_get_singular_values(n2v2r_handle* h, double* s) {
  if (h && h->multi()) h = h->ranks[0];
  return guarded(h, [&]() -> int {
    if (!h->have_embedding) {
      h->err = "No n2v2r embeddings found";
      return N2V2R_ERR_NOT_READY;
    }
    std::copy(h->sigma.begin(), h->sigma.end(), s);
    return N2V2R_OK;
  });
}

int n2v2r_set_embedding(n2v2r_handle* h, int num_layers, int64_t n, int d, const float* Y) {
  return guarded(h, [&]() -> int {
    if (num_layers < 1 || n < 1 || d < 1 || !Y) return N2V2R_ERR_BAD_ARG;
    if (h->comm || h->multi()) {
      h->err = "set_embedding is single-GPU only";
      return N2V2R_ERR_BAD_ARG;
    }
    h->K = num_layers;
    h->set_partition(n);
    h->d = d;
    h->ldy = d;
    h->Y.ensure(sizeof(float) * (size_t)num_layers * n * d);
    HIPCHK(hipMemcpyAsync(h->Y.p, Y, sizeof(float) * (size_t)num_layers * n * d,
                          hipMemcpyHostToDevice, h->stream));
    HIPCHK(hipStreamSynchronize(h->stream));
    h->sigma.assign(d, 0.0);
    h->have_embedding = true;
    h->ncmp = h->ncols = 0;
    return N2V2R_OK;
  });
}

}
```

Measured before the change: 694,700 nodes/s.

## Carve device buffers from shared arenas and write SpMM output directly into Y

Replaces many separate hipMalloc calls for CSR, transpose, column-block, sort, panel, pool and solver scratch buffers with single arena allocations carved into non-owning views. This cuts allocation overhead and fragmentation, and it falls back to per-buffer allocation if the arena allocation fails. It also adds a capture path so the column-block SpMM writes its stage-1 output straight into the Y embedding panel, which removes a per-block 2D copy. The pool is now sized up front from a fit estimate. The changes add lifetime complexity, because views depend on the arena and any arena reallocation invalidates them.

```diff
diff --git a/include/n2v2r.h b/include/n2v2r.h
--- a/include/n2v2r.h
+++ b/include/n2v2r.h
@@ -33,7 +33,8 @@
        N2V2R_EIG_TIME_SPMM = 16 ,
        N2V2R_EIG_TEST_NO_STAGNATION = 64 ,
        N2V2R_EIG_TEST_FAIL_ALONE = 128 ,
-       N2V2R_EIG_TEST_TRI_TIMEOUT = 1024  };
+       N2V2R_EIG_TEST_TRI_TIMEOUT = 1024 ,
+       N2V2R_EIG_TEST_POOL_ARENA_FAIL = 2048  };
 
 typedef struct n2v2r_handle n2v2r_handle;
 typedef struct n2v2r_simgroup n2v2r_simgroup;
diff --git a/include/n2v2r_diag.h b/include/n2v2r_diag.h
--- a/include/n2v2r_diag.h
+++ b/include/n2v2r_diag.h
@@ -19,6 +19,19 @@
 int n2v2r_pip_pass(n2v2r_handle* h, int64_t n, int nq, const float* Q, float* Za, float* Zb,
                    float tau, int first, int form, uint64_t seed, double* gram, double* R,
                    int* flags, int* any_flag, int* skipped);
+
+typedef struct {
+  int enabled;
+  int arena_allocs;
+  int single_block_allocs;
+  int pool_arenas;
+  int pool_blocks;
+  int pool_high;
+  int64_t pool_bytes;
+  int64_t scratch_bytes;
+  int64_t panel_bytes;
+} n2v2r_arena_info;
+int n2v2r_get_arena_info(n2v2r_handle* h, n2v2r_arena_info* info);
 
 typedef struct n2v2r_gram_info {
   int form;
diff --git a/node2vec2rank_amd/_lib.py b/node2vec2rank_amd/_lib.py
--- a/node2vec2rank_amd/_lib.py
+++ b/node2vec2rank_amd/_lib.py
@@ -28,6 +28,7 @@
 EIG_TIME_SPMM = 16
 EIG_TEST_NO_STAGNATION = 64
 EIG_TEST_FAIL_ALONE = 128
+EIG_TEST_POOL_ARENA_FAIL = 2048
 
 STRATEGY = {"sequential": 0, "one_vs_before": 1, "one_vs_rest": 2}
 METRIC = {"cosine": 0, "euclidean": 1, "correlation": 2}
@@ -53,6 +54,7 @@
     "n2v2r_soft_connectivity_chunks", "n2v2r_set_layer_corr_method",
     "n2v2r_soft_connectivity_method", "n2v2r_corr_ranks", "n2v2r_corr_standardise",
     "n2v2r_bench_corr_rows", "n2v2r_rr_stage", "n2v2r_embed_step",
+    "n2v2r_get_arena_info",
 ]
 UNIQUE_ID_BYTES = 128
 
@@ -99,6 +101,12 @@
     _fields_ = [("form", ctypes.c_int), ("launches", ctypes.c_int), ("ldu", ctypes.c_int),
                 ("rpw", ctypes.c_int), ("colmax_chunks", ctypes.c_int64),
                 ("colmax_rows", ctypes.c_int64)]
+
+
+class ArenaInfo(ctypes.Structure):
+    _fields_ = ([(k, ctypes.c_int) for k in ("enabled", "arena_allocs", "single_block_allocs",
+                                              "pool_arenas", "pool_blocks", "pool_high")] +
+                [(k, ctypes.c_int64) for k in ("pool_bytes", "scratch_bytes", "panel_bytes")])
 
 
 class RitzInfo(ctypes.Structure):
@@ -201,6 +209,7 @@
             "n2v2r_gram_apply": (_i, [_vp, _i, _p(np.float32), _vp, _p(np.float32),
                                       ctypes.POINTER(GramInfo)]),
             "n2v2r_embed_step": (_i, [_vp, _i, _i, _vp, _vp, ctypes.POINTER(EmbedInfo)]),
+            "n2v2r_get_arena_info": (_i, [_vp, ctypes.POINTER(ArenaInfo)]),
             "n2v2r_ritz_step": (_i, [_vp, _i, _i, _i, _i, _vp, _vp, _vp, _vp, _vp, _vp, _vp,
                                      ctypes.POINTER(RitzInfo)]),
             "n2v2r_block_gram": (_i, [_vp, _i, _i, _i, _vp, _vp, _vp, ctypes.POINTER(PassInfo)]),
@@ -866,6 +875,11 @@
             ctypes.byref(info)), "gram_apply")
         return W, Z, {k: getattr(info, k) for k, _ in GramInfo._fields_}
 
+    def arena_info(self):
+        info = ArenaInfo()
+        self._check(self.lib.n2v2r_get_arena_info(self.h, ctypes.byref(info)), "get_arena_info")
+        return {k: getattr(info, k) for k, _ in ArenaInfo._fields_}
+
     def embed_step(self, U, theta, b: int = 8):
         if U is None or theta is None:
             raise ValueError("embed_step: U and theta are required")
diff --git a/node2vec2rank_amd/build.py b/node2vec2rank_amd/build.py
--- a/node2vec2rank_amd/build.py
+++ b/node2vec2rank_amd/build.py
@@ -15,7 +15,7 @@
                "rr.hip", "rr_band.hip", "rr_sturm.hip", "ingest.hip", "engine.cpp", "layers.cpp",
                "comm.cpp", "gram_op.cpp", "solver.cpp", "ranking.cpp", "multi.cpp"]
 HOST_SOURCES: list = []
-HEADERS = ["common.h", "corr_tile.h", "pip_pass.h", "spmm_args.h", "engine.h", "gram_op.h", os.path.join("..", "..", "include", "n2v2r.h"),
+HEADERS = ["arena.h", "common.h", "corr_tile.h", "pip_pass.h", "spmm_args.h", "engine.h", "gram_op.h", os.path.join("..", "..", "include", "n2v2r.h"),
            os.path.join("..", "..", "include", "n2v2r_diag.h")]
 ARCH = os.environ.get("N2V2R_OFFLOAD_ARCH", "gfx950")
 _EXTRA = os.environ.get("N2V2R_EXTRA_HIP_FLAGS", "").split() if _TAG else []
diff --git a/node2vec2rank_amd/csrc/arena.h b/node2vec2rank_amd/csrc/arena.h
--- /dev/null
+++ b/node2vec2rank_amd/csrc/arena.h
@@ -0,0 +1,32 @@
+#pragma once
+
+#include <cstddef>
+#include <cstdint>
+
+namespace n2v2r_int {
+
+constexpr size_t kArenaAlign = 256;
+
+inline bool arena_carve(const size_t* sizes, size_t count, size_t* off, size_t* total) {
+  size_t at = 0;
+  for (size_t i = 0; i < count; ++i) {
+    const size_t s = sizes[i];
+    if (s > SIZE_MAX - (kArenaAlign - 1)) return false;
+    const size_t r = (s + kArenaAlign - 1) / kArenaAlign * kArenaAlign;
+    if (r > SIZE_MAX - at) return false;
+    at += r;
+  }
+  at = 0;
+  for (size_t i = 0; i < count; ++i) {
+    off[i] = at;
+    at += (sizes[i] + kArenaAlign - 1) / kArenaAlign * kArenaAlign;
+  }
+  *total = at;
+  return true;
+}
+
+inline size_t arena_stride(size_t bytes) {
+  return (bytes + kArenaAlign - 1) / kArenaAlign * kArenaAlign;
+}
+
+}
diff --git a/node2vec2rank_amd/csrc/engine.h b/node2vec2rank_amd/csrc/engine.h
--- a/node2vec2rank_amd/csrc/engine.h
+++ b/node2vec2rank_amd/csrc/engine.h
@@ -22,6 +22,7 @@
 
 #include "../../include/n2v2r.h"
 #include "../../include/n2v2r_diag.h"
+#include "arena.h"
 #include "common.h"
 
 #include "pip_pass.h"
@@ -258,17 +259,30 @@
   return v;
 }
 
+inline bool arena_enabled() {
+  const char* e = std::getenv("N2V2R_ARENA");
+  return !(e && e[0] == '0');
+}
+
 struct DevBuf {
   void* p = nullptr;
   size_t bytes = 0;
+  bool owned = true;
   DevBuf() = default;
   DevBuf(const DevBuf&) = delete;
   DevBuf& operator=(const DevBuf&) = delete;
   ~DevBuf() { release(); }
   void release() {
-    if (p) (void)hipFree(p);
+    if (p && owned) (void)hipFree(p);
     p = nullptr;
     bytes = 0;
+    owned = true;
+  }
+  void view(const DevBuf& a, size_t off, size_t b) {
+    release();
+    p = static_cast<char*>(a.p) + off;
+    bytes = b;
+    owned = false;
   }
   void ensure(size_t b, hipStream_t st = nullptr) {
     if (bytes >= b && p) return;
@@ -305,6 +319,7 @@
   void swap(DevBuf& o) {
     std::swap(p, o.p);
     std::swap(bytes, o.bytes);
+    std::swap(owned, o.owned);
   }
   template <class T>
   T* as() const {
@@ -312,7 +327,41 @@
   }
 };
 
+struct Carve {
+  DevBuf* buf;
+  size_t bytes;
+};
+inline void carve_views(DevBuf& arena, const std::vector<Carve>& want, hipStream_t st, bool raw) {
+  bool fits = true;
+  for (const Carve& c : want) fits = fits && (c.bytes == 0 || (c.buf->p && c.buf->bytes >= c.bytes));
+  if (fits) return;
+  if (arena_enabled()) {
+    std::vector<size_t> sizes, off(want.size());
+    for (const Carve& c : want) sizes.push_back(c.bytes);
+    size_t total = 0;
+    if (!arena_carve(sizes.data(), sizes.size(), off.data(), &total))
+      throw StatusFail{N2V2R_ERR_OUT_OF_MEMORY, "buffer group size overflows"};
+    for (const Carve& c : want) c.buf->release();
+    arena.release();
+    try {
+      if (raw) arena.ensure_raw(total);
+      else arena.ensure(total, st);
+      for (size_t i = 0; i < want.size(); ++i)
+        if (sizes[i]) want[i].buf->view(arena, off[i], sizes[i]);
+      return;
+    } catch (const StatusFail&) {
+      (void)hipGetLastError();
+    }
+  }
+  for (const Carve& c : want) {
+    if (!c.bytes) continue;
+    if (raw) c.buf->ensure_raw(c.bytes);
+    else c.buf->ensure(c.bytes, st);
+  }
+}
+
 struct LayerDev {
+  DevBuf csr_arena, t_arena;
   DevBuf indptr, indices, data;
   DevBuf t_indptr, t_indices, t_data;
   int64_t nnz = 0, t_nnz = 0;
@@ -335,6 +384,7 @@
                   t_nnz, t_unit ? 1 : 0};
   }
   struct ColBlocks {
+    DevBuf arena;
     DevBuf wo, idx, dat;
     CsrBlk blk[CB_MAX];
     int nb = 0;
@@ -353,11 +403,18 @@
     return CsrDev{c_indptr.as<int64_t>(), c_indices.as<int32_t>(), c_data.as<float>(), c_rows,
                   c_nnz, (symmetric ? unit : t_unit) ? 1 : 0};
   }
+  void drop_transpose() {
+    t_indptr.release();
+    t_indices.release();
+    t_data.release();
+    t_arena.release();
+  }
   void drop_col_blocks() {
     for (ColBlocks* c : {&cb, &cb_t}) {
       c->wo.release();
       c->idx.release();
       c->dat.release();
+      c->arena.release();
       c->built = false;
     }
     c_indptr.release();
@@ -438,7 +495,19 @@
 
 struct EigWorkspace {
   std::vector<std::unique_ptr<DevBuf>> pool;
+  std::vector<std::unique_ptr<DevBuf>> pool_arenas;
   size_t block_bytes = 0;
+  int pool_high = 0;
+  void drop_pool() {
+    pool.clear();
+    pool_arenas.clear();
+    pool_high = 0;
+  }
+  ~EigWorkspace() { drop_pool(); }
+  DevBuf scratch_arena;
+  DevBuf zk_arena;
+  int arena_allocs = 0, single_block_allocs = 0;
+  bool fail_pool_arena_once = false;
   std::vector<std::unique_ptr<DevBuf>> zk;
   DevBuf zg;
   DevBuf rinv, flg, anyflag, gsmall, csmall;
@@ -541,6 +610,7 @@
   }
   DevBuf rs_keys[2], rs_idx[2], rs_pos, rs_hist, rs_or, rs_and;
   DevBuf ing_keys[2], ing_pay[2], ing_hist, ing_flag;
+  DevBuf ing_arena;
   DevBuf tf_scr;
   DevBuf tom_out;
   DevBuf ypanel;
diff --git a/node2vec2rank_amd/csrc/gram_op.cpp b/node2vec2rank_amd/csrc/gram_op.cpp
--- a/node2vec2rank_amd/csrc/gram_op.cpp
+++ b/node2vec2rank_amd/csrc/gram_op.cpp
@@ -73,8 +73,23 @@
   tkind.clear();
   tbytes.clear();
   const size_t bb = sizeof(float) * npad * b;
-  while ((int)h->ews.zk.size() < K) h->ews.zk.emplace_back(new DevBuf());
-  for (int k = 0; k < K; ++k) h->ews.zk[k]->ensure(bb);
+  EigWorkspace& w = h->ews;
+  while ((int)w.zk.size() < K) w.zk.emplace_back(new DevBuf());
+  bool fits = true;
+  for (int k = 0; k < K; ++k) fits = fits && w.zk[k]->p && w.zk[k]->bytes >= bb;
+  if (!fits && arena_enabled()) {
+    const size_t stride = arena_stride(bb), count = w.zk.size();
+    for (auto& z : w.zk) z->release();
+    w.zk_arena.release();
+    try {
+      w.zk_arena.ensure(stride * count, st);
+      ++w.arena_allocs;
+      for (size_t k = 0; k < count; ++k) w.zk[k]->view(w.zk_arena, stride * k, bb);
+    } catch (const StatusFail&) {
+      (void)hipGetLastError();
+    }
+  }
+  for (int k = 0; k < K; ++k) w.zk[k]->ensure(bb);
   if (h->comm) {
     h->gath.ensure(sizeof(float) * h->world * npad * b);
     h->ews.zg.ensure(sizeof(float) * (size_t)K * h->world * npad * b);
@@ -197,10 +212,11 @@
   const double bytes = layer < 0 ? stage_bytes(true) : layer_bytes(layer, true);
   int te;
   if (col_blocks) {
-    SpmmTileArgs a = tile_args(false, k0, nk, 0, 8);
+    const bool cap = cap_y && layer < 0;
+    SpmmTileArgs a = tile_args(false, k0, nk, 0, cap ? cap_ld : 8);
     for (int i = 0; i < nk; ++i) {
       a.X[i] = xg;
-      a.Y[i] = zk(k0 + i);
+      a.Y[i] = cap ? cap_y + (size_t)(k0 + i) * cap_stride : zk(k0 + i);
     }
     te = tbeg();
     HIPCHK(n2v2r_launch_spmm_tile(a, st));
@@ -268,7 +284,8 @@
 
 void GramOp::stage2_tiled(float* Wout) {
   SpmmTileArgs s = tile_args(true, 0, K, 1, 8);
-  for (int k = 0; k < K; ++k) s.X[k] = stage2_in(k);
+  for (int k = 0; k < K; ++k) s.X[k] = cap_y ? cap_y + (size_t)k * cap_stride : stage2_in(k);
+  if (cap_y) s.ldx = cap_ld;
   s.Y[0] = Wout;
   const double b0 = stage_bytes(true), b1 = stage_bytes(false);
   const int te = tbeg();
@@ -366,6 +383,7 @@
     else
       stage2_flat(Wout);
   }
+  cap_y = nullptr;
   t_spmm += now_ms() - t0;
 }
 
diff --git a/node2vec2rank_amd/csrc/gram_op.h b/node2vec2rank_amd/csrc/gram_op.h
--- a/node2vec2rank_amd/csrc/gram_op.h
+++ b/node2vec2rank_amd/csrc/gram_op.h
@@ -48,6 +48,13 @@
   void apply(const float* X, float* Wout);
 
   float* zk(int k) const { return h->ews.zk[k]->as<float>(); }
+  float* cap_y = nullptr;
+  int64_t cap_ld = 0, cap_stride = 0;
+  void capture_next(float* y, int64_t ld, int64_t layer_stride) {
+    cap_y = y;
+    cap_ld = ld;
+    cap_stride = layer_stride;
+  }
   float* s2part(int k) const { return h->ews.s2part.as<float>() + (size_t)k * npad * 8; }
   void materialize();
   int pending_parts(const float* parts[SPMM_MAX_LAYERS]) const {
diff --git a/node2vec2rank_amd/csrc/layers.cpp b/node2vec2rank_amd/csrc/layers.cpp
--- a/node2vec2rank_amd/csrc/layers.cpp
+++ b/node2vec2rank_amd/csrc/layers.cpp
@@ -16,14 +16,21 @@
   out.built = true;
   out.usable = false;
   if (n <= 0 || out.cbits == 0) return;
-  DevBuf cnt, rp64, tsum;
-  cnt.ensure(sizeof(int32_t) * nb * n, st);
+  DevBuf tmp, cnt, rp64, tsum;
+  const int64_t ntiles = n2v2r_cb_scan_tiles(n, nb);
+  carve_views(tmp, {{&cnt, sizeof(int32_t) * nb * n}, {&tsum, sizeof(int64_t) * ntiles},
+                    {&rp64, sizeof(int64_t) * nb * (n + 1)}}, st, false);
+  const int64_t nw1 = ((n + ((int64_t)1 << wbits) - 1) >> wbits) + 1;
+  const size_t wo_bytes = sizeof(int32_t) * nb * nw1;
+  const size_t idx_bytes = sizeof(int32_t) * std::max<int64_t>(A.nnz, 1);
+  const size_t dat_bytes = A.unit ? 0 : sizeof(float) * std::max<int64_t>(A.nnz, 1);
+  const bool at_once = A.nnz <= (int64_t)INT32_MAX;
+  if (at_once)
+    carve_views(out.arena, {{&out.wo, wo_bytes}, {&out.idx, idx_bytes}, {&out.dat, dat_bytes}}, st,
+                false);
+  else
+    out.wo.ensure(wo_bytes, st);
   HIPCHK(n2v2r_launch_cb_count(A, cw, nb, cnt.as<int32_t>(), st));
-  const int64_t ntiles = n2v2r_cb_scan_tiles(n, nb);
-  tsum.ensure(sizeof(int64_t) * ntiles, st);
-  rp64.ensure(sizeof(int64_t) * nb * (n + 1), st);
-  const int64_t nw1 = ((n + ((int64_t)1 << wbits) - 1) >> wbits) + 1;
-  out.wo.ensure(sizeof(int32_t) * nb * nw1, st);
   HIPCHK(n2v2r_launch_cb_rowptrs(cnt.as<int32_t>(), n, nb, A.nnz, tsum.as<int64_t>(),
                                  (size_t)ntiles, rp64.as<int64_t>(), out.wo.as<int32_t>(), wbits,
                                  st));
@@ -39,8 +46,7 @@
     throw StatusFail{N2V2R_ERR_INTERNAL, "column-block split lost entries"};
   for (int j = 0; j < nb; ++j)
     if (ends[2 * j + 1] - ends[2 * j] > (int64_t)INT32_MAX) return;
-  out.idx.ensure(sizeof(int32_t) * std::max<int64_t>(A.nnz, 1), st);
-  if (!A.unit) out.dat.ensure(sizeof(float) * std::max<int64_t>(A.nnz, 1), st);
+  if (!at_once) carve_views(out.arena, {{&out.idx, idx_bytes}, {&out.dat, dat_bytes}}, st, false);
   HIPCHK(n2v2r_launch_cb_fill(A, cw, nb, rp64.as<int64_t>(), out.idx.as<int32_t>(),
                               A.unit ? nullptr : out.dat.as<float>(), out.cbits, wbits, st));
   HIPCHK(hipStreamSynchronize(st));
@@ -388,9 +394,11 @@
     DevBuf& dip = whole ? L.indptr : gip;
     DevBuf& dix = whole ? L.indices : gix;
     DevBuf& ddv = whole ? L.data : gdv;
-    dip.ensure(sizeof(int64_t) * (n + 1));
-    dix.ensure(sizeof(int32_t) * std::max<int64_t>(nnz, 1));
-    ddv.ensure(sizeof(float) * std::max<int64_t>(nnz, 1));
+    DevBuf garena;
+    carve_views(whole ? L.csr_arena : garena,
+                {{&dip, sizeof(int64_t) * (n + 1)},
+                 {&dix, sizeof(int32_t) * std::max<int64_t>(nnz, 1)},
+                 {&ddv, sizeof(float) * std::max<int64_t>(nnz, 1)}}, st, false);
     HIPCHK(hipMemcpyAsync(dip.p, indptr, sizeof(int64_t) * (n + 1), hipMemcpyHostToDevice, st));
     const bool ones = nnz > 0 && host_all_ones(nnz, data);
     if (nnz) {
@@ -408,10 +416,13 @@
     DevBuf& flag = h->ing_flag;
     flag.ensure_raw(sizeof(unsigned) * 4);
     HIPCHK(hipMemsetAsync(flag.p, 0, sizeof(unsigned) * 4, st));
-    if (need_t && nnz) {
-      keys[0].ensure_raw(sizeof(uint64_t) * nnz);
-      pay[0].ensure_raw(sizeof(int32_t) * nnz);
-    }
+    auto sort_scratch = [&]() {
+      carve_views(h->ing_arena,
+                  {{&keys[0], sizeof(uint64_t) * nnz}, {&pay[0], sizeof(int32_t) * nnz},
+                   {&keys[1], sizeof(uint64_t) * nnz}, {&pay[1], sizeof(int32_t) * nnz},
+                   {&hist, sizeof(uint32_t) * n2v2r_radix_hist_elems(nnz, 1)}}, st, true);
+    };
+    if (need_t && nnz) sort_scratch();
     HIPCHK(n2v2r_launch_csr_scan(dip.as<int64_t>(), dix.as<int32_t>(), ddv.as<float>(), n, n,
                                  need_t && nnz ? keys[0].as<uint64_t>() : nullptr,
                                  need_t && nnz ? pay[0].as<int32_t>() : nullptr,
@@ -426,23 +437,20 @@
     const bool unit = !(fl & 2u);
     const bool sorted = !(fl & 4u);
     auto transpose = [&](const int64_t* ip_, const int32_t* ix_, const float* dv_, bool have_keys,
-                         DevBuf& tp, DevBuf& tx, DevBuf& td) {
-      tp.ensure(sizeof(int64_t) * (n + 1));
-      tx.ensure(sizeof(int32_t) * std::max<int64_t>(nnz, 1));
-      if (!unit) td.ensure(sizeof(float) * std::max<int64_t>(nnz, 1));
+                         DevBuf& ta, DevBuf& tp, DevBuf& tx, DevBuf& td) {
+      carve_views(ta,
+                  {{&tp, sizeof(int64_t) * (n + 1)},
+                   {&tx, sizeof(int32_t) * std::max<int64_t>(nnz, 1)},
+                   {&td, unit ? 0 : sizeof(float) * std::max<int64_t>(nnz, 1)}}, st, false);
       if (nnz == 0) {
         HIPCHK(n2v2r_launch_csr_from_sorted(nullptr, nullptr, nullptr, 0, n, tp.as<int64_t>(),
                                             nullptr, nullptr, st));
         return;
       }
-      keys[0].ensure_raw(sizeof(uint64_t) * nnz);
-      pay[0].ensure_raw(sizeof(int32_t) * nnz);
-      keys[1].ensure_raw(sizeof(uint64_t) * nnz);
-      pay[1].ensure_raw(sizeof(int32_t) * nnz);
+      sort_scratch();
       if (!have_keys)
         HIPCHK(n2v2r_launch_csr_scan(ip_, ix_, dv_, n, n, keys[0].as<uint64_t>(),
                                      pay[0].as<int32_t>(), flag.as<unsigned>() + 1, st));
-      hist.ensure_raw(sizeof(uint32_t) * n2v2r_radix_hist_elems(nnz, 1));
       int bits = 1;
       while (bits < 31 && ((int64_t)1 << bits) < n) ++bits;
       int cur = 0;
@@ -457,12 +465,13 @@
                                           unit ? nullptr : td.as<float>(), st));
     };
     bool sym = symmetric == N2V2R_SYM_YES;
-    DevBuf gtp, gtx, gtd;
+    DevBuf gta, gtp, gtx, gtd;
+    DevBuf& ta = whole ? L.t_arena : gta;
     DevBuf& tp = whole ? L.t_indptr : gtp;
     DevBuf& tx = whole ? L.t_indices : gtx;
     DevBuf& td = whole ? L.t_data : gtd;
     if (need_t) {
-      transpose(dip.as<int64_t>(), dix.as<int32_t>(), ddv.as<float>(), true, tp, tx, td);
+      transpose(dip.as<int64_t>(), dix.as<int32_t>(), ddv.as<float>(), true, ta, tp, tx, td);
       if (symmetric == N2V2R_SYM_DETECT) {
         const float* tv = unit ? ddv.as<float>() : td.as<float>();
         HIPCHK(hipMemsetAsync(flag.as<unsigned>() + 2, 0, sizeof(unsigned), st));
@@ -471,8 +480,8 @@
                                           tp.as<int64_t>(), tx.as<int32_t>(), tv, n, nnz,
                                           flag.as<unsigned>() + 2, st));
         } else {
-          DevBuf sp_, sx, sv;
-          transpose(tp.as<int64_t>(), tx.as<int32_t>(), tv, false, sp_, sx, sv);
+          DevBuf sa, sp_, sx, sv;
+          transpose(tp.as<int64_t>(), tx.as<int32_t>(), tv, false, sa, sp_, sx, sv);
           HIPCHK(n2v2r_launch_csr_compare(sp_.as<int64_t>(), sx.as<int32_t>(),
                                           unit ? ddv.as<float>() : sv.as<float>(),
                                           tp.as<int64_t>(), tx.as<int32_t>(), tv, n, nnz,
@@ -491,6 +500,8 @@
     keys[1].release();
     pay[0].release();
     pay[1].release();
+    if (!hist.owned) hist.release();
+    h->ing_arena.release();
     auto slice = [&](DevBuf& sip, DevBuf& six, DevBuf& sdv, bool copy_values, DevBuf& oip,
                      DevBuf& oix, DevBuf& odv, int64_t& onnz) {
       int64_t p0 = 0, p1 = 0;
@@ -516,11 +527,7 @@
     if (whole) {
       L.nnz = nnz;
       L.t_nnz = nnz;
-      if (sym) {
-        L.t_indptr.release();
-        L.t_indices.release();
-        L.t_data.release();
-      }
+      if (sym) L.drop_transpose();
     } else {
       slice(gip, gix, gdv, true, L.indptr, L.indices, L.data, L.nnz);
       if (!sym) slice(gtp, gtx, gtd, !unit, L.t_indptr, L.t_indices, L.t_data, L.t_nnz);
@@ -1004,16 +1011,16 @@
       L.data.swap(a[k].dv);
       L.nnz = a[k].nnz;
       L.unit = a[k].unit;
+      L.csr_arena.release();
       if (L.symmetric) {
-        L.t_indptr.release();
-        L.t_indices.release();
-        L.t_data.release();
+        L.drop_transpose();
         L.t_nnz = L.nnz;
         L.t_unit = L.unit;
       } else {
         L.t_indptr.swap(t[k].ip);
         L.t_indices.swap(t[k].ix);
         L.t_data.swap(t[k].dv);
+        L.t_arena.release();
         L.t_nnz = t[k].nnz;
         L.t_unit = t[k].unit;
       }
diff --git a/node2vec2rank_amd/csrc/solver.cpp b/node2vec2rank_amd/csrc/solver.cpp
--- a/node2vec2rank_amd/csrc/solver.cpp
+++ b/node2vec2rank_amd/csrc/solver.cpp
@@ -132,6 +132,7 @@
   int flags = 0;
   bool flag(int f) const { return (flags & f) != 0; }
   int keep = 0, c_max = 0;
+  int ldu_fit = 0;
   double tol = 0, stag_cap = 0;
   int max_restarts = 0;
   bool sturm = false;
@@ -213,23 +214,65 @@
     for (DevBuf* d : {&w.rinv, &w.flg, &w.anyflag, &w.gsmall, &w.csmall, &w.tri, &w.refl,
                       &w.ytri, &w.tscr, &w.hband, &w.band, &w.varr, &w.taua, &w.rrerr, &w.fcoef,
                       &h->partial, &h->theta, &h->resid})
-      if (d->p) HIPCHK(hipMemsetAsync(d->p, 0xFF, d->bytes, st));
+      if (d->p && d->bytes) HIPCHK(hipMemsetAsync(d->p, 0xFF, d->bytes, st));
     for (auto& d : w.pool) HIPCHK(hipMemsetAsync(d->p, 0xFF, d->bytes, st));
     op.poison_scratch();
   }
 
+  int pool_bound = 0;
+  int blocks_out = 0;
+  bool pool_arena_ok = true;
+
+  int pool_blocks_of_fit() const {
+    const int qd = (d + b - 1) / b;
+    return lean ? nb_max + 3 + pb + qd : 2 * nb_max + 2 * pb + 2;
+  }
+
+  bool grow_pool(int count) {
+    EigWorkspace& w = h->ews;
+    const size_t stride = arena_stride(w.block_bytes);
+    std::unique_ptr<DevBuf> a(new DevBuf());
+    try {
+      if (w.fail_pool_arena_once) {
+        w.fail_pool_arena_once = false;
+        throw StatusFail{N2V2R_ERR_OUT_OF_MEMORY, "test: the pool arena reports failure"};
+      }
+      a->ensure(stride * (size_t)count, st);
+    } catch (const StatusFail&) {
+      (void)hipGetLastError();
+      pool_arena_ok = false;
+      return false;
+    }
+    ++w.arena_allocs;
+    for (int i = 0; i < count; ++i) {
+      w.pool.emplace_back(new DevBuf());
+      w.pool.back()->view(*a, stride * (size_t)i, w.block_bytes);
+      freelist.push_back(w.pool.back()->as<float>());
+    }
+    w.pool_arenas.push_back(std::move(a));
+    return true;
+  }
+
   float* take() {
+    EigWorkspace& w = h->ews;
     if (freelist.empty()) {
-      h->ews.pool.emplace_back(new DevBuf());
-      h->ews.pool.back()->ensure(sizeof(float) * npad * b, st);
-      return h->ews.pool.back()->as<float>();
+      const int missing = pool_bound - (int)w.pool.size();
+      if (!(arena_enabled() && pool_arena_ok && missing > 0 && grow_pool(missing))) {
+        w.pool.emplace_back(new DevBuf());
+        w.pool.back()->ensure(sizeof(float) * npad * b, st);
+        ++w.single_block_allocs;
+        freelist.push_back(w.pool.back()->as<float>());
+      }
     }
     float* p = freelist.back();
     freelist.pop_back();
+    w.pool_high = std::max(w.pool_high, ++blocks_out);
     return p;
   }
   void give(float* p) {
-    if (p) freelist.push_back(p);
+    if (!p) return;
+    freelist.push_back(p);
+    --blocks_out;
   }
 
   BlockList blocks(const std::vector<float*>& v, int from, int count) const {
@@ -454,60 +497,113 @@
   }
 
 
-  void reuse_pool() {
+  void reuse_pool(int bound = 0, int ahead = 0) {
+    EigWorkspace& w = h->ews;
     const size_t bb = sizeof(float) * npad * b;
-    if (h->ews.block_bytes != bb) {
-      h->ews.pool.clear();
-      h->ews.block_bytes = bb;
-    }
+    if (w.block_bytes != bb) {
+      w.drop_pool();
+      w.block_bytes = bb;
+    }
+    pool_bound = bound;
+    pool_arena_ok = true;
+    blocks_out = 0;
     freelist.clear();
-    for (auto& blk : h->ews.pool) freelist.push_back(blk->as<float>());
+    for (auto& blk : w.pool) freelist.push_back(blk->as<float>());
+    if (arena_enabled() && ahead > (int)w.pool.size()) grow_pool(ahead - (int)w.pool.size());
+  }
+
+  struct ScratchList {
+    std::vector<DevBuf*> buf;
+    std::vector<size_t> bytes;
+    void want(DevBuf& d, size_t b, bool used = true) {
+      buf.push_back(&d);
+      bytes.push_back(used ? std::max<size_t>(b, 16) : 0);
+    }
+  };
+  void place_scratch(const ScratchList& L) {
+    EigWorkspace& w = h->ews;
+    const size_t nbuf = L.buf.size();
+    bool fits = true;
+    for (size_t i = 0; i < nbuf; ++i)
+      fits = fits && (L.bytes[i] == 0 || (L.buf[i]->p && L.buf[i]->bytes >= L.bytes[i]));
+    if (fits) return;
+    if (arena_enabled()) {
+      std::vector<size_t> sizes(nbuf), off(nbuf);
+      for (size_t i = 0; i < nbuf; ++i) sizes[i] = std::max(L.bytes[i], L.buf[i]->bytes);
+      size_t total = 0;
+      if (!arena_carve(sizes.data(), nbuf, off.data(), &total))
+        throw StatusFail{N2V2R_ERR_OUT_OF_MEMORY, "solver scratch size overflows"};
+      for (DevBuf* d : L.buf) d->release();
+      w.scratch_arena.release();
+      bool ok = true;
+      try {
+        w.scratch_arena.ensure(total, st);
+      } catch (const StatusFail&) {
+        (void)hipGetLastError();
+        ok = false;
+      }
+      if (ok) {
+        ++w.arena_allocs;
+        for (size_t i = 0; i < nbuf; ++i) L.buf[i]->view(w.scratch_arena, off[i], sizes[i]);
+        return;
+      }
+    }
+    for (size_t i = 0; i < nbuf; ++i)
+      if (L.bytes[i]) L.buf[i]->ensure(L.bytes[i]);
   }
 
   void size_scratch() {
+    EigWorkspace& w = h->ews;
+    band_reduce = rr_reduce_fits(keep, c_max);
+    band_rr = b == 8 && !flag(N2V2R_EIG_DENSE_RR) && c_max <= N2V2R_BAND_MAXC &&
+              (band_reduce || rr_sturm_enabled());
+    sturm = band_rr && rr_sturm_enabled();
+    lean = b == 8 && band_rr && sturm && !lean_off && lean_enabled();
+    rb.lay_out(keep);
     h->partial_elems = std::max<size_t>(4096ull * 1024ull, (size_t)c_max * c_max * 8);
     h->partial_elems = std::max<size_t>(h->partial_elems,
                                         (size_t)((n + 8191) / 8192 + 24) * 2 * (c_max + 2 * b) * b);
-    h->partial.ensure(sizeof(double) * h->partial_elems);
-    h->ews.gsmall.ensure(sizeof(double) * (size_t)c_max * c_max);
-    h->ews.csmall.ensure(sizeof(float) * (size_t)c_max * c_max);
-    h->ews.tri.ensure(sizeof(double) * 3 * (size_t)c_max);
-    h->ews.refl.ensure(sizeof(double) * std::max<size_t>((size_t)c_max * c_max,
-                                                        (size_t)c_max * (c_max / 8 + 2) * 9));
-    h->ews.ytri.ensure(sizeof(double) * (size_t)c_max * keep);
-    h->ews.tscr.ensure(sizeof(double) * 6 * (size_t)((keep + 63) / 64 * 64) * c_max);
-    h->ews.trcoop.ensure(n2v2r_rr_tridiag_scratch_bytes(c_max));
-    h->ews.btf.ensure(n2v2r_rr_bt_scratch_bytes(c_max));
-    h->ews.rinv.ensure(sizeof(double) * 64 * 64);
-    h->ews.fcoef.ensure(sizeof(float) * (size_t)(c_max + 64) * 64);
-    h->ews.flg.ensure(sizeof(int) * 256);
-    h->ews.anyflag.ensure(sizeof(int) * 4);
-    h->theta.ensure(sizeof(double) * c_max);
-    h->resid.ensure(sizeof(double) * c_max);
-    band_reduce = rr_reduce_fits(keep, c_max);
-    band_rr = b == 8 && !flag(N2V2R_EIG_DENSE_RR) && c_max <= N2V2R_BAND_MAXC &&
-              (band_reduce || rr_sturm_enabled());
-    if (band_rr) {
-      h->ews.hband.ensure(sizeof(double) * ((size_t)(keep + b) * b + (size_t)nb_max * 2 * b * b));
-      h->ews.band.ensure(sizeof(double) * (size_t)c_max * (b + 1));
-      h->ews.varr.ensure(sizeof(double) * (size_t)(keep + b) * (keep + b));
-      h->ews.taua.ensure(sizeof(double) * (size_t)(keep + b));
-      h->ews.rrerr.ensure(sizeof(int) * 4);
-      h->ews.sturm.ensure(sizeof(double) * n2v2r_rr_sturm_scratch(c_max, keep));
-    }
-    sturm = band_rr && rr_sturm_enabled();
+    ScratchList L;
+    L.want(h->partial, sizeof(double) * h->partial_elems);
+    L.want(w.gsmall, sizeof(double) * (size_t)c_max * c_max);
+    L.want(w.csmall, sizeof(float) * (size_t)c_max * c_max);
+    L.want(w.tri, sizeof(double) * 3 * (size_t)c_max);
+    L.want(w.refl, sizeof(double) * std::max<size_t>((size_t)c_max * c_max,
+                                                    (size_t)c_max * (c_max / 8 + 2) * 9));
+    L.want(w.ytri, sizeof(double) * (size_t)c_max * keep);
+    L.want(w.tscr, sizeof(double) * 6 * (size_t)((keep + 63) / 64 * 64) * c_max);
+    L.want(w.trcoop, n2v2r_rr_tridiag_scratch_bytes(c_max));
+    L.want(w.btf, n2v2r_rr_bt_scratch_bytes(c_max));
+    L.want(w.rinv, sizeof(double) * 64 * 64);
+    L.want(w.fcoef, sizeof(float) * (size_t)(c_max + 64) * 64);
+    L.want(w.flg, sizeof(int) * 256);
+    L.want(w.anyflag, sizeof(int) * 4);
+    L.want(h->theta, sizeof(double) * c_max);
+    L.want(h->resid, sizeof(double) * c_max);
+    L.want(w.hband, sizeof(double) * ((size_t)(keep + b) * b + (size_t)nb_max * 2 * b * b), band_rr);
+    L.want(w.band, sizeof(double) * (size_t)c_max * (b + 1), band_rr);
+    L.want(w.varr, sizeof(double) * (size_t)(keep + b) * (keep + b), band_rr);
+    L.want(w.taua, sizeof(double) * (size_t)(keep + b), band_rr);
+    L.want(w.rrerr, sizeof(int) * 4, band_rr);
+    L.want(w.sturm, band_rr ? sizeof(double) * n2v2r_rr_sturm_scratch(c_max, keep) : 0, band_rr);
+    L.want(w.skipc, sizeof(int) * (4 + N2V2R_BAND_MAXC / 8));
+    L.want(w.rres, sizeof(double) * 128, lean);
+    L.want(w.dbgflag, sizeof(int) * 4);
+    L.want(w.tflag, sizeof(double) * 2);
+    L.want(w.rback, rb.bytes(rb.words));
+    L.want(w.g2, sizeof(double) * 2 * (size_t)(nb_max + 2) * 64, lean);
+    L.want(w.pair_ra, sizeof(double) * 64, lean);
+    L.want(w.pair_plan, sizeof(int) * N2V2R_PAIR_PLAN_WORDS, lean);
+    L.want(h->keys, sizeof(unsigned long long) * 1024 * (size_t)ldu_fit, ldu_fit > 0);
+    L.want(h->best, sizeof(unsigned long long) * ldu_fit, ldu_fit > 0);
+    L.want(h->colscale, sizeof(float) * ldu_fit, ldu_fit > 0);
+    place_scratch(L);
     part_p = h->partial.as<double>();
     part_n = h->partial_elems;
-    gsm_p = h->ews.gsmall.as<double>();
-    flg_p = h->ews.flg.as<int>();
-    any_p = h->ews.anyflag.as<int>();
-    lean = b == 8 && band_rr && sturm && !lean_off && lean_enabled();
-    h->ews.skipc.ensure(sizeof(int) * (4 + N2V2R_BAND_MAXC / 8));
-    HIPCHK(hipMemsetAsync(h->ews.skipc.p, 0, sizeof(int) * (4 + N2V2R_BAND_MAXC / 8), st));
-    if (lean) h->ews.rres.ensure(sizeof(double) * 128);
-    rb.lay_out(keep);
-    h->ews.dbgflag.ensure(sizeof(int) * 4);
-    h->ews.tflag.ensure(sizeof(double) * 2);
+    gsm_p = w.gsmall.as<double>();
+    flg_p = w.flg.as<int>();
+    any_p = w.anyflag.as<int>();
+    HIPCHK(hipMemsetAsync(w.skipc.p, 0, sizeof(int) * (4 + N2V2R_BAND_MAXC / 8), st));
     wh.assign(keep, 0.0);
     res2.assign(keep, 0.0);
   }
@@ -815,12 +911,14 @@
     const char* ycv = std::getenv("N2V2R_YCAP");
     const bool cap = op.col_blocks && !h->comm && b == 8 && qd * b == ldu &&
                      !(ycv && ycv[0] == '0');
+    const bool direct = cap && !(ycv && ycv[0] == 'c');
     if (cap) h->Y.ensure(sizeof(float) * (size_t)K * npad * ldu, st);
     for (int q = 0; q < qd; ++q) {
       MV[q] = take();
+      if (direct) op.capture_next(h->Y.as<float>() + (size_t)q * b, ldu, (int64_t)npad * ldu);
       op.apply(X[q], MV[q]);
       op.materialize();
-      if (cap)
+      if (cap && !direct)
         for (int k = 0; k < K; ++k)
           HIPCHK(hipMemcpy2DAsync(h->Y.as<float>() + (size_t)k * npad * ldu + (size_t)q * b,
                                   sizeof(float) * ldu, op.zk(k),
@@ -905,7 +1003,7 @@
     stats->rr_fallbacks = stats_rr_fallbacks;
     stats->est_scale = est_scale;
     stats->lean_checks = lean_checks;
-    stats->pool_blocks = (int)h->ews.pool.size();
+    stats->pool_blocks = h->ews.pool_high;
     stats->spmm_form = op.spmm_form();
     stats->stag_cap = stag_cap;
     stats->y_captured = y_captured ? 1 : 0;
@@ -931,9 +1029,13 @@
     pb = keep / b;
     nb_max = c_max / b;
     stag_cap = 2.0 * std::max(tol, std::sqrt((double)c_max) * 0x1p-24);
-    reuse_pool();
+    ldu_fit = ldu;
     op.setup(b, flag(N2V2R_EIG_TIME_SPMM));
     size_scratch();
+    if (flag(N2V2R_EIG_TEST_POOL_ARENA_FAIL)) h->ews.fail_pool_arena_once = true;
+    const int most = pool_blocks_of_fit();
+    reuse_pool(most, lean ? most : most - 2);
+    h->ews.fail_pool_arena_once = false;
     read_reorth_switches();
     poison_scratch();
 
@@ -1184,7 +1286,7 @@
     h->ncmp = h->ncols = 0;
     h->have_borda = false;
     for (DevBuf* b : {&h->ing_keys[0], &h->ing_keys[1], &h->ing_pay[0], &h->ing_pay[1],
-                      &h->ing_hist})
+                      &h->ing_hist, &h->ing_arena})
       b->release();
     const int ldu = ((d + 63) / 64) * 64;
     h->U.ensure(sizeof(float) * h->npad * ldu);
@@ -1423,6 +1525,27 @@
   });
 }
 
+int n2v2r_get_arena_info(n2v2r_handle* h, n2v2r_arena_info* info) {
+  if (h && h->multi()) h = h->ranks[0];
+  return guarded(h, [&]() -> int {
+    if (!info) return N2V2R_ERR_BAD_ARG;
+    const EigWorkspace& w = h->ews;
+    *info = n2v2r_arena_info{};
+    info->enabled = arena_enabled() ? 1 : 0;
+    info->arena_allocs = w.arena_allocs;
+    info->single_block_allocs = w.single_block_allocs;
+    info->pool_arenas = (int)w.pool_arenas.size();
+    info->pool_blocks = (int)w.pool.size();
+    info->pool_high = w.pool_high;
+    for (auto& a : w.pool_arenas) info->pool_bytes += (int64_t)a->bytes;
+    for (auto& d : w.pool)
+      if (d->owned) info->pool_bytes += (int64_t)d->bytes;
+    info->scratch_bytes = (int64_t)w.scratch_arena.bytes;
+    info->panel_bytes = (int64_t)w.zk_arena.bytes;
+    return N2V2R_OK;
+  });
+}
+
 int n2v2r_get_embedding(n2v2r_handle* h, float* Y) {
   if (h && h->multi()) return multi_get_embedding(h, Y);
   return guarded(h, [&]() -> int {
```

Measured after the change: 694,700 nodes/s. About the same (-0.0%).
